# cloudwego/dynamicgo

Measured on AMD Instinct MI355X. Metric: conv/j2t GB/s JSON in + msgs/s, 64K-batch device-resident, 1→8 MI355X, higher is better.
Workload: dtype u8; 1 GPU; C2: 65536 flat baseline.Simple messages <=256 B, seed 42; global_batch=65536, msgs_per_rank=65536, thrift_bytes_rank0=6662181, flags=1, parallelism=dp1 (one batch per rank, descriptor broadcast over -), no data-path collective, inflight=2

## Files before the change

### dynamicgo_amd/csrc/flat_image.h

```cpp
#pragma once
#include <stdint.h>
#include <string.h>

namespace dg {

constexpr int FLI_WLO = -40;
constexpr int FLI_WN = 64;
constexpr uint32_t FLI_NP10U = 20, FLI_NP10D = 23;
constexpr uint32_t FLI_P10U = 0;
constexpr uint32_t FLI_P10D = FLI_P10U + 8 * FLI_NP10U;
constexpr uint32_t FLI_PW = FLI_P10D + 8 * FLI_NP10D;
constexpr uint32_t FLI_TABS = (FLI_PW + 8 * FLI_WN + 15) & ~15u;

static const double FLI_P10D_VALUES[FLI_NP10D] = {1e0,  1e1,  1e2,  1e3,  1e4,  1e5,  1e6,  1e7,  1e8,  1e9,  1e10, 1e11,
                                                  1e12, 1e13, 1e14, 1e15, 1e16, 1e17, 1e18, 1e19, 1e20, 1e21, 1e22};

constexpr uint32_t fli_blob16(uint32_t total_len) { return (total_len + 15) & ~15u; }
constexpr uint32_t fli_len(uint32_t total_len) { return fli_blob16(total_len) + FLI_TABS; }

inline void fli_build(const uint8_t *blob, uint32_t total_len, const uint64_t (*pw_hi)[2], uint8_t *img)
{
    const uint32_t b16 = fli_blob16(total_len);
    memset(img, 0, fli_len(total_len));
    memcpy(img, blob, total_len);
    uint8_t *t = img + b16;
    uint64_t v = 1;
    for (uint32_t k = 0; k < FLI_NP10U; k++, v *= 10) memcpy(t + FLI_P10U + 8 * k, &v, 8);
    memcpy(t + FLI_P10D, FLI_P10D_VALUES, sizeof FLI_P10D_VALUES);
    for (int k = 0; k < FLI_WN; k++) memcpy(t + FLI_PW + 8 * k, &pw_hi[FLI_WLO + 348 + k][1], 8);
}

}
```

### dynamicgo_amd/csrc/host_internal.h

```cpp
#pragma once
#include <hip/hip_runtime.h>

#include <stdint.h>
#include <stdlib.h>

#include <algorithm>
#include <memory>
#include <mutex>
#include <vector>

#include "../../include/dgj2t.h"
#include "../../include/dgj2t_desc.h"
#include "host_layout.h"

__attribute__((visibility("hidden"))) int set_err(int code, const char *fmt, ...);
#define HIPCHK(x)                                                                              \
    do {                                                                                       \
        hipError_t e_ = (x);                                                                   \
        if (e_ != hipSuccess) return set_err(DG_E_HIP, "%s: %s", #x, hipGetErrorString(e_));  \
    } while (0)


template <class T, hipError_t (*FREE)(void *)>
struct ArrBase {
    T *p = nullptr;
    uint64_t cap = 0;
    ArrBase() = default;
    ArrBase(ArrBase &&o) noexcept : p(o.p), cap(o.cap) { o.p = nullptr, o.cap = 0; }
    ArrBase &operator=(ArrBase &&o) noexcept
    {
        std::swap(p, o.p);
        std::swap(cap, o.cap);
        return *this;
    }
    ~ArrBase() { reset(); }
    void reset()
    {
        if (p) (void)FREE(p);
        p = nullptr, cap = 0;
    }
    operator T *() const { return p; }
};

template <class T>
struct DevArr : ArrBase<T, hipFree> {
    int alloc(uint64_t n)
    {
        HIPCHK(hipMalloc(&this->p, n * sizeof(T)));
        this->cap = n;
        return DG_OK;
    }
    int grow(uint64_t want)
    {
        if (this->cap >= want) return DG_OK;
        const uint64_t nc = std::max<uint64_t>(want, this->cap * 2);
        this->reset();
        return alloc(nc);
    }
};

template <class T>
struct PinArr : ArrBase<T, hipHostFree> {
    int alloc(uint64_t n, unsigned flags = hipHostMallocDefault)
    {
        HIPCHK(hipHostMalloc((void **)&this->p, n * sizeof(T), flags));
        this->cap = n;
        return DG_OK;
    }
    int grow(uint64_t want)
    {
        if (this->cap >= want) return DG_OK;
        const uint64_t nc = std::max<uint64_t>(std::max<uint64_t>(want, this->cap * 2), (1 << 16) / sizeof(T));
        this->reset();
        static const unsigned fl = getenv("DG_HOST_NUMA") ? hipHostMallocNumaUser : hipHostMallocDefault;
        return alloc(nc, fl);
    }
};

template <class H, hipError_t (*DESTROY)(H)>
struct Handle {
    H h = nullptr;
    Handle() = default;
    Handle(Handle &&o) noexcept : h(o.h) { o.h = nullptr; }
    Handle &operator=(Handle &&o) noexcept
    {
        std::swap(h, o.h);
        return *this;
    }
    ~Handle()
    {
        if (h) (void)DESTROY(h);
    }
    operator H() const { return h; }
};
struct Event : Handle<hipEvent_t, hipEventDestroy> {
    hipError_t create() { return hipEventCreate(&h); }
    hipError_t create(unsigned flags) { return hipEventCreateWithFlags(&h, flags); }
};
struct Stream : Handle<hipStream_t, hipStreamDestroy> {
    hipError_t create(unsigned flags) { return hipStreamCreateWithFlags(&h, flags); }
};

struct StreamOrder {
    Event done;
    hipStream_t last = nullptr;
    hipError_t acquire(hipStream_t s)
    {
        if (!done) {
            hipError_t e = done.create(hipEventDisableTiming | hipEventDisableSystemFence);
            if (e != hipSuccess) return e;
        }
        return last && last != s ? hipStreamWaitEvent(s, done, 0) : hipSuccess;
    }
    hipError_t publish(hipStream_t s)
    {
        hipError_t e = hipEventRecord(done, s);
        if (e == hipSuccess) last = s;
        return e;
    }
    hipError_t wait_host() const { return last ? hipEventSynchronize(done) : hipSuccess; }
    template <class T>
    int grow(DevArr<T> &a, uint64_t want)
    {
        if (a.cap >= want) return DG_OK;
        HIPCHK(wait_host());
        return a.grow(want);
    }
    void forget(const hipStream_t *s, int n)
    {
        if (std::find(s, s + n, last) != s + n) last = nullptr;
    }
};

struct SharedWs : StreamOrder {
    DevArr<uint8_t> ws;
};

struct AltCounters {
    uint32_t *set[2] = {nullptr, nullptr};
    uint32_t bytes = 0, cur = 0;
    uint32_t *mine() const { return set[cur]; }
    uint32_t *other() const { return set[cur ^ 1u]; }
    int init(DevArr<uint32_t> &buf, uint32_t words)
    {
        if (int rc = buf.alloc(4)) return rc;
        HIPCHK(hipMemset(buf, 0, 16));
        HIPCHK(hipDeviceSynchronize());
        set[0] = buf, set[1] = buf + words, bytes = 4 * words;
        return DG_OK;
    }
    void finish(bool ok, hipStream_t s)
    {
        if (ok) cur ^= 1u;
        else
            for (uint32_t *p : set) (void)hipMemsetAsync(p, 0, bytes, s);
    }
};

enum : uint32_t {
    CNT_BAIL = 0,
    CNT_BIG = 1,
    CNT_WAVEQ = 2,
    CNT_HUGE = 3,
    CNT_DEEP = 4,
    CNT_DEEP_DONE = 5,
    CNT_PACK = 6,
    CNT_T2J_A = 8,
    CNT_T2J_B = 16,
    T2J_DEEPQ = 0,
    T2J_BIG = 1,
    T2J_WAVEQ = 2,
    T2J_BAIL = 3,
};
constexpr uint32_t DG_NCOUNTS = 24;
constexpr uint32_t DG_J2T_COUNTS_BYTES = 6 * 4;
constexpr uint32_t FRAME_CAP = 4096;

constexpr int DG_MAX_SCRATCH = 40;
struct Scratch : StreamOrder {
    hipStream_t owner = nullptr;
    Stream side;
    Event side_done, side_go;
    DevArr<uint8_t> ws_fast;
    uint64_t ws_fast_lanes = 0;
    DevArr<uint64_t> deep_list;
    DevArr<uint32_t> counts;
    DevArr<uint32_t> bail_list, big_list;
    DevArr<uint8_t> ws_wave, ws_deep;
    DevArr<uint64_t> sums;
    DevArr<uint8_t> d_frame;
    std::vector<uint8_t> frame;
    DevArr<uint32_t> t2j_list;
    DevArr<uint32_t> t2j_big;
    DevArr<uint32_t> t2j_bail;
    AltCounters t2j_cnt;
    ~Scratch()
    {
        (void)wait_host();
        if (side) (void)hipStreamSynchronize(side);
    }
};

struct Knobs {
    int64_t flat = -1;
    int64_t wave_min = 512;
    int64_t wave_occ = 0;
    int64_t small_mpw = 64;
    int64_t list_blocks = 16;
    int64_t t2j_spread = 0;
    int64_t t2j_overlap = 0;
    int64_t t2j_wave_min = 256;
    int64_t flat_wrap = -1;
    int64_t tget_spread = 0;
    int64_t cut_wave_min = 4096;
    int64_t edit_reuse_rec = 0;
    int64_t edit_lanes = 4;
    int64_t edit_wave_min = 4096;
    int64_t kids_wide_min = 256;
    int64_t kids_no_scan = 0;
    int64_t cols_full_search = 0;
};

struct PipeBuf;
struct PipeBufDelete {
    void operator()(PipeBuf *p) const;
};

struct dg_ctx {
    int device = 0;
    Stream stream;
    int n_cu = 0;
    Knobs knobs;
    uint32_t rr = 0;
    std::mutex mu;
    const Event *kt = nullptr;
    Event fork_ev;
    std::vector<Event> side_ev;
    std::vector<Stream> side;
    SharedWs tget;
    DevArr<uint32_t> tget_list, tget_cnt_buf;
    AltCounters tget_cnt;
    StreamOrder cut;
    DevArr<uint32_t> cut_list, cut_cnt_buf;
    AltCounters cut_cnt;
    StreamOrder edit;
    DevArr<dg_tget_rec> edit_rec;
    uint64_t edit_rec_n = 0;
    StreamOrder editm;
    DevArr<dg_tget_rec> editm_rec;
    SharedWs kids;
    DevArr<uint32_t> kids_list, kids_cnt_buf;
    AltCounters kids_cnt;
    DevArr<uint64_t> kids_sums;
    SharedWs cols;
    DevArr<uint32_t> cols_list, cols_cnt_buf;
    AltCounters cols_cnt;
    DevArr<uint64_t> cols_sums;
    SharedWs t2j_tok;
    SharedWs t2j_deep;
    PinArr<uint8_t> h_down;
    PinArr<uint8_t> h_up;
    DevArr<uint64_t> d_pack_off;
    DevArr<uint8_t> d_pack;
    DevArr<uint8_t> d_cb;
    DevArr<uint64_t> d_aux;
    DevArr<uint64_t> d_ret;
    DevArr<uint32_t> d_out_len;
    DevArr<uint64_t> d_out_off;
    DevArr<uint8_t> d_out;
    DevArr<uint64_t> d_in_off;
    DevArr<uint8_t> d_json;
    DevArr<unsigned long long> d_stats;
    DevArr<uint64_t> d_zero;
    DevArr<uint32_t> d_pending;
    std::vector<std::unique_ptr<Scratch>> scratch;
    std::mutex pipe_mu;
    PinArr<uint8_t> h_pipe_aux, h_pipe_out;
    PinArr<uint8_t> h_pipe_ovf;
    DevArr<uint64_t> d_pipe_cur;
    std::vector<std::unique_ptr<PipeBuf, PipeBufDelete>> pipe;
    ~dg_ctx()
    {
        (void)hipSetDevice(device);
        if (stream) (void)hipStreamSynchronize(stream);
    }
};

struct Entry {
    std::unique_lock<std::mutex> lk;
    hipStream_t s = nullptr;
    int rc = DG_OK;
    Entry(dg_ctx *c, bool ok, void *stream = nullptr, const char *what = "bad args")
    {
        if (!ok) {
            rc = set_err(DG_E_INVALID, "%s", what);
            return;
        }
        lk = std::unique_lock<std::mutex>(c->mu);
        const hipError_t e = hipSetDevice(c->device);
        if (e != hipSuccess) rc = set_err(DG_E_HIP, "hipSetDevice(c->device): %s", hipGetErrorString(e));
        s = stream ? (hipStream_t)stream : (hipStream_t)c->stream;
    }
};

struct dg_desc {
    dg_ctx *ctx = nullptr;
    DevArr<uint8_t> d_blob;
    DevArr<uint8_t> d_flat;
    size_t len = 0;
    dg_desc_hdr hdr;
    DevArr<uint8_t> d_side;
    std::vector<uint8_t> hblob;
    size_t side_len = 0;
};

struct dg_path {
    dg_ctx *ctx;
    DevArr<uint8_t> d_blob;
    dg_path_hdr hdr;
};

struct dg_cols {
    dg_ctx *ctx;
    DevArr<uint8_t> d_blob;
    dg_path_hdr hdr;
    uint8_t kinds[DG_TGET_MAX_PATHS];
};

struct TGetBatch {
    const uint8_t *src;
    const uint64_t *in_off;
    uint64_t n;
    dg_tget_rec *rec;
    uint64_t *val_off;
    uint32_t *val_len;
    uint64_t max_len;
};

__attribute__((visibility("hidden"))) int dg_i_path_validate(const void *blob, size_t len, dg_path_hdr &h);

__attribute__((visibility("hidden"))) int tget_launch(dg_ctx *c, const dg_path *ps, uint8_t root_type,
                                                      const TGetBatch &b, hipStream_t s);

struct HMIn {
    const dg_hm_entry *tab = nullptr;
    uint32_t n_hm = 0;
    const uint8_t *bytes = nullptr;
    const dg_cb_entry *vm = nullptr;
};

struct BatchArgs {
    const uint8_t *src = nullptr;
    const uint64_t *in_off = nullptr;
    uint64_t n = 0, flags = 0;
    uint8_t *out = nullptr;
    const uint64_t *out_off = nullptr;
    uint32_t *out_len = nullptr;
    uint64_t *ret = nullptr;
    uint32_t *pending = nullptr;
    uint64_t max_len = 0;
    HMIn hm;
    uint64_t *aux = nullptr;
};

struct HostOut {
    uint8_t *out;
    uint64_t out_cap;
    uint64_t *out_off, *out_need;
};

struct PackChain {
    const uint64_t *base_in = nullptr;
    uint64_t dst_cap = 0;
    int base_mod16 = 0;
    uint64_t *ret_dst = nullptr, *cur_out = nullptr, *ovf_out = nullptr;
    hipEvent_t pack_after = nullptr;
};

__attribute__((visibility("hidden"))) void dg_i_scratch_release(dg_ctx *c, const hipStream_t *s, int n);

__attribute__((visibility("hidden"))) int scratch_for(dg_ctx *c, hipStream_t s, Scratch **out);

__attribute__((visibility("hidden"))) int dg_i_convert_pack(dg_ctx *c, const dg_desc *d, uint32_t root,
                                                            const BatchArgs &b, uint8_t *packed, uint64_t *pack_off,
                                                            hipStream_t s, const PackChain &ch);

__attribute__((visibility("hidden"))) int dg_i_pack_scan(dg_ctx *c, hipStream_t s, const BatchArgs &b, uint8_t *d_dst,
                                                         uint64_t *d_dst_off);

inline int empty_batch(uint64_t *off, uint64_t *need)
{
    if (off) off[0] = 0;
    if (need) *need = 0;
    return DG_OK;
}

struct HostBatch {
    dg_ctx *const c;
    const hipStream_t s;
    std::vector<uint64_t> io, so, vo, src;
    uint64_t n = 0, max_len = 0;
    bool busy = false;
    HostBatch(dg_ctx *c_, hipStream_t s_) : c(c_), s(s_) {}
    HostBatch(const HostBatch &) = delete;
    ~HostBatch()
    {
        if (busy) (void)hipStreamSynchronize(s);
    }
    int sync()
    {
        busy = false;
        HIPCHK(hipStreamSynchronize(s));
        return DG_OK;
    }
    int copy(void *dst, const void *from, uint64_t bytes, hipMemcpyKind kind)
    {
        busy = true;
        if (bytes) HIPCHK(hipMemcpyAsync(dst, from, bytes, kind, s));
        return DG_OK;
    }
    template <class F>
    int layout(const uint64_t *in_off, const uint64_t *idx, uint64_t m, F cap_of, bool with_slots = true,
               bool longest = true)
    {
        n = m, io.resize(m + 1), src.resize(idx ? m : 0);
        if (with_slots) so.resize(m + 1);
        uint64_t bad = 0, cap = 0;
        const int rc = dg::hl_layout(in_off, idx, m, cap_of, io.data(), with_slots ? so.data() : nullptr,
                                     idx ? src.data() : nullptr, longest && !idx ? &max_len : nullptr, &bad, &cap);
        if (rc == dg::HL_DESCENDING) return set_err(DG_E_INVALID, "in_off not ascending");
        if (rc) return set_err(DG_E_INVALID, "message %llu: an output of %llu bytes", (unsigned long long)bad,
                               (unsigned long long)cap);
        return DG_OK;
    }
    int messages(const uint64_t *in_off, uint64_t m, bool longest = true)
    {
        return layout(in_off, nullptr, m, [](uint64_t, uint64_t) { return uint64_t(0); }, false, longest);
    }
    int values(const uint64_t *val_off, uint64_t m, uint64_t K, uint64_t *max_val)
    {
        vo.resize(m * K + 1);
        return dg::hl_rebase(val_off, m * K, K, vo.data(), max_val) ? set_err(DG_E_INVALID, "val_off not ascending") : DG_OK;
    }
    int upload_messages(const uint8_t *thrift, const uint64_t *in_off)
    {
        int rc;
        if ((rc = c->d_json.grow(io[n] + 64)) || (rc = c->d_in_off.grow(n + 1))) return rc;
        if (src.empty()) rc = copy(c->d_json, thrift + in_off[0], io[n], hipMemcpyHostToDevice);
        for (uint64_t k = 0; k < src.size() && !rc; k++)
            rc = copy(c->d_json + io[k], thrift + src[k], io[k + 1] - io[k], hipMemcpyHostToDevice);
        if (rc) return rc;
        HIPCHK(hipMemsetAsync(c->d_json + io[n], 0, 64, s));
        return copy(c->d_in_off, io.data(), (n + 1) * 8, hipMemcpyHostToDevice);
    }
    int upload_slots(bool packs = true)
    {
        int rc;
        if ((rc = c->d_out.grow(so[n] + 64)) || (rc = c->d_out_off.grow(n + 1)) || (rc = c->d_out_len.grow(n + 1)) ||
            (rc = c->d_ret.grow(n + 1)) ||
            (packs && ((rc = c->d_pack.grow(so[n] + 64)) || (rc = c->d_pack_off.grow(n + 1)))))
            return rc;
        return copy(c->d_out_off, so.data(), (n + 1) * 8, hipMemcpyHostToDevice);
    }
    int upload_values(const uint8_t *val, const uint64_t *val_off, uint64_t shared)
    {
        const uint64_t vtotal = val_off ? vo.back() : shared;
        int rc;
        if ((rc = c->d_cb.grow(vtotal + 64)) || (rc = c->d_aux.grow(vo.size())) ||
            (rc = copy(c->d_cb, val_off ? val + val_off[0] : val, vtotal, hipMemcpyHostToDevice)))
            return rc;
        HIPCHK(hipMemsetAsync(c->d_cb + vtotal, 0, 64, s));
        return copy(c->d_aux, vo.data(), vo.size() * 8, hipMemcpyHostToDevice);
    }
    int pack(bool by_ret, uint64_t *ret, uint64_t *pack_off, uint32_t *len = nullptr)
    {
        BatchArgs pb;
        pb.out = c->d_out, pb.out_off = c->d_out_off, pb.out_len = c->d_out_len, pb.n = n;
        if (by_ret) pb.ret = c->d_ret;
        int rc;
        if ((rc = dg_i_pack_scan(c, s, pb, c->d_pack, c->d_pack_off)) ||
            (rc = copy(ret, c->d_ret, n * 8, hipMemcpyDeviceToHost)) ||
            (len && (rc = copy(len, c->d_out_len, n * 4, hipMemcpyDeviceToHost))) ||
            (rc = copy(pack_off, c->d_pack_off, (n + 1) * 8, hipMemcpyDeviceToHost)))
            return rc;
        return sync();
    }
    int download(void *dst, const void *d_from, uint64_t bytes)
    {
        if (int rc = copy(dst, d_from, bytes, hipMemcpyDeviceToHost)) return rc;
        return bytes ? sync() : DG_OK;
    }
    int pack_and_download(const HostOut &o, uint64_t *ret)
    {
        if (int rc = pack(false, ret, o.out_off)) return rc;
        const uint64_t total = o.out_off[n];
        if (o.out_need) *o.out_need = total;
        if (total > o.out_cap || (!o.out && total))
            return set_err(DG_E_NOMEM, "output needs %llu bytes", (unsigned long long)total);
        return download(o.out, c->d_pack, total);
    }
};

inline int upload_blob(DevArr<uint8_t> &d, const void *blob, size_t len, const char *what)
{
    if (int rc = d.alloc(len + 16)) return rc;
    hipError_t e = hipMemcpy(d, blob, len, hipMemcpyHostToDevice);
    if (e == hipSuccess) e = hipMemset(d + len, 0, 16);
    if (e == hipSuccess) e = hipDeviceSynchronize();
    if (e != hipSuccess) return set_err(DG_E_HIP, "%s upload: %s", what, hipGetErrorString(e));
    return DG_OK;
}

template <class P>
void destroy_with_blob(P *p)
{
    if (!p) return;
    {
        Entry g(p->ctx, true);
        p->d_blob.reset();
    }
    delete p;
}

inline uint32_t edit_step_extra(uint32_t kind, uint32_t key_len)
{
    return kind == DG_PS_FIELD ? 3u : kind == DG_PS_INDEX ? 0u : kind == DG_PS_STRKEY ? 4u + key_len
           : kind == DG_PS_BINKEY ? key_len : 8u;
}

template <class Lane, class Wave>
hipError_t launch_splice_routes(const dg_ctx *c, uint64_t n, uint32_t waves, bool no_wave, Lane lane, Wave wave)
{
    hipError_t err = hipSuccess;
    if (c->knobs.edit_wave_min > 0) {
        const int64_t g = c->knobs.edit_lanes;
        lane(g == 4 || g == 16 ? (uint32_t)g : 1u);
        err = hipGetLastError();
    }
    if (err == hipSuccess && !no_wave) {
        const uint64_t want = (n + waves - 1) / waves;
        wave((uint32_t)std::min<uint64_t>(want, (uint64_t)c->n_cu * 8));
        err = hipGetLastError();
    }
    return err;
}
```

### dynamicgo_amd/csrc/j2t_fast.h

```cpp
#pragma once
#include "j2t_device.h"

namespace dg {

#ifdef DG_FPROF
DGI unsigned long long *fprof_slots()
{
    __shared__ unsigned long long s_fp[16][17];
    return &s_fp[0][0];
}
DGI void fprof_mark(int k)
{
    const uint64_t now = __builtin_amdgcn_s_memtime();
    const uint32_t lane = threadIdx.x & 63, w = threadIdx.x >> 6;
    const uint64_t ex = __builtin_amdgcn_read_exec();
    if (lane == (uint32_t)__builtin_ctzll(ex)) {
        unsigned long long *f = fprof_slots() + w * 17;
        f[k] += now - f[16];
        f[16] = now;
    }
}
#define FP_MARK(k) fprof_mark(k)
#else
#define FP_MARK(k)
#endif

#define SI typename S::idx

constexpr uint32_t FK_STRUCT = 1, FK_MAP = 2, FK_LIST = 3;
constexpr uint32_t FAST_LDS_DEPTH = 8;

struct FFrame {
    uint32_t a;
    uint32_t b;
    uint64_t u;
};
typedef __attribute__((address_space(3))) FFrame LFFrame;
typedef const __attribute__((address_space(3))) double lds_f64;

constexpr uint64_t FAST_FLAGS = DG_F_ALLOW_UNKNOWN | DG_F_WRITE_DEFAULT | DG_F_ENABLE_VM | DG_F_ENABLE_I2S |
                                DG_F_WRITE_REQUIRE | DG_F_NO_BASE64 | DG_F_WRITE_OPTIONAL | DG_F_NO_WRITE_BASE |
                                DG_F_ENABLE_HM | DG_F_HM_SPLIT | DG_F_CB_COLLECT;

constexpr int EL_WLO = -40;
constexpr int EL_WN = 64;
struct FastTabs {
    const __attribute__((address_space(3))) uint64_t *p10u;
    lds_f64 *p10d;
    const __attribute__((address_space(3))) uint64_t *pw = nullptr;
};
DGI void el_window_fill(uint64_t *pw, uint32_t t)
{
    if (t < (uint32_t)EL_WN) pw[t] = DG_POW10_M128[EL_WLO + 348 + (int)t][1];
}
DGI bool eisel_lemire_t(uint64_t mant, int exp10, int sgn, double &val, const FastTabs &tb)
{
    if (exp10 < -348 || exp10 > 347) return false;
    const uint32_t wi = (uint32_t)(exp10 - EL_WLO);
    const uint64_t p_hi = tb.pw && wi < (uint32_t)EL_WN ? tb.pw[wi] : DG_POW10_M128[exp10 + 348][1];
    return eisel_lemire_p(mant, exp10, sgn, val, p_hi);
}


template <class S>
DGI uint32_t digits8(S &src, SI i, uint64_t &x)
{
    uint64_t w = src.get8(i);
    const uint32_t xl = (uint32_t)w ^ 0x30303030u, xh = (uint32_t)(w >> 32) ^ 0x30303030u;
    x = (uint64_t)xl | ((uint64_t)xh << 32);
    uint32_t ndl = (((xl & 0x7F7F7F7Fu) + 0x76767676u) | xl) & 0x80808080u;
    uint32_t ndh = (((xh & 0x7F7F7F7Fu) + 0x76767676u) | xh) & 0x80808080u;
    SI lim = src.n - i;
    if (lim < 8) {
        if (lim <= 4) {
            ndh = 0x80808080u;
            if (lim < 4) ndl |= lim <= 0 ? 0x80808080u : (0x80808080u & (~0u << (lim << 3)));
        } else {
            ndh |= 0x80808080u & (~0u << ((lim - 4) << 3));
        }
    }
    if (ndl) return (uint32_t)__builtin_ctz(ndl) >> 3;
    return ndh ? 4u + ((uint32_t)__builtin_ctz(ndh) >> 3) : 8u;
}

DGI uint32_t swar_val4(uint32_t x, uint32_t k)
{
    uint32_t y = k >= 4 ? x : (k == 0 ? 0u : x << ((4 - k) << 3));
    y &= 0x0F0F0F0Fu;
    y = (((y << 3) + (y << 1)) + (y >> 8)) & 0x00FF00FFu;
    return __umul24(y & 0xFFu, 100u) + (y >> 16);
}
DGI uint64_t swar_val(uint64_t x, uint32_t t)
{
    const uint32_t t1 = t < 4 ? t : 4u, t2 = t - t1;
    const uint32_t v1 = swar_val4((uint32_t)x, t1);
    if (!t2) return v1;
    const uint32_t v2 = swar_val4((uint32_t)(x >> 32), t2);
    const uint32_t p = t2 == 1 ? 10u : t2 == 2 ? 100u : t2 == 3 ? 1000u : 10000u;
    return (uint64_t)v1 * p + v2;
}

DGI uint32_t acc_digits(uint64_t &man, int &nd, uint64_t x, uint32_t k, const FastTabs &tb)
{
    (void)tb;
    uint32_t room = (uint32_t)(19 - nd);
    uint32_t t = k < room ? k : room;
    if (t) {
        uint32_t p = (t & 1) ? 10u : 1u;
        p = (t & 2) ? p * 100u : p;
        p = (t & 4) ? p * 10000u : p;
        p = (t & 8) ? 100000000u : p;
        man = man * (uint64_t)p + swar_val(x, t);
        nd += (int)t;
    }
    return t;
}

DGI bool atof_exact_l(uint64_t man, int exp, int sgn, double &val, const FastTabs &tb)
{
    val = (double)man;
    if (man >> 52 != 0) return false;
    val = with_sign(val, sgn);
    if (exp == 0 || man == 0) return true;
    if (exp > 0 && exp <= 15 + 22) {
        if (exp > 22) {
            val = __dmul_rn(val, tb.p10d[exp - 22]);
            exp = 22;
        }
        if (val > 1e15 || val < -1e15) return false;
        val = __dmul_rn(val, tb.p10d[exp]);
        return true;
    }
    if (exp < 0 && exp >= -22) {
        val = __ddiv_rn(val, tb.p10d[-exp]);
        return true;
    }
    return false;
}

template <class S>
DGI bool fast_int_regs(const S &src, int64_t &iv, double &dv, int32_t &end)
{
    const int32_t n = (int32_t)src.n;
    if (n < 1 || n > 20) return false;
    const uint64_t a0 = src.get8(0), a1 = src.get8(8), a2 = src.get8(16);
    const uint32_t neg = (uint8_t)a0 == '-' ? 1u : 0u;
    const uint32_t nd = (uint32_t)n - neg;
    const uint64_t d0 = neg ? (a0 >> 8) | (a1 << 56) : a0, d1 = neg ? (a1 >> 8) | (a2 << 56) : a1,
                   d2 = neg ? a2 >> 8 : a2;
    const uint64_t x0 = d0 ^ 0x3030303030303030ull, x1 = d1 ^ 0x3030303030303030ull, x2 = d2 ^ 0x3030303030303030ull;
    auto nondig = [](uint64_t x) { return (((x & 0x7F7F7F7F7F7F7F7Full) + 0x7676767676767676ull) | x) & 0x8080808080808080ull; };
    auto upto = [](uint32_t k) { return k >= 8 ? ~0ull : (1ull << (k << 3)) - 1; };
    const uint32_t t0 = nd < 8 ? nd : 8u, t1 = nd <= 8 ? 0u : nd - 8 < 8 ? nd - 8 : 8u, t2 = nd <= 16 ? 0u : nd - 16;
    const uint64_t bad = (nondig(x0) & upto(t0)) | (nondig(x1) & upto(t1)) | (nondig(x2) & upto(t2));
    const uint32_t f = (uint32_t)(x0 & 0xFF);
    if (nd < 1 || nd > 19 || bad || (f == 0 && nd > 1)) return false;
    auto p10 = [](uint32_t t) {
        uint32_t p = (t & 1) ? 10u : 1u;
        p = (t & 2) ? p * 100u : p;
        p = (t & 4) ? p * 10000u : p;
        return (t & 8) ? 100000000u : p;
    };
    uint64_t man = swar_val(x0, t0);
    man = man * (uint64_t)p10(t1) + swar_val(x1, t1);
    man = man * (uint64_t)p10(t2) + swar_val(x2, t2);
    if ((man >> 63) && !(neg && man == (1ull << 63))) return false;
    const int sgn = neg ? -1 : 1;
    iv = (int64_t)(man * (uint64_t)(int64_t)sgn);
    dv = man ? with_sign((double)man, sgn) : 0.0;
    end = n;
    return true;
}

template <class S>
DGI bool fast_dec_regs(const S &src, uint64_t &man, int &exp10, int &sgn)
{
    const int32_t n = (int32_t)src.n;
    if (n < 3 || n > 21) return false;
    const uint64_t a0 = src.get8(0), a1 = src.get8(8), a2 = src.get8(16);
    const uint32_t neg = (uint8_t)a0 == '-' ? 1u : 0u;
    const uint32_t len = (uint32_t)n - neg;
    const uint64_t d0 = neg ? (a0 >> 8) | (a1 << 56) : a0, d1 = neg ? (a1 >> 8) | (a2 << 56) : a1,
                   d2 = neg ? a2 >> 8 : a2;
    auto upto = [](uint32_t k) { return k >= 8 ? ~0ull : (1ull << (k << 3)) - 1; };
    auto eqdot = [](uint64_t x) {
        const uint64_t y = x ^ 0x2E2E2E2E2E2E2E2Eull;
        return ~(((y & 0x7F7F7F7F7F7F7F7Full) + 0x7F7F7F7F7F7F7F7Full) | y | 0x7F7F7F7F7F7F7F7Full);
    };
    const uint32_t u0 = len < 8 ? len : 8u, u1 = len <= 8 ? 0u : len - 8 < 8 ? len - 8 : 8u,
                   u2 = len <= 16 ? 0u : len - 16;
    const uint64_t m0 = eqdot(d0) & upto(u0), m1 = eqdot(d1) & upto(u1), m2 = eqdot(d2) & upto(u2);
    if (__builtin_popcountll(m0) + __builtin_popcountll(m1) + __builtin_popcountll(m2) != 1) return false;
    const uint32_t pd = m0 ? (uint32_t)__builtin_ctzll(m0) >> 3
                       : m1 ? 8u + ((uint32_t)__builtin_ctzll(m1) >> 3) : 16u + ((uint32_t)__builtin_ctzll(m2) >> 3);
    if (pd < 1 || pd + 2 > len) return false;
    const uint64_t s0 = (d0 >> 8) | (d1 << 56), s1 = (d1 >> 8) | (d2 << 56), s2 = d2 >> 8;
    const uint64_t k0 = upto(pd), k1 = pd <= 8 ? 0ull : upto(pd - 8), k2 = pd <= 16 ? 0ull : upto(pd - 16);
    const uint64_t r0 = (d0 & k0) | (s0 & ~k0), r1 = (d1 & k1) | (s1 & ~k1), r2 = (d2 & k2) | (s2 & ~k2);
    const uint32_t nd = len - 1;
    const uint64_t x0 = r0 ^ 0x3030303030303030ull, x1 = r1 ^ 0x3030303030303030ull, x2 = r2 ^ 0x3030303030303030ull;
    auto nondig = [](uint64_t x) { return (((x & 0x7F7F7F7F7F7F7F7Full) + 0x7676767676767676ull) | x) & 0x8080808080808080ull; };
    const uint32_t t0 = nd < 8 ? nd : 8u, t1 = nd <= 8 ? 0u : nd - 8 < 8 ? nd - 8 : 8u, t2 = nd <= 16 ? 0u : nd - 16;
    const uint64_t bad = (nondig(x0) & upto(t0)) | (nondig(x1) & upto(t1)) | (nondig(x2) & upto(t2));
    if (nd > 19 || bad || ((x0 & 0xFF) == 0 && pd > 1)) return false;
    auto p10 = [](uint32_t t) {
        uint32_t p = (t & 1) ? 10u : 1u;
        p = (t & 2) ? p * 100u : p;
        p = (t & 4) ? p * 10000u : p;
        return (t & 8) ? 100000000u : p;
    };
    uint64_t m = swar_val(x0, t0);
    m = m * (uint64_t)p10(t1) + swar_val(x1, t1);
    m = m * (uint64_t)p10(t2) + swar_val(x2, t2);
    man = m;
    exp10 = -(int)(nd - pd);
    sgn = neg ? -1 : 1;
    return true;
}

template <class S, class = void>
struct is_regsrc {
    static constexpr bool value = false;
};
template <class S>
struct is_regsrc<S, decltype((void)S::kRegs)> {
    static constexpr bool value = S::kRegs;
};

template <class S>
DGI bool fast_vnumber(S &src, SI &p, const FastTabs &tb, int64_t &iv, double &dv, bool &isint)
{
    SI i = p;
    uint64_t man = 0;
    int exp10 = 0, sgn = 1;
    bool trunc = false, regdec = false;
    if constexpr (is_regsrc<S>::value) {
        int32_t e;
        if (p == 0 && fast_int_regs(src, iv, dv, e)) {
            isint = true;
            p = (SI)e;
            return true;
        }
        if (p == 0 && fast_dec_regs(src, man, exp10, sgn)) {
            regdec = true;
            i = (SI)src.n;
        }
    }
    if (!regdec) {
    uint8_t c = src.at(i);
    if (c == '-') {
        sgn = -1;
        c = src.at(++i);
    }
    if ((uint8_t)(c - '0') > 9) return false;
    isint = true;
    iv = 0;
    dv = 0.0;
    if (c == '0') {
        uint8_t c1 = src.at(i + 1);
        if (c1 != '.' && c1 != 'e' && c1 != 'E') {
            p = i + 1;
            return true;
        }
    }
    int nd = 0;
    bool dbl = false;
    uint64_t x;
    for (;;) {
        uint32_t k = digits8(src, i, x);
        uint32_t t = acc_digits(man, nd, x, k, tb);
        exp10 += (int)(k - t);
        i += k;
        if (k < 8) break;
    }
    if (exp10 > 0) trunc = true;
    if (src.at(i) == '.') {
        i++;
        dbl = true;
        if ((uint8_t)(src.at(i) - '0') > 9) return false;
    }
    if (man == 0 && exp10 == 0) {
        while (src.at(i) == '0') {
            i++;
            exp10--;
        }
        nd = 0;
    }
    while (dbl && nd < 19) {
        uint32_t k = digits8(src, i, x);
        uint32_t t = acc_digits(man, nd, x, k, tb);
        exp10 -= (int)t;
        i += t;
        if (t < 8) break;
    }
    while (dbl) {
        uint32_t k = digits8(src, i, x);
        if (k) trunc = true;
        i += k;
        if (k < 8) break;
    }
    c = src.at(i);
    if (c == 'e' || c == 'E') {
        int esm = 1, e = 0;
        dbl = true;
        c = src.at(++i);
        if (c == '+' || c == '-') {
            esm = c == '+' ? 1 : -1;
            c = src.at(++i);
        }
        if ((uint8_t)(c - '0') > 9) return false;
        while ((uint8_t)(c - '0') <= 9) {
            if (e < 10000) e = e * 10 + (c - '0');
            c = src.at(++i);
        }
        exp10 += e * esm;
    } else if (!dbl) {
        bool ovf = exp10 != 0 || ((man >> 63) == 1 && (((uint64_t)(int64_t)sgn) & man) != (1ull << 63));
        if (!ovf) {
            iv = (int64_t)(man * (uint64_t)(int64_t)sgn);
            dv = with_sign((double)man, sgn);
            p = i;
            return true;
        }
    }
    }
    double val;
    if (!atof_exact_l(man, exp10, sgn, val, tb)) {
        if (!eisel_lemire_t(man, exp10, sgn, val, tb)) return false;
        if (trunc) {
            double vu;
            if (!eisel_lemire_t(man + 1, exp10, sgn, vu, tb) || vu != val) return false;
        }
    }
    if ((__double_as_longlong(val) << 1) == 0xFFE0000000000000ull) return false;
    isint = false;
    dv = val;
    p = i;
    return true;
}

template <class O>
DGI bool emit_number(O &out, uint8_t tt, bool isint, int64_t iv, double dv)
{
    switch (tt) {
    case DG_T_BYTE: out.w8(isint ? (uint8_t)iv : (uint8_t)cvt32(dv)); return true;
    case DG_T_I16: out.w16(isint ? (uint16_t)iv : (uint16_t)cvt32(dv)); return true;
    case DG_T_I32: out.w32(isint ? (uint32_t)iv : (uint32_t)cvt32(dv)); return true;
    case DG_T_I64: out.w64(isint ? (uint64_t)iv : (uint64_t)cvt64(dv)); return true;
    case DG_T_DOUBLE: out.w64((uint64_t)__double_as_longlong(dv)); return true;
    }
    return false;
}

template <class S, class O>
DGI void fast_copy(S &src, SI s0, SI n, O &out)
{
    SI i = 0;
    for (; i + 8 <= n; i += 8) out.wle(src.get8(s0 + i), 8);
    if (i < n) out.wle(src.get8(s0 + i), (uint32_t)(n - i));
}

template <class S>
DGI bool hex4w(S &src, SI i, uint32_t &v)
{
    uint32_t w = (uint32_t)src.get8(i);
    uint32_t r = 0;
#pragma unroll
    for (int k = 0; k < 4; k++) {
        int h = hexv((uint8_t)(w >> (8 * k)));
        if (h < 0) return false;
        r = (r << 4) | (uint32_t)h;
    }
    v = r;
    return true;
}

template <class S, class O>
DGI bool fast_unquote(S &src, SI s0, SI nb, O &out)
{
    SI i = s0, end = s0 + nb;
    while (i < end) {
        uint64_t w = src.get8(i);
        SI rem = end - i;
        uint64_t m = eqbytes(w, '\\');
        if (rem < 8) m &= (1ull << (rem << 3)) - 1;
        if (m == 0) {
            uint32_t k = rem < 8 ? (uint32_t)rem : 8u;
            out.wle(w, k);
            i += k;
            continue;
        }
        uint32_t j = (uint32_t)__builtin_ctzll(m) >> 3;
        if (j) out.wle(w, j);
        i += j;
        if (end - i < 2) return false;
        uint8_t c = src.at(i + 1);
        uint8_t cc;
        switch (c) {
        case '/': cc = '/'; break;
        case '"': cc = '"'; break;
        case 'b': cc = '\b'; break;
        case 'f': cc = '\f'; break;
        case 'n': cc = '\n'; break;
        case 'r': cc = '\r'; break;
        case 't': cc = '\t'; break;
        case '\\': cc = '\\'; break;
        case 'u': cc = 0; break;
        default: return false;
        }
        if (c != 'u') {
            out.w8(cc);
            i += 2;
            continue;
        }
        if (end - i < 6) return false;
        uint32_t r0, r1;
        if (!hex4w(src, i + 2, r0)) return false;
        i += 6;
        if (r0 <= 0x7f) {
            out.w8((uint8_t)r0);
        } else if (r0 <= 0x7ff) {
            out.wle((0xc0 | (r0 >> 6)) | ((0x80 | (r0 & 0x3f)) << 8), 2);
        } else if (r0 < 0xd800 || r0 > 0xdfff) {
            out.wle((0xe0 | (r0 >> 12)) | ((0x80 | ((r0 >> 6) & 0x3f)) << 8) | ((0x80 | (r0 & 0x3f)) << 16), 3);
        } else {
            if (end - i < 6 || r0 > 0xdbff || src.at(i) != '\\' || src.at(i + 1) != 'u') return false;
            if (!hex4w(src, i + 2, r1)) return false;
            if (r1 < 0xdc00 || r1 > 0xdfff) return false;
            i += 6;
            r0 = ((r0 - 0xd800) << 10) + (r1 - 0xdc00) + 0x10000;
            out.wle((0xf0 | (r0 >> 18)) | ((0x80 | ((r0 >> 12) & 0x3f)) << 8) | ((0x80 | ((r0 >> 6) & 0x3f)) << 16) |
                        ((uint64_t)(0x80 | (r0 & 0x3f)) << 24),
                    4);
        }
    }
    return true;
}

template <class S>
DGI bool fast_string(S &src, SI &p, Out &out)
{
    SI s0 = p;
    bool esc;
    SI e = advance_string(src, s0, esc);
    if (e < 0) return false;
    p = e;
    SI nb = e - 1 - s0;
    if (!esc) {
        out.w32((uint32_t)nb);
        fast_copy(src, s0, nb, out);
        return true;
    }
    uint64_t lp = out.alloc(4);
    uint64_t st = out.len;
    if (!fast_unquote(src, s0, nb, out)) return false;
    out.put32(lp, (uint32_t)(out.len - st));
    return true;
}

DGI bool b64_4(uint32_t w, uint32_t &o)
{
    const uint32_t H = 0x80808080u;
    if (w & H) return false;
#define DG_GE(lo) ((w + (uint32_t)(0x80 - (lo)) * 0x01010101u) & H)
    const uint32_t up = DG_GE('A') & ~DG_GE('Z' + 1);
    const uint32_t lw = DG_GE('a') & ~DG_GE('z' + 1);
    const uint32_t dg = DG_GE('0') & ~DG_GE('9' + 1);
#undef DG_GE
    const uint32_t pl = zb32(w ^ 0x2B2B2B2Bu), sl = zb32(w ^ 0x2F2F2F2Fu);
    if ((up | lw | dg | pl | sl) != H) return false;
    const uint32_t off = (ff32(up) & 0xBFBFBFBFu) | (ff32(lw) & 0xB9B9B9B9u) | (ff32(dg) & 0x04040404u) |
                         (ff32(pl) & 0x13131313u) | (ff32(sl) & 0x10101010u);
    const uint32_t v = ((w & 0x7F7F7F7Fu) + (off & 0x7F7F7F7Fu)) ^ ((w ^ off) & H);
    const uint32_t t = ((v & 0x3Fu) << 18) | (((v >> 8) & 0x3Fu) << 12) | (((v >> 16) & 0x3Fu) << 6) | (v >> 24);
    o = (t >> 16) | (t & 0xFF00u) | ((t & 0xFFu) << 16);
    return true;
}
DGI bool b64_8(uint64_t w, uint64_t &o)
{
    uint32_t lo, hi;
    const bool a = b64_4((uint32_t)w, lo), b = b64_4((uint32_t)(w >> 32), hi);
    o = (uint64_t)lo | ((uint64_t)hi << 24);
    return a && b;
}

template <class S>
DGI bool fast_binary(S &src, SI &p, Out &out)
{
    SI s0 = p;
    bool esc;
    SI e = advance_string(src, s0, esc);
    if (e < 0 || esc) return false;
    p = e;
    SI nb = e - 1 - s0;
    int64_t want = -1;
    if ((nb & 3) == 0) {
        const uint8_t c2 = nb ? src.raw(s0 + nb - 2) : 0, c3 = nb ? src.raw(s0 + nb - 1) : 0;
        want = (int64_t)(nb / 4 * 3) - (c3 == '=' ? (c2 == '=' ? 2 : 1) : 0);
    }
    uint64_t lp = 0;
    if (want >= 0) out.w32((uint32_t)want);
    else lp = out.alloc(4);
    SI ip = 0;
    int64_t op = 0;
    while (ip + 8 <= nb) {
        uint64_t o;
        if (!b64_8(src.get8(s0 + ip), o)) break;
        out.wle(o, 6);
        ip += 8;
        op += 6;
    }
    if (ip < nb) {
        op = b64decode_from(out, src, s0, nb, ip, op);
        if (op < 0) return false;
    }
    if (want >= 0) return op == want;
    out.put32(lp, (uint32_t)op);
    return true;
}

template <class S, int AS>
DGI bool key_eq(S &src, SI k0, uint32_t kn, const __attribute__((address_space(AS))) uint64_t *pk)
{
    for (uint32_t j = 0; j < kn; j += 8) {
        uint64_t a = src.get8(k0 + j);
        uint32_t rem = kn - j;
        if (rem < 8) a &= (1ull << (rem << 3)) - 1;
        if (a != pk[j >> 3]) return false;
    }
    return true;
}

template <bool LEAN = false, class S, class DV>
DGI bool fast_convert(const DV &D, S &src, Out &out, uint64_t flag, uint32_t root, LFFrame *fr, uint32_t fstride,
                      const FastTabs &tb)
{
    if (src.n == 0 || ldrec(&D.T[root]).ttype == DG_T_STRING) return false;
    SI p = 0;
    uint32_t sp = 0;
    uint32_t ca = 0, ck = 0, cb = 0;
    uint64_t cu = 0;
    bool null_val = false;
    uint64_t unwind = 0;
    uint32_t lastf = 0;
    uint32_t td = root;
    bool vmv = false;
    uint8_t c;

#define FAST_PUSH(na, nk, nu)                                             \
    do {                                                                  \
        if (sp) {                                                         \
            if (sp > FAST_LDS_DEPTH) return false;                        \
            LFFrame &f_ = fr[(sp - 1) * fstride];                         \
            f_.a = ca;                                                    \
            f_.b = ck | (cb << 2);                                        \
            f_.u = cu;                                                    \
        }                                                                 \
        sp++;                                                             \
        ca = (na);                                                        \
        ck = (nk);                                                        \
        cb = 0;                                                           \
        cu = (nu);                                                        \
    } while (0)
#define FAST_POP()                                                        \
    do {                                                                  \
        if (--sp) {                                                       \
            const LFFrame &f_ = fr[(sp - 1) * fstride];                   \
            ca = f_.a;                                                    \
            ck = f_.b & 3;                                                \
            cb = f_.b >> 2;                                               \
            cu = f_.u;                                                    \
        }                                                                 \
    } while (0)

    for (;;) {
        FP_MARK(0);
        c = src.at(p++);
        while (c <= ' ') {
            if (!isspace_(c)) return false;
            c = src.at(p++);
        }
        const dg_type t = ldrec(&D.T[td]);
        bool opened = false;
        FP_MARK(1);
        if (vmv) {
            vmv = false;
            const bool quoted = c == '"';
            bool number = true;
            if (quoted) {
                if (t.ttype == DG_T_STRING) {
                    if (!fast_string(src, p, out)) return false;
                    number = false;
                } else if (src.at(p) == '"') {
                    if constexpr (LEAN) return false;
                    const dg_field f = ldrec(&D.F[lastf]);
                    if (f.dflt_len != DG_NONE) {
                        for (uint32_t j = 0; j < f.dflt_len; j++) out.w8(D.P[f.dflt_off + j]);
                    } else {
                        switch (t.ttype) {
                        case DG_T_BOOL:
                        case DG_T_BYTE: out.w8(0); break;
                        case DG_T_I16: out.w16(0); break;
                        case DG_T_I32: out.w32(0); break;
                        case DG_T_I64:
                        case DG_T_DOUBLE: out.w64(0); break;
                        default: return false;
                        }
                    }
                    p += 1;
                    number = false;
                }
            } else {
                if (c != '-' && (uint8_t)(c - '0') > 9) return false;
                p -= 1;
            }
            if (number) {
                const SI s0 = p;
                int64_t iv;
                double dv;
                bool isint;
                if (!fast_vnumber(src, p, tb, iv, dv, isint)) return false;
                if (t.ttype == DG_T_STRING) {
                    out.w32((uint32_t)(p - s0));
                    fast_copy(src, s0, p - s0, out);
                } else if (t.ttype == DG_T_I16) {
                    emit_number(out, DG_T_I16, isint, iv, dv);
                    emit_number(out, DG_T_BYTE, isint, iv, dv);
                } else if (t.ttype == DG_T_BOOL || !emit_number(out, t.ttype, isint, iv, dv)) {
                    return false;
                }
                if (quoted) {
                    if (src.at(p) != '"') return false;
                    p += 1;
                }
            }
            goto after_value;
        }
        switch (c) {
        case '"':
            if (t.ttype != DG_T_STRING) return false;
            if ((flag & DG_F_NO_BASE64) == 0 && (t.flags & DG_TF_BINARY)) {
                if (!fast_binary(src, p, out)) return false;
                FP_MARK(2);
            } else {
                if (!fast_string(src, p, out)) return false;
                FP_MARK(3);
            }
            break;
        case '0': case '1': case '2': case '3': case '4':
        case '5': case '6': case '7': case '8': case '9': case '-': {
            p -= 1;
            int64_t iv;
            double dv;
            bool isint;
            if (!fast_vnumber(src, p, tb, iv, dv, isint)) return false;
            FP_MARK(4);
            if (!emit_number(out, t.ttype, isint, iv, dv)) return false;
            FP_MARK(5);
            break;
        }
        case 't':
            if (p + 3 > src.n || (uint32_t)src.get8(p - 1) != VS_TRUE || t.ttype != DG_T_BOOL) return false;
            p += 3;
            out.w8(1);
            break;
        case 'f':
            if (p + 4 > src.n || (uint32_t)src.get8(p) != VS_ALSE || t.ttype != DG_T_BOOL) return false;
            p += 4;
            out.w8(0);
            break;
        case 'n':
            if (p + 3 > src.n || (uint32_t)src.get8(p - 1) != VS_NULL || sp == 0) return false;
            p += 3;
            null_val = true;
            break;
        case '[': {
            if (t.ttype != DG_T_LIST && t.ttype != DG_T_SET) return false;
            out.w8(ldrec(&D.T[t.elem]).ttype);
            uint64_t bp = out.alloc(4);
            FAST_PUSH(t.elem, FK_LIST, bp);
            opened = true;
            break;
        }
        case '{':
            if (t.ttype == DG_T_STRUCT) {
                const dg_struct sd = ldrec(&D.S[t.st]);
                if (sd.req_words != 1) return false;
                if ((flag & DG_F_ENABLE_HM) && (sd.flags & DG_SF_HTTP_MAPPING)) return false;
                FAST_PUSH(t.st, FK_STRUCT, D.R[sd.req_begin]);
            } else if (t.ttype == DG_T_MAP) {
                out.wle(ldrec(&D.T[t.key]).ttype | ((uint32_t)ldrec(&D.T[t.elem]).ttype << 8), 2);
                uint64_t bp = out.alloc(4);
                FAST_PUSH(t.elem, FK_MAP, bp | ((uint64_t)t.key << 32));
            } else {
                return false;
            }
            opened = true;
            break;
        default:
            return false;
        }

        after_value:
        FP_MARK(6);
        bool first = opened;
        for (;;) {
            if (sp == 0) {
                out.finish();
                return out.len <= out.cap;
            }
            c = src.at(p++);
            while (c <= ' ') {
                if (!isspace_(c)) return false;
                c = src.at(p++);
            }
            if (ck == FK_LIST) {
                if (first) {
                    first = false;
                    if (c == ']') {
                        FAST_POP();
                        continue;
                    }
                    p -= 1;
                    td = ca;
                    break;
                }
                if (null_val) null_val = false;
                else cb++;
                if (c == ',') {
                    td = ca;
                    break;
                }
                if (c != ']') return false;
                out.put32(cu, cb);
                FAST_POP();
                continue;
            }
            if (first) {
                first = false;
                if (c == '}') {
                    if (ck == FK_MAP) {
                        FAST_POP();
                        continue;
                    }
                    goto close_struct;
                }
            } else if (ck == FK_MAP) {
                if (null_val) {
                    null_val = false;
                    out.set_len(unwind);
                } else {
                    cb++;
                }
                if (c == '}') {
                    out.put32((uint32_t)cu, cb);
                    FAST_POP();
                    continue;
                }
                if (c != ',') return false;
                c = src.at(p++);
                while (c <= ' ') {
                    if (!isspace_(c)) return false;
                    c = src.at(p++);
                }
            } else {
                if (null_val) {
                    null_val = false;
                    const dg_field f = ldrec(&D.F[lastf]);
                    const dg_struct sd = ldrec(&D.S[ca]);
                    uint64_t m = 1ull << (lastf - sd.field_begin);
                    if (f.required == DG_REQ_DEFAULT || f.required == DG_REQ_REQUIRED) cu |= m;
                    else if (f.required == DG_REQ_OPTIONAL) cu &= ~m;
                    out.set_len(unwind);
                }
                if (c == '}') goto close_struct;
                if (c != ',') return false;
                c = src.at(p++);
                while (c <= ' ') {
                    if (!isspace_(c)) return false;
                    c = src.at(p++);
                }
            }
            FP_MARK(7);
            if (c != '"') return false;
            {
                SI k0 = p;
                uint32_t kn;
                int32_t fi = -1;
                dg_field f;
                if (ck == FK_STRUCT) {
                    const dg_struct sdp = ldrec(&D.S[ca]);
                    if (cb < sdp.n_fields) {
                        f = ldrec(&D.F[sdp.field_begin + cb]);
                        kn = f.key_len;
                        if ((f.flags & (DG_FF_ALIAS_SELF | DG_FF_KEY_PLAIN)) == (DG_FF_ALIAS_SELF | DG_FF_KEY_PLAIN) &&
                            k0 + (SI)kn < src.n && key_eq(src, k0, kn, (decltype(&D.R[0]))(&D.P[f.key_off])) &&
                            src.raw(k0 + (SI)kn) == '"') {
                            fi = (int32_t)(sdp.field_begin + cb);
                            p = k0 + (SI)kn + 1;
                        }
                    }
                }
                if (fi < 0) {
                    bool esc;
                    SI e = advance_string(src, k0, esc);
                    if (e < 0 || esc) return false;
                    p = e;
                    kn = (uint32_t)(e - 1 - k0);
                }
                c = src.at(p++);
                while (c <= ' ') {
                    if (!isspace_(c)) return false;
                    c = src.at(p++);
                }
                if (c != ':') return false;
                FP_MARK(8);
                if (ck == FK_MAP) {
                    unwind = out.len;
                    const uint8_t kt = ldrec(&D.T[(uint32_t)(cu >> 32)]).ttype;
                    if (kt == DG_T_STRING) {
                        out.w32(kn);
                        fast_copy(src, k0, kn, out);
                    } else {
                        if constexpr (LEAN) return false;
                        S ks = src.sub(k0, kn);
                        SI q = 0;
                        int64_t iv;
                        double dv;
                        bool isint;
                        if (!fast_vnumber(ks, q, tb, iv, dv, isint)) return false;
                        if (!emit_number(out, kt, isint, iv, dv)) return false;
                    }
                    td = ca;
                    break;
                }
                const dg_struct sd = ldrec(&D.S[ca]);
                if (fi < 0 && cb < sd.n_fields) {
                    f = ldrec(&D.F[sd.field_begin + cb]);
                    if ((f.flags & DG_FF_ALIAS_SELF) && f.key_len == kn &&
                        key_eq(src, k0, kn, (decltype(&D.R[0]))(&D.P[f.key_off])))
                        fi = (int32_t)(sd.field_begin + cb);
                }
                if (fi < 0) {
                    uint32_t h = DG_NAME_HASH_SEED;
                    for (uint32_t j = 0; j < kn; j += 8) {
                        const uint64_t w = src.get8(k0 + (SI)j);
                        const uint32_t r = kn - j < 8 ? kn - j : 8u;
#pragma unroll
                        for (uint32_t b = 0; b < 8; b++)
                            if (b < r) h = DG_NAME_HASH_STEP(h, (uint8_t)(w >> (8 * b)));
                    }
                    for (uint32_t s = h & sd.name_mask;; s = (s + 1) & sd.name_mask) {
                        const dg_name nm = ldrec(&D.N[sd.name_begin + s]);
                        if (nm.field == DG_NONE) break;
                        if (nm.hash == h && nm.key_len == kn &&
                            key_eq(src, k0, kn, (decltype(&D.R[0]))(&D.P[nm.key_off]))) {
                            fi = (int32_t)nm.field;
                            break;
                        }
                    }
                    if (fi >= 0) f = ldrec(&D.F[fi]);
                }
                if (fi < 0 || ((f.flags & DG_FF_REQUEST_BASE) && (flag & DG_F_NO_WRITE_BASE))) {
                    if (fi < 0 && (flag & DG_F_ALLOW_UNKNOWN) == 0) return false;
                    c = src.at(p++);
                    while (c <= ' ') {
                        if (!isspace_(c)) return false;
                        c = src.at(p++);
                    }
                    p -= 1;
                    if constexpr (LEAN) return false;
                    SkipRes sr = skip_one(src, p, nullptr, 64);
                    if (sr.r < 0) return false;
                    p = sr.p;
                    continue;
                }
                uint32_t k = (uint32_t)fi - sd.field_begin;
                const dg_type ft = ldrec(&D.T[f.type]);
                if ((flag & DG_F_ENABLE_VM) && f.vm != DG_VM_NONE) {
                    if (f.vm != DG_VM_JSCONV) return false;
                    vmv = true;
                    lastf = (uint32_t)fi;
                } else {
                    unwind = out.len;
                    lastf = (uint32_t)fi;
                }
                out.wle((uint32_t)ft.ttype | ((uint32_t)__builtin_bswap16(f.id) << 8), 3);
                cu &= ~(1ull << k);
                cb = k + 1;
                td = f.type;
                FP_MARK(9);
                break;
            }
        close_struct: {
            FP_MARK(10);
            const dg_struct sd = ldrec(&D.S[ca]);
            uint64_t bits = cu;
            bool wr = flag & DG_F_WRITE_REQUIRE, wd = flag & DG_F_WRITE_DEFAULT, wo = flag & DG_F_WRITE_OPTIONAL;
            while (bits) {
                uint32_t k = __builtin_ctzll(bits);
                bits &= bits - 1;
                const dg_field f = ldrec(&D.F[sd.field_begin + k]);
                if (f.flags & DG_FF_REQUEST_BASE) continue;
                if (!wr && f.required == DG_REQ_REQUIRED) return false;
                if ((wr && f.required == DG_REQ_REQUIRED) || (wd && f.required == DG_REQ_DEFAULT) ||
                    (wo && f.required == DG_REQ_OPTIONAL)) {
                    if constexpr (LEAN) return false;
                    const dg_type ft = ldrec(&D.T[f.type]);
                    out.wle((uint32_t)ft.ttype | ((uint32_t)__builtin_bswap16(f.id) << 8), 3);
                    if (f.dflt_len != DG_NONE) {
                        for (uint32_t j = 0; j < f.dflt_len; j++) out.w8(D.P[f.dflt_off + j]);
                        continue;
                    }
                    switch (ft.ttype) {
                    case DG_T_BOOL:
                    case DG_T_BYTE: out.w8(0); break;
                    case DG_T_I16: out.w16(0); break;
                    case DG_T_I32:
                    case DG_T_STRING: out.w32(0); break;
                    case DG_T_I64:
                    case DG_T_DOUBLE: out.w64(0); break;
                    case DG_T_LIST:
                    case DG_T_SET:
                        out.w8(ldrec(&D.T[ft.elem]).ttype);
                        out.w32(0);
                        break;
                    case DG_T_MAP:
                        out.w8(ldrec(&D.T[ft.key]).ttype);
                        out.w8(ldrec(&D.T[ft.elem]).ttype);
                        out.w32(0);
                        break;
                    case DG_T_STRUCT: out.w8(0); break;
                    default: return false;
                    }
                }
            }
            out.w8(0);
            FAST_POP();
            FP_MARK(11);
            continue;
        }
        }
    }
#undef FAST_PUSH
#undef FAST_POP
}
#undef SI

}
```

### dynamicgo_amd/csrc/j2t_flat.h

```cpp
#pragma once
#include "flat_image.h"
#include "j2t_small.h"

namespace dg {

constexpr uint32_t FL_G = 4;
#ifndef DG_FL_WAVES
#define DG_FL_WAVES 4
#endif
constexpr uint32_t FL_WAVES = DG_FL_WAVES;
#ifndef DG_FL_FPW
#define DG_FL_FPW 2
#endif
constexpr uint32_t FL_FPW = DG_FL_FPW;
constexpr uint32_t FL_SLOTS = FL_FPW * FL_WAVES;
constexpr uint32_t FL_MPB = 64;
constexpr uint32_t FL_LW = 9;
constexpr uint32_t FL_MAXLEN = 256;
constexpr uint32_t FL_SLOTW = FL_MAXLEN / 8;
constexpr uint32_t FL_STAGEW = FL_MPB * FL_SLOTW;
constexpr uint32_t FL_SLACKW = FL_G * FL_LW + 2;
constexpr uint32_t FL_MAXF = 24;
constexpr uint32_t FL_DESC = 16 * 1024;
#ifndef DG_FL_INLINE
#define DG_FL_INLINE 8
#endif
#ifndef DG_FL_CHUNK
#define DG_FL_CHUNK 32
#endif
constexpr uint32_t FL_INLINE = DG_FL_INLINE;
constexpr uint32_t FL_CHUNK = DG_FL_CHUNK;
constexpr uint32_t FL_MAXTASK = 320;
constexpr uint32_t FL_KEYS = 32;
constexpr uint32_t FL_NESC = 8;
static_assert(FLI_WLO == EL_WLO && FLI_WN == EL_WN, "the image's window is FastTabs' window");
constexpr uint32_t FL_FMAPW = FL_SLOTS * FL_MPB / 8;
static_assert(FL_MAXTASK >= FL_FMAPW + FL_MPB, "the task area holds the field map and, behind it, an unstaged block's offsets");
#ifndef DG_FL_WPE
#define DG_FL_WPE 4
#endif

#ifndef DG_FL_DEFER_NUM
#define DG_FL_DEFER_NUM 0
#endif
#ifndef DG_FL_PERM
#define DG_FL_PERM 0
#endif
#ifndef DG_FL_REMAP
#define DG_FL_REMAP 1
#endif

#ifdef DG_FLPROF_G
#define FLG_ARG , uint64_t *flg
#define FLG_PASS , flg
#define FLG(k)                                             \
    do {                                                   \
        const uint64_t now_ = __builtin_amdgcn_s_memtime(); \
        flg[k] += now_ - flg[7];                           \
        flg[7] = now_;                                     \
    } while (0)
#else
#define FLG_ARG
#define FLG_PASS
#define FLG(k)
#endif
DGI uint32_t fl_slot(uint32_t w, uint32_t h)
{
    return DG_FL_PERM == 1 ? (h & 1 ? (h + 1) * FL_WAVES - 1 - w : h * FL_WAVES + w) : w + h * FL_WAVES;
}

#define DG_DPP(v, ctrl) ((uint32_t)__builtin_amdgcn_update_dpp(0, (int)(v), (ctrl), 0xF, 0xF, false))
DGI uint32_t g4_incl_sum(uint32_t v, uint32_t g)
{
    uint32_t t = DG_DPP(v, 0x111);
    v += g >= 1 ? t : 0u;
    t = DG_DPP(v, 0x112);
    v += g >= 2 ? t : 0u;
    return v;
}
DGI uint32_t g4_sum(uint32_t v)
{
    v += DG_DPP(v, 0xB1);
    v += DG_DPP(v, 0x4E);
    return v;
}
DGI uint32_t g4_next(uint32_t v, uint32_t g)
{
    const uint32_t t = DG_DPP(v, 0x101);
    return g < 3 ? t : 0u;
}

DGI uint32_t eq32(uint32_t w, uint32_t cc) { return zb32(w ^ cc); }

struct LSrc {
    typedef int32_t idx;
    const __attribute__((address_space(3))) uint64_t *w8;
    int32_t off0;
    int32_t n;
    DGI void init(const __attribute__((address_space(3))) uint64_t *words, int32_t off, int32_t len)
    {
        w8 = words;
        off0 = off;
        n = len;
    }
    DGI uint8_t raw(int32_t i) const
    {
        return ((const __attribute__((address_space(3))) uint8_t *)w8)[off0 + i];
    }
    DGI uint8_t at(int32_t i) const { return (uint32_t)i < (uint32_t)n ? raw(i) : 0; }
    DGI uint64_t get8(int32_t i) const
    {
        const uint32_t b = (uint32_t)(off0 + i), k = b >> 3, sh = (b & 7) << 3;
        const uint64_t lo = w8[k], hi = w8[k + 1];
        return (lo >> sh) | ((hi << 1) << (63 - sh));
    }
    DGI LSrc sub(int32_t s0, int32_t len) const
    {
        LSrc r;
        r.init(w8, off0 + s0, len);
        return r;
    }
};

constexpr int32_t RSL_MAX = 24;
struct RSrcL {
    typedef int32_t idx;
    static constexpr bool kRegs = true;
    uint64_t w0, w1, w2, w3, w4;
    uint32_t sh;
    int32_t n;
    DGI void load(const LSrc &src, int32_t p, int32_t len)
    {
        const uint32_t b = (uint32_t)(src.off0 + p);
        const __attribute__((address_space(3))) uint64_t *q = src.w8 + (b >> 3);
        sh = b & 7;
        n = len;
        w0 = q[0];
        w1 = q[1];
        w2 = q[2];
        w3 = q[3];
        w4 = q[4];
    }
    DGI uint64_t word(uint32_t j) const { return j == 0 ? w0 : j == 1 ? w1 : j == 2 ? w2 : j == 3 ? w3 : w4; }
    DGI uint8_t raw(int32_t i) const
    {
        const uint32_t b = sh + (uint32_t)i;
        return (uint8_t)(word(b >> 3) >> ((b & 7) << 3));
    }
    DGI uint8_t at(int32_t i) const { return (uint32_t)i < (uint32_t)n ? raw(i) : 0; }
    DGI uint64_t get8(int32_t i) const
    {
        const uint32_t b = sh + (uint32_t)i, j = b >> 3, s8 = (b & 7) << 3;
        return (word(j) >> s8) | ((word(j + 1) << 1) << (63 - s8));
    }
};

enum : uint32_t { FV_NONE = 0, FV_NUM, FV_STR, FV_BIN, FV_BOOL, FV_NUMSTR };
struct FField {
    int32_t fi;
    uint32_t kind;
    uint32_t s0, nb;
    bool esc;
    bool isint;
    int64_t iv;
    double dv;
    uint32_t size;
    uint8_t tt;
    uint16_t id;
    bool i16q;
    bool defer;
};

template <class S>
DGI uint32_t skip_ws(S &s, uint32_t p)
{
    while (p < (uint32_t)s.n && isspace_(s.raw((int32_t)p))) p++;
    return p;
}

template <class S, class DV>
DGI int32_t fl_lookup(const DV &D, const dg_struct &sd, S &src, uint32_t k0, uint32_t kn)
{
    typedef typename S::idx SI;
    uint32_t h = DG_NAME_HASH_SEED;
    for (uint32_t j = 0; j < kn; j += 8) {
        const uint64_t w = src.get8((SI)(k0 + j));
        const uint32_t r = kn - j < 8 ? kn - j : 8u;
#pragma unroll
        for (uint32_t bb = 0; bb < 8; bb++)
            if (bb < r) h = DG_NAME_HASH_STEP(h, (uint8_t)(w >> (8 * bb)));
    }
    for (uint32_t s = h & sd.name_mask;; s = (s + 1) & sd.name_mask) {
        const dg_name nm = ldrec(&D.N[sd.name_begin + s]);
        if (nm.field == DG_NONE) return -1;
        if (nm.hash == h && nm.key_len == kn && key_eq(src, (SI)k0, kn, (decltype(&D.R[0]))(&D.P[nm.key_off])))
            return (int32_t)nm.field;
    }
}

typedef const __attribute__((address_space(3))) uint32_t lds_esc;
DGI uint32_t esc_pos(uint32_t x) { return x & 0xFFF; }
DGI uint32_t esc_in(uint32_t x) { return (x >> 12) & 1 ? 6u : 2u; }
DGI uint32_t esc_cp(uint32_t x) { return (x >> 13) & 0xFFFF; }
DGI uint32_t esc_out(uint32_t x) { const uint32_t cp = esc_cp(x); return cp <= 0x7f ? 1u : cp <= 0x7ff ? 2u : 3u; }
DGI uint32_t esc_utf8(uint32_t x)
{
    const uint32_t cp = esc_cp(x);
    return cp <= 0x7f ? cp
           : cp <= 0x7ff ? (0xc0 | (cp >> 6)) | ((0x80 | (cp & 0x3f)) << 8)
                         : (0xe0 | (cp >> 12)) | ((0x80 | ((cp >> 6) & 0x3f)) << 8) | ((0x80 | (cp & 0x3f)) << 16);
}
DGI bool fl_hex4(uint32_t w, uint32_t &v)
{
    uint32_t r = 0, ok = 1;
#pragma unroll
    for (int k = 0; k < 4; k++) {
        const uint32_t b = (w >> (8 * k)) & 0xFF, d = b - '0', l = (b | 0x20) - 'a';
        ok &= (uint32_t)(d < 10) | (uint32_t)(l < 6);
        r = (r << 4) | (d < 10 ? d : (l + 10) & 0xF);
    }
    v = r;
    return ok != 0;
}
DGI uint32_t fl_escape(uint32_t p, uint64_t e0)
{
    const uint32_t c = (uint32_t)(e0 >> 8) & 0xFF;
    if (c == 'u') {
        uint32_t cp;
        if (!fl_hex4((uint32_t)(e0 >> 16), cp) || (cp >= 0xd800 && cp <= 0xdfff)) return 0;
        return 0x80000000u | p | (1u << 12) | (cp << 13);
    }
    const uint32_t cc = c == 'b' ? 8u : c == 'f' ? 12u : c == 'n' ? 10u : c == 'r' ? 13u : c == 't' ? 9u : c;
    const bool ok = (c == '"') | (c == '\\') | (c == '/') | (c == 'b') | (c == 'f') | (c == 'n') | (c == 'r') | (c == 't');
    return ok ? 0x80000000u | p | (cc << 13) : 0u;
}
DGI bool fl_esc_in(lds_esc *E, uint32_t ne, uint32_t a, uint32_t b, uint32_t &shrink)
{
    bool any = false;
    shrink = 0;
    for (uint32_t e = 0; e < ne; e++) {
        const uint32_t x = E[e];
        const uint32_t p = esc_pos(x);
        const bool in = p >= a && p < b;
        any |= in;
        shrink += in ? esc_in(x) - esc_out(x) : 0u;
    }
    return any;
}

template <bool KO = false, class S, class DV>
DGI bool fl_field(const DV &D, const dg_struct &sd, S &src, uint32_t sk, uint32_t ck, uint32_t ek, uint32_t nq,
                  bool hasbs, lds_esc *E, uint32_t ne, const __attribute__((address_space(3))) uint64_t *KW,
                  const __attribute__((address_space(3))) uint32_t *KM, uint32_t nk, uint32_t k, uint64_t flag,
                  const FastTabs &tb, FField &F FLG_ARG)
{
    typedef typename S::idx SI;
    const uint8_t d_s = src.raw((SI)sk), d_q = src.raw((SI)(ck - 1)), d_v = src.raw((SI)(ck + 1)),
                  d_e = src.raw((SI)(ek - 1));
    const bool pred = k < sd.n_fields;
    dg_field f = ldrec(&D.F[sd.field_begin + (pred ? k : 0u)]);
    uint32_t p = sk, q = ck, v0 = ck + 1, ve = ek;
    uint8_t cs = d_s, cq = d_q, c = d_v, ce = d_e;
    if (isspace_(d_s) | isspace_(d_q) | isspace_(d_v) | isspace_(d_e) | (ck + 1 >= ek)) {
        p = skip_ws(src, sk);
        while (q > p && isspace_(src.raw((SI)(q - 1)))) q--;
        v0 = skip_ws(src, ck + 1);
        while (ve > v0 && isspace_(src.raw((SI)(ve - 1)))) ve--;
        if (v0 >= ve) return false;
        cs = src.raw((SI)p);
        cq = src.raw((SI)(q - 1));
        c = src.raw((SI)v0);
        ce = src.raw((SI)(ve - 1));
    }
    if ((q < p + 2) | (cs != '"') | (cq != '"') | (nq != (c == '"' ? 4u : 2u))) return false;
    const uint32_t k0 = p + 1, kn = q - 1 - k0;
    FLG(1);
    uint32_t shrink = 0;
    if (hasbs && fl_esc_in(E, ne, k0, k0 + kn, shrink)) return false;
    int32_t fi = -1;
    uint64_t a0m = 0, a1m = 0;
    {
        const __attribute__((address_space(3))) uint64_t *pk = (decltype(&D.R[0]))(&D.P[f.key_off]);
        bool hit;
        if (kn <= 16) {
            const uint64_t a0 = src.get8((SI)k0), a1 = src.get8((SI)(k0 + 8)), b0 = pk[0], b1 = pk[1];
            const uint64_t m0 = kn >= 8 ? ~0ull : (1ull << (kn << 3)) - 1;
            const uint64_t m1 = kn >= 16 ? ~0ull : kn <= 8 ? 0ull : (1ull << ((kn - 8) << 3)) - 1;
            a0m = a0 & m0;
            a1m = a1 & m1;
            hit = (a0m == b0) & ((kn <= 8) | (a1m == b1));
        } else {
            hit = key_eq(src, (SI)k0, kn, pk);
        }
        if (pred & ((f.flags & DG_FF_ALIAS_SELF) != 0) & (f.key_len == kn) & hit) fi = (int32_t)(sd.field_begin + k);
    }
    if (fi < 0) {
        if (nk && kn <= 16) {
#pragma unroll 4
            for (uint32_t e = 0; e < nk; e++) {
                const uint32_t mt = KM[e];
                if (((mt >> 24) == kn) & (KW[2 * e] == a0m) & (KW[2 * e + 1] == a1m)) fi = (int32_t)(mt & 0xFFFFFFu);
            }
        } else {
            fi = fl_lookup(D, sd, src, k0, kn);
        }
        if (fi >= 0) f = ldrec(&D.F[fi]);
    }
    if constexpr (KO) {
        F.fi = fi;
        return true;
    }
    FLG(2);
    F.defer = false;
    uint32_t vk;
    uint32_t vs0 = 0, vnb = 0;
    bool vesc = false, isint = false, bv = false;
    int64_t iv = 0;
    double dv = 0.0;
    if (c == '"') {
        if ((ve - v0 < 2) | (ce != '"')) return false;
        vs0 = v0 + 1;
        vnb = ve - 1 - vs0;
        vesc = hasbs && fl_esc_in(E, ne, vs0, vs0 + vnb, shrink);
        vk = FV_STR;
    } else if (c == '-' || (uint8_t)(c - '0') <= 9) {
        const bool later = DG_FL_DEFER_NUM && fi >= 0 && !((flag & DG_F_ENABLE_VM) && f.vm != DG_VM_NONE);
        if (!later) {
            const int32_t nl = (int32_t)(ve - v0);
            bool okn;
            if (nl <= RSL_MAX) {
                RSrcL rs;
                rs.load(src, (int32_t)v0, nl);
                int32_t qq = 0;
                okn = fast_vnumber(rs, qq, tb, iv, dv, isint) && qq == nl;
            } else {
                SI qq = (SI)v0;
                okn = fast_vnumber(src, qq, tb, iv, dv, isint) && (uint32_t)qq == ve;
            }
            if (!okn) return false;
        }
        F.defer = later;
        vs0 = v0;
        vnb = ve - v0;
        vk = FV_NUM;
    } else if (c == 't') {
        if (ve - v0 != 4 || (uint32_t)src.get8((SI)v0) != VS_TRUE) return false;
        bv = true;
        vk = FV_BOOL;
    } else if (c == 'f') {
        if (ve - v0 != 5 || (uint32_t)src.get8((SI)(v0 + 1)) != VS_ALSE) return false;
        vk = FV_BOOL;
    } else {
        return false;
    }
    FLG(3);
    F.fi = fi;
    if (fi < 0 || ((f.flags & DG_FF_REQUEST_BASE) && (flag & DG_F_NO_WRITE_BASE))) {
        if (fi < 0 && !(flag & DG_F_ALLOW_UNKNOWN)) return false;
        if (fi >= 0) return false;
        F.kind = FV_NONE;
        F.size = 0;
        return true;
    }
    const dg_type ft = ldrec(&D.T[f.type]);
    const uint8_t tt = ft.ttype;
    const bool bin = (ft.flags & DG_TF_BINARY) && !(flag & DG_F_NO_BASE64);
    F.tt = tt;
    F.id = f.id;
    F.i16q = false;
    uint32_t vsize;
    if ((flag & DG_F_ENABLE_VM) && f.vm != DG_VM_NONE) {
        if (f.vm != DG_VM_JSCONV) return false;
        if (vk == FV_STR && tt != DG_T_STRING) {
            if (vnb == 0 || vesc) return false;
            S sub = src.sub((SI)vs0, (SI)vnb);
            SI qq = 0;
            if (!fast_vnumber(sub, qq, tb, iv, dv, isint) || (uint32_t)qq != vnb) return false;
            vk = FV_NUM;
        } else if (vk == FV_NUM && tt == DG_T_STRING) {
            vk = FV_NUMSTR;
        } else if (vk == FV_BOOL) {
            return false;
        }
        if (vk == FV_NUM && tt == DG_T_I16) F.i16q = true;
    }
    switch (vk) {
    case FV_STR:
        if (tt != DG_T_STRING) return false;
        if (bin) {
            if (vesc || (vnb & 3)) return false;
            const uint8_t c2 = vnb ? src.raw((SI)(vs0 + vnb - 2)) : 0, c3 = vnb ? src.raw((SI)(vs0 + vnb - 1)) : 0;
            vsize = 4 + vnb / 4 * 3 - (c3 == '=' ? (c2 == '=' ? 2 : 1) : 0);
            vk = FV_BIN;
        } else if (vesc) {
            vsize = 4 + vnb - shrink;
        } else {
            vsize = 4 + vnb;
        }
        break;
    case FV_NUMSTR:
        vsize = 4 + vnb;
        break;
    case FV_NUM:
        switch (tt) {
        case DG_T_BYTE: vsize = 1; break;
        case DG_T_I16: vsize = F.i16q ? 3 : 2; break;
        case DG_T_I32: vsize = 4; break;
        case DG_T_I64: case DG_T_DOUBLE: vsize = 8; break;
        default: return false;
        }
        break;
    default:
        if (tt != DG_T_BOOL) return false;
        vsize = 1;
        break;
    }
    F.kind = vk;
    F.s0 = vs0;
    F.nb = vnb;
    F.esc = vesc;
    F.isint = isint;
    F.iv = vk == FV_BOOL ? (int64_t)bv : iv;
    F.dv = dv;
    F.size = 3 + vsize;
    FLG(4);
    return true;
}

template <class S, class O>
DGI void body_copy(S &src, uint32_t s0, uint32_t n, O &o)
{
    fast_copy(src, (typename S::idx)s0, (typename S::idx)n, o);
}
template <class S, class O>
DGI bool body_b64(S &src, uint32_t s0, uint32_t n, bool last, O &o)
{
    typedef typename S::idx SI;
    uint32_t ip = 0;
    const uint32_t full = last && n >= 4 ? n - 4 : n;
    for (; ip + 8 <= full; ip += 8) {
        uint64_t v;
        if (!b64_8(src.get8((SI)(s0 + ip)), v)) return false;
        o.wle(v, 6);
    }
    for (; ip < full; ip += 4) {
        uint32_t v;
        if (!b64_4((uint32_t)src.get8((SI)(s0 + ip)), v)) return false;
        o.wle(v, 3);
    }
    if (last && n >= 4) {
        uint32_t w = (uint32_t)src.get8((SI)(s0 + ip));
        const uint32_t c2 = (w >> 16) & 0xFF, c3 = w >> 24;
        if (c2 == '=' && c3 != '=') return false;
        const uint32_t keep = c3 == '=' ? (c2 == '=' ? 1u : 2u) : 3u;
        if (c3 == '=') w = (w & 0x00FFFFFFu) | ((uint32_t)'A' << 24);
        if (c2 == '=') w = (w & 0xFF00FFFFu) | ((uint32_t)'A' << 16);
        uint32_t v;
        if (!b64_4(w, v)) return false;
        o.wle(v, keep);
    }
    return true;
}

template <class S, class O>
DGI uint32_t flat_write(S &src, const FField &F, const FastTabs &tb, O &o, lds_esc *E, uint32_t ne)
{
    typedef typename S::idx SI;
    if (F.kind == FV_NONE) return 1;
    bool isint = F.isint;
    int64_t iv = F.iv;
    double dv = F.dv;
    if (F.kind == FV_NUM && F.defer) {
        SI qq = (SI)F.s0;
        if (!fast_vnumber(src, qq, tb, iv, dv, isint) || (uint32_t)qq != F.s0 + F.nb) return 0;
    }
    o.wle((uint32_t)F.tt | ((uint32_t)__builtin_bswap16(F.id) << 8), 3);
    switch (F.kind) {
    case FV_BOOL: o.w8((uint8_t)iv); return 1;
    case FV_NUM:
        if (F.i16q) {
            emit_number(o, DG_T_I16, isint, iv, dv);
            emit_number(o, DG_T_BYTE, isint, iv, dv);
            return 1;
        }
        return emit_number(o, F.tt, isint, iv, dv) ? 1u : 0u;
    case FV_NUMSTR:
    case FV_STR:
        o.w32(F.kind == FV_NUMSTR ? F.nb : F.size - 7);
        if (F.esc) {
            uint32_t cur = F.s0;
            const uint32_t end = F.s0 + F.nb;
            for (uint32_t it = 0; it < FL_NESC; it++) {
                uint32_t best = 0xFFFFFFFFu;
                for (uint32_t e = 0; e < ne; e++) {
                    const uint32_t x = E[e], p = esc_pos(x);
                    if (p >= cur && p < end && p < esc_pos(best)) best = x;
                }
                if (best == 0xFFFFFFFFu) break;
                const uint32_t p = esc_pos(best);
                body_copy(src, cur, p - cur, o);
                o.wle(esc_utf8(best), esc_out(best));
                cur = p + esc_in(best);
            }
            body_copy(src, cur, end - cur, o);
            return 1;
        }
        if (F.nb > FL_INLINE) return 2;
        body_copy(src, F.s0, F.nb, o);
        return 1;
    default:
        o.w32(F.size - 7);
        if (F.nb > FL_INLINE) return 2;
        return body_b64(src, F.s0, F.nb, true, o) ? 1u : 0u;
    }
}

struct FlatParams {
    const uint8_t *img;
    dg_desc_hdr hdr;
    uint32_t *bail_count;
    uint32_t *bail_list;
    uint32_t wrap;
    uint32_t wrap_inner;
    uint64_t wrap_ok;
};

#ifdef DG_FLPROF
#define FLP_DECL uint64_t flp_t = __builtin_amdgcn_s_memtime(); uint64_t flp[8] = {0, 0, 0, 0, 0, 0, 0, 0};
#define FLP(k)                                              \
    do {                                                    \
        const uint64_t now_ = __builtin_amdgcn_s_memtime(); \
        flp[k] += now_ - flp_t;                             \
        flp_t = now_;                                       \
    } while (0)
#define FLP_END()                                                                        \
    do {                                                                                 \
        if ((threadIdx.x & 63) == 0 && (blockIdx.x & 31) == 0)                           \
            for (int k_ = 0; k_ < 8; k_++) atomicAdd(&P.stats[2 + k_], (unsigned long long)flp[k_]); \
    } while (0)
#else
#define FLP_DECL
#define FLP(k)
#define FLP_END()
#endif
#ifdef DG_FLPROF_F
#define FLF_DECL uint64_t flf[12] = {0, 0, 0, 0, 0, 0, 0, 0, 0, 0, 0, 0};
#define FLF_T0() const uint64_t flf_t0 = __builtin_amdgcn_s_memtime()
#define FLF_ADD(k) do { if ((k) < 12) flf[k] += __builtin_amdgcn_s_memtime() - flf_t0; } while (0)
#define FLF_END()                                                                         \
    do {                                                                                  \
        if ((threadIdx.x & 63) == 0 && (blockIdx.x & 31) == 0)                            \
            for (int k_ = 0; k_ < 12; k_++) atomicAdd(&P.stats[2 + k_], (unsigned long long)flf[k_]); \
    } while (0)
#else
#define FLF_DECL
#define FLF_T0()
#define FLF_ADD(k)
#define FLF_END()
#endif

struct FlatLds {
    uint64_t in[FL_STAGEW + FL_SLACKW];
    uint64_t task[FL_MAXTASK];
    uint64_t oa[FL_MPB];
    uint32_t cap[FL_MPB];
    uint32_t ok[FL_MPB];
    uint32_t n[FL_MPB];
    uint32_t lw[FL_MPB];
    uint32_t oc[FL_MPB];
    uint32_t nfq[FL_MPB];
    uint32_t plo[FL_MPB], phi[FL_MPB];
    uint32_t big[FL_MPB];
    uint32_t nbytes[FL_MPB];
    uint32_t wid[FL_MPB];
    uint32_t nesc[FL_MPB];
    uint32_t esc[FL_MPB * FL_NESC];
    uint64_t kw[2 * FL_KEYS];
    uint32_t km[FL_KEYS];
    uint32_t fkm[FL_SLOTS];
    uint32_t sep[FL_MAXF * FL_MPB];
    uint16_t col[FL_MAXF * FL_MPB];
    uint16_t size[2 * FL_SLOTS * FL_MPB];
    uint32_t fseen[FL_MPB];
    uint32_t rounds, ntask, tgrab, noremap;
    uint8_t *a_out;
    uint64_t *a_ret;
    uint32_t *a_out_len, *a_bail_count, *a_bail_list;
    uint32_t a_nb, a_wrap;
};
static_assert(sizeof(FlatLds) % 16 == 0, "the image behind FlatLds starts 16-byte aligned");

template <int V>
__global__ __launch_bounds__(64 * FL_WAVES) __attribute__((amdgpu_waves_per_eu(DG_FL_WPE))) void j2t_flat_kernel(
    Params P, FlatParams S)
{
    __shared__ __attribute__((aligned(16))) FlatLds L;
    extern __shared__ __attribute__((aligned(16))) uint64_t s_fdesc[];
    FLP_DECL
    FLF_DECL
    const uint32_t tid = threadIdx.x, lane = tid & 63, wave = tid >> 6;
    const uint64_t b0 = (uint64_t)blockIdx.x * FL_MPB;
    const uint64_t b1 = b0 + FL_MPB < P.n ? b0 + FL_MPB : P.n;
    const uint32_t nb = (uint32_t)(b1 - b0);
    constexpr uint32_t NT = 64 * FL_WAVES;
    static_assert(FL_WAVES >= 4, "the prologue gives waves 0..3 a part each");

    const uint32_t blob16 = fli_blob16(S.hdr.total_len);
    const uint32_t ni = (blob16 + FLI_TABS) >> 4;
    const uint4 *gi = (const uint4 *)S.img;
    const uint4 i0 = gi[min(tid, ni - 1)], i1 = gi[min(tid + NT, ni - 1)];
    const uint64_t *po = (wave & 1) ? P.out_off : P.in_off;
    const uint64_t ov = po[b0 + min(lane, nb)];
    const uint64_t lo = P.in_off[b0], hi = P.in_off[b1], oend = P.out_off[b1];
    const uint64_t base = lo & ~15ull;
    const bool staged = hi - base <= (uint64_t)FL_STAGEW * 8;
    const uint32_t nw = staged ? (uint32_t)((hi - base + 15) >> 4) : 0u;
    static_assert(FL_STAGEW * 8 / 16 <= 4 * NT, "four 16-byte loads per thread cover the stage");
    const uint4 *gs = (const uint4 *)(P.json + base);
    const uint32_t l = nw ? nw - 1 : 0u;
    const uint4 v0 = gs[min(tid, l)], v1 = gs[min(tid + NT, l)], v2 = gs[min(tid + 2 * NT, l)],
                v3 = gs[min(tid + 3 * NT, l)];
    const uint64_t onx = __shfl_down(ov, 1);
    const uint64_t nx = lane == 63 ? ((wave & 1) ? oend : hi) : onx;
    if (tid == 0) {
        L.rounds = 0;
        L.ntask = 0;
        L.tgrab = 0;
        L.noremap = 0;
        L.a_out = P.out;
        L.a_ret = P.ret;
        L.a_out_len = P.out_len;
        L.a_bail_count = S.bail_count;
        L.a_bail_list = S.bail_list;
        L.a_nb = nb;
        L.a_wrap = S.wrap;
    }
    const uint32_t wv = (uint32_t)__builtin_amdgcn_readfirstlane((int)wave);
    if (wv == 0) {
        uint32_t ok = 0, n = 0, lw = 0, big = 0;
        const bool live = lane < nb;
        const uint64_t a = ov, n64 = live ? nx - a : 0;
        const bool tobig = live && P.big_list && (n64 > P.big_max || n64 > FL_MAXLEN);
        list_big_w(P, tobig, b0 + lane, n64);
        if (tobig) {
            big = 1;
        } else if (n64 > 0 && n64 <= FL_MAXLEN) {
            n = (uint32_t)n64;
            ok = 1;
            if (staged) lw = (uint32_t)(((a - base) >> 3) << 3) | (uint32_t)(a & 7);
            else lw = (lane * FL_SLOTW) << 3;
        }
        L.ok[lane] = ok;
        L.n[lane] = n;
        L.lw[lane] = lw;
        L.big[lane] = big;
        if (!staged) L.task[FL_FMAPW + lane] = a;
    } else if (wv == 1) {
        const bool live = lane < nb;
        L.oa[lane] = live ? ov : 0;
        L.cap[lane] = live ? (uint32_t)min(nx - ov, (uint64_t)0xFFFFFFFFu) : 0u;
    } else if (wv == 2) {
        L.plo[lane] = 0;
        L.phi[lane] = 0;
        L.oc[lane] = 0;
        L.nfq[lane] = 0;
        L.nesc[lane] = 0;
        L.fseen[lane] = 0;
    } else if (wv == 3) {
        for (uint32_t k = lane; k < FL_FMAPW; k += 64) L.task[k] = ~0ull;
    }
    {
        uint4 *ls = (uint4 *)L.in;
        if (tid < nw) ls[tid] = v0;
        if (tid + NT < nw) ls[tid + NT] = v1;
        if (tid + 2 * NT < nw) ls[tid + 2 * NT] = v2;
        if (tid + 3 * NT < nw) ls[tid + 3 * NT] = v3;
        uint4 *li = (uint4 *)s_fdesc;
        if (tid < ni) li[tid] = i0;
        if (tid + NT < ni) li[tid + NT] = i1;
        for (uint32_t k = tid + 2 * NT; k < ni; k += NT) li[k] = gi[k];
    }
    __syncthreads();
    const uint32_t g = tid & 3, m1 = tid >> 2;
    if (!staged) {
        if (tid < FL_G * FL_MPB && L.ok[m1]) {
            const uint64_t a = L.task[FL_FMAPW + m1];
            const uint32_t nw = (L.n[m1] + 7) >> 3, sh = (uint32_t)(a & 7) << 3;
            const glb_u64 *gsrc = (const glb_u64 *)(const void *)P.json + (a >> 3);
            constexpr uint32_t NWL = FL_MAXLEN / 8 / FL_G;
            uint64_t lo[NWL], hi[NWL];
#pragma unroll
            for (uint32_t j = 0; j < NWL; j++) {
                const uint32_t w = g + FL_G * j;
                lo[j] = gsrc[min(w, nw)];
                hi[j] = gsrc[min(w + 1, nw)];
            }
#pragma unroll
            for (uint32_t j = 0; j < NWL; j++) {
                const uint32_t w = g + FL_G * j;
                if (w < nw) L.in[(L.lw[m1] >> 3) + w] = sh ? (lo[j] >> sh) | (hi[j] << (64 - sh)) : lo[j];
            }
        }
        __syncthreads();
    }
    FLP(0);
#if defined(DG_FL_STOP) && DG_FL_STOP == 9
    return;
#endif
    const auto D = desc_view<3>((const __attribute__((address_space(3))) uint8_t *)(void *)s_fdesc, S.hdr);
    const __attribute__((address_space(3))) uint8_t *tabs =
        (const __attribute__((address_space(3))) uint8_t *)(void *)s_fdesc + blob16;
    const FastTabs tb{(const __attribute__((address_space(3))) uint64_t *)(tabs + FLI_P10U), (lds_f64 *)(tabs + FLI_P10D),
                      (const __attribute__((address_space(3))) uint64_t *)(tabs + FLI_PW)};
    const dg_type rt = ldrec(&D.T[S.wrap ? S.wrap_inner : P.root]);
    const dg_struct sd = ldrec(&D.S[rt.st]);
    const uint32_t nk = sd.name_mask + 1 <= FL_KEYS ? sd.name_mask + 1 : 0u;
    if (tid < nk) {
        const dg_name nm = ldrec(&D.N[sd.name_begin + tid]);
        uint32_t mt = 0xFF000000u;
        uint64_t w0 = 0, w1 = 0;
        if (nm.field != DG_NONE && nm.key_len <= 16) {
            const __attribute__((address_space(3))) uint64_t *pk = (decltype(&D.R[0]))(&D.P[nm.key_off]);
            w0 = nm.key_len ? pk[0] : 0ull;
            w1 = nm.key_len > 8 ? pk[1] : 0ull;
            mt = nm.field | (nm.key_len << 24);
        }
        L.km[tid] = mt;
        L.kw[2 * tid] = w0;
        L.kw[2 * tid + 1] = w1;
    }
    if (tid >= 64 && tid < 64 + FL_SLOTS) {
        const uint32_t j = tid - 64;
        uint32_t len = 0xFF;
        if (j < sd.n_fields) {
            const dg_field f = ldrec(&D.F[sd.field_begin + j]);
            if (f.flags & DG_FF_ALIAS_SELF) len = f.key_len;
        }
        L.fkm[j] = len;
    }
    if (S.wrap) {
        if (tid < FL_MPB) {
            uint32_t wid = 0;
            if (L.ok[tid]) {
                const uint32_t n = L.n[tid], lwa = L.lw[tid];
                LSrc src;
                src.init((const __attribute__((address_space(3))) uint64_t *)(void *)&L.in[lwa >> 3], (int32_t)(lwa & 7),
                         (int32_t)n);
                uint32_t p = skip_ws(src, 0);
                bool ok = p < n && src.raw((int32_t)p) == '{';
                p = ok ? skip_ws(src, p + 1) : p;
                ok = ok && p < n && src.raw((int32_t)p) == '"';
                const uint32_t k0 = p + 1;
                uint32_t q = k0;
                while (ok && q < n && src.raw((int32_t)q) != '"') {
                    if (src.raw((int32_t)q) == '\\') ok = false;
                    q++;
                }
                ok = ok && q < n;
                const uint32_t kn = q - k0;
                p = ok ? skip_ws(src, q + 1) : p;
                ok = ok && p < n && src.raw((int32_t)p) == ':';
                p = ok ? skip_ws(src, p + 1) : p;
                ok = ok && p < n && src.raw((int32_t)p) == '{';
                uint32_t e = n;
                while (ok && e > p && isspace_(src.raw((int32_t)(e - 1)))) e--;
                ok = ok && e > p + 1 && src.raw((int32_t)(e - 1)) == '}';
                uint32_t ic = e - 1;
                while (ok && ic > p && isspace_(src.raw((int32_t)(ic - 1)))) ic--;
                ok = ok && ic > p + 1 && src.raw((int32_t)(ic - 1)) == '}';
                if (ok) {
                    const dg_struct rs = ldrec(&D.S[ldrec(&D.T[P.root]).st]);
                    const int32_t fi = fl_lookup(D, rs, src, k0, kn);
                    const uint32_t k = (uint32_t)fi - rs.field_begin;
                    ok = fi >= 0 && k < 64 && ((S.wrap_ok >> k) & 1);
                    if (ok) {
                        wid = 0x10000u | ldrec(&D.F[fi]).id;
                        L.lw[tid] = lwa + p;
                        L.n[tid] = ic - p;
                        L.oa[tid] += 3;
                        L.cap[tid] = L.cap[tid] > 4 ? L.cap[tid] - 4 : 0u;
                    }
                }
                if (!ok) L.ok[tid] = 0;
            }
            L.wid[tid] = wid;
        }
        __syncthreads();
    }

    if (tid < FL_G * FL_MPB) {
        const bool on = L.ok[m1] != 0;
        const uint32_t n = L.n[m1], lwa = L.lw[m1], a7 = lwa & 7, lw = lwa >> 3;
        const int32_t nv0 = on ? (int32_t)n - 64 * (int32_t)g : 0;
        const uint32_t nv = nv0 <= 0 ? 0u : nv0 >= 64 ? 64u : (uint32_t)nv0;
        const uint64_t vmask = nv >= 64 ? ~0ull : (1ull << nv) - 1;
        uint32_t d[18];
#pragma unroll
        for (uint32_t j = 0; j < 9; j++) {
            const uint64_t w = L.in[lw + 8 * g + j];
            d[2 * j] = (uint32_t)w;
            d[2 * j + 1] = (uint32_t)(w >> 32);
        }
        const bool hi4 = a7 >= 4;
        const uint32_t sh = a7 & 3;
        uint32_t x[16];
#pragma unroll
        for (uint32_t i = 0; i < 16; i++) {
            const uint32_t lo_ = hi4 ? d[i + 1] : d[i], hi_ = hi4 ? d[i + 2] : d[i + 1];
            x[i] = __builtin_amdgcn_alignbyte(hi_, lo_, sh);
        }
        auto pack8 = [](uint32_t m0, uint32_t m1_) -> uint32_t {
            return (((m0 >> 7) | (m1_ >> 3)) * 0x01020408u) >> 24;
        };
        uint32_t ql = 0, qh = 0, cl = 0, ch = 0, kl = 0, kh = 0, anybs = 0;
#pragma unroll
        for (uint32_t j = 0; j < 8; j++) {
            const uint32_t x0 = x[2 * j], x1 = x[2 * j + 1];
            const uint32_t q8 = pack8(eq32(x0, 0x22222222u), eq32(x1, 0x22222222u));
            const uint32_t c8 = pack8(eq32(x0, 0x2C2C2C2Cu), eq32(x1, 0x2C2C2C2Cu));
            const uint32_t k8 = pack8(eq32(x0, 0x3A3A3A3Au), eq32(x1, 0x3A3A3A3Au));
            anybs |= eq32(x0, 0x5C5C5C5Cu) | eq32(x1, 0x5C5C5C5Cu);
            if (j < 4) {
                ql |= q8 << (8 * j);
                cl |= c8 << (8 * j);
                kl |= k8 << (8 * j);
            } else {
                qh |= q8 << (8 * (j - 4));
                ch |= c8 << (8 * (j - 4));
                kh |= k8 << (8 * (j - 4));
            }
        }
        uint64_t Q = ((uint64_t)qh << 32 | ql) & vmask, C = ((uint64_t)ch << 32 | cl) & vmask,
                 K = ((uint64_t)kh << 32 | kl) & vmask;
        const uint32_t nq = (uint32_t)__builtin_popcountll(Q);
        const uint32_t qx = g4_incl_sum(nq, g) - nq;
        uint64_t S = Q;
        S ^= S << 1;
        S ^= S << 2;
        S ^= S << 4;
        S ^= S << 8;
        S ^= S << 16;
        S ^= S << 32;
        if (qx & 1) S = ~S;
        C &= ~S;
        K &= ~S;
        const uint32_t nc = (uint32_t)__builtin_popcountll(C), nk = (uint32_t)__builtin_popcountll(K);
        const uint32_t pk = nc | (nk << 10) | (nq << 20);
        const uint32_t pin = g4_incl_sum(pk, g);
        const uint32_t ptot = g4_sum(pk);
        const uint32_t hasbs = g4_sum((anybs & 0x80808080u) && nv ? 1u : 0u);
        FLP(1);
        uint32_t bad = 0;
        if (hasbs) {
            uint32_t bl = 0, bh = 0;
#pragma unroll
            for (uint32_t j = 0; j < 8; j++) {
                const uint32_t b8 = pack8(eq32(x[2 * j], 0x5C5C5C5Cu), eq32(x[2 * j + 1], 0x5C5C5C5Cu));
                if (j < 4) bl |= b8 << (8 * j);
                else bh |= b8 << (8 * (j - 4));
            }
            const uint64_t B = ((uint64_t)bh << 32 | bl) & vmask, QB = Q | B;
            const uint32_t nxt = g4_next((uint32_t)(QB & 1), g);
            const uint64_t bb = B & ((QB >> 1) | ((uint64_t)nxt << 63));
            uint32_t ebad = 0;
            if (on && !bb && B) {
                LSrc es;
                es.init((const __attribute__((address_space(3))) uint64_t *)(void *)&L.in[lw], (int32_t)a7, (int32_t)n);
                for (uint64_t eb = B; eb; eb &= eb - 1) {
                    const uint32_t p = 64 * g + (uint32_t)__builtin_ctzll(eb);
                    const uint32_t x = fl_escape(p, es.get8((int32_t)p));
                    const uint32_t idx = atomicAdd(&L.nesc[m1], 1u);
                    if (!x || p + esc_in(x) > n) ebad = 1;
                    else if (idx < FL_NESC) L.esc[m1 * FL_NESC + idx] = x;
                    else ebad = 1;
                }
            }
            bad = g4_sum((bb ? 1u : 0u) | ebad);
        }
        if (on) {
            uint32_t ci = (pin & 0x3FF) - nc, ki = ((pin >> 10) & 0x3FF) - nk;
            const uint32_t pos0 = 64 * g;
            uint64_t c = C, k = K;
            while (c) {
                const uint32_t bit = (uint32_t)__builtin_ctzll(c);
                c &= c - 1;
                if (ci < FL_MAXF)
                    L.sep[ci * FL_MPB + m1] =
                        (pos0 + bit) | ((qx + (uint32_t)__builtin_popcountll(Q & ((1ull << bit) - 1))) << 16);
                ci++;
            }
            while (k) {
                const uint32_t bit = (uint32_t)__builtin_ctzll(k);
                k &= k - 1;
                if (ki < FL_MAXF) L.col[ki * FL_MPB + m1] = (uint16_t)(pos0 + bit);
                ki++;
            }
        }
        FLP(2);
        if (g == 0 && on) {
            LSrc src;
            src.init((const __attribute__((address_space(3))) uint64_t *)(void *)&L.in[lw], (int32_t)a7, (int32_t)n);
            const uint32_t open = skip_ws(src, 0);
            uint32_t close = n - 1;
            while (close > open && isspace_(src.raw((int32_t)close))) close--;
            const uint32_t nsep = ptot & 0x3FF, ncol = (ptot >> 10) & 0x3FF, qtot = ptot >> 20;
            bool ok = !bad && open < close && src.raw((int32_t)open) == '{' && src.raw((int32_t)close) == '}' &&
                      !(qtot & 1) && nsep + 1 < FL_MAXF;
            uint32_t nf = nsep + 1;
            if (ok && nsep == 0 && ncol == 0 && skip_ws(src, open + 1) == close) nf = 0;
            ok = ok && ncol == nf;
            L.ok[m1] = ok ? 1u : 0u;
            L.oc[m1] = open | (close << 16);
            L.nfq[m1] = nf | (qtot << 8) | (hasbs ? 1u << 31 : 0u);
            if (ok) atomicMax(&L.rounds, (nf + FL_SLOTS - 1) / FL_SLOTS);
        }
    }
    __syncthreads();
    FLP(3);
#if defined(DG_FL_STOP) && DG_FL_STOP == 1
    return;
#endif

    {
        const uint32_t mm = lane;
#ifndef DG_FL_ROT
#define DG_FL_ROT 1
#endif
        const uint32_t fwave = DG_FL_ROT ? (wave + blockIdx.x) % FL_WAVES : wave;
        const uint32_t ok0 = L.ok[mm], lwa = L.lw[mm], oc = L.oc[mm], nfq = L.nfq[mm];
        const uint32_t nf = nfq & 0xFF, qtot = (nfq >> 8) & 0x3FF;
        const bool hasbs = (nfq >> 31) != 0;
        const uint32_t cap = L.cap[mm];
        gu8 *const slot = (gu8 *)(void *)(L.a_out + L.oa[mm]);
        LSrc src;
        src.init((const __attribute__((address_space(3))) uint64_t *)(void *)&L.in[lwa >> 3], (int32_t)(lwa & 7), (int32_t)L.n[mm]);
        const uint32_t rounds = L.rounds;
        uint32_t nbytes = 0;
        lds_esc *E = (lds_esc *)(void *)&L.esc[mm * FL_NESC];
        const __attribute__((address_space(3))) uint64_t *KW = (const __attribute__((address_space(3))) uint64_t *)(void *)L.kw;
        const __attribute__((address_space(3))) uint32_t *KM = (const __attribute__((address_space(3))) uint32_t *)(void *)L.km;
        const uint32_t ne = min(L.nesc[mm], FL_NESC);
#ifdef DG_FLPROF_G
        uint64_t flg[8] = {0, 0, 0, 0, 0, 0, 0, __builtin_amdgcn_s_memtime()};
#endif
        auto parse = [&](uint32_t k, FField &F) {
            F.size = 0;
            F.kind = FV_NONE;
            if (ok0 && k < nf) {
                const uint32_t e0 = k ? L.sep[(k - 1) * FL_MPB + mm] : 0;
                const uint32_t sk = k ? (e0 & 0xFFFF) + 1 : (oc & 0xFFFF) + 1, q0 = e0 >> 16;
                uint32_t ek = oc >> 16, q1 = qtot;
                if (k + 1 < nf) {
                    const uint32_t e1 = L.sep[k * FL_MPB + mm];
                    ek = e1 & 0xFFFF;
                    q1 = e1 >> 16;
                }
                const uint32_t ck = L.col[k * FL_MPB + mm];
                FLG(0);
                if (!(ck >= sk && ck < ek && fl_field(D, sd, src, sk, ck, ek, q1 - q0, hasbs, E, ne, KW, KM, nk, k, P.flag, tb, F FLG_PASS))) {
                    L.ok[mm] = 0;
                    F.size = 0;
                    F.kind = FV_NONE;
                } else if (F.fi >= 0) {
                    const uint32_t bit = (uint32_t)F.fi - sd.field_begin;
                    atomicOr(&L.plo[mm], bit < 32 ? 1u << (bit & 31) : 0u);
                    atomicOr(&L.phi[mm], bit >= 32 ? 1u << (bit & 31) : 0u);
                }
                FLG(5);
            }
        };
        auto write = [&](const FField &F, uint32_t off) -> uint32_t {
            if (!F.size) return 1;
            if (off + F.size >= cap) return 0;
            WOut o;
            o.init(slot + off);
#ifdef DG_FL_ABL_NOSTORE
            o.dry = true;
#endif
            const uint32_t wr = flat_write(src, F, tb, o, E, ne);
            o.finish();
            return wr;
        };
        uint8_t *fmap = (uint8_t *)(void *)L.task;
        bool remap_try = DG_FL_REMAP && rounds == 1 && sd.n_fields <= FL_SLOTS && nk != 0;
        if (remap_try) {
            uint32_t mis = 0;
#pragma unroll
            for (uint32_t h = 0; h < FL_FPW; h++) {
                const uint32_t k = fl_slot(fwave, h);
                if (ok0 && k < nf) {
                    const uint32_t sk = k ? (L.sep[(k - 1) * FL_MPB + mm] & 0xFFFF) + 1 : (oc & 0xFFFF) + 1;
                    const uint32_t ck = L.col[k * FL_MPB + mm];
                    mis |= (k >= sd.n_fields || L.fkm[k] != ck - sk - 2) ? 1u : 0u;
                }
            }
            if (ballot(mis != 0) && lane == 0) atomicOr(&L.noremap, 2u);
            __syncthreads();
            remap_try = (L.noremap & 2u) != 0;
        }
        if (remap_try) {
            uint32_t fail = 0;
#pragma unroll
            for (uint32_t h = 0; h < FL_FPW; h++) {
                const uint32_t k = fl_slot(fwave, h);
                if (ok0 && k < nf) {
                    const uint32_t e0 = k ? L.sep[(k - 1) * FL_MPB + mm] : 0;
                    const uint32_t sk = k ? (e0 & 0xFFFF) + 1 : (oc & 0xFFFF) + 1, q0 = e0 >> 16;
                    uint32_t ek = oc >> 16, q1 = qtot;
                    if (k + 1 < nf) {
                        const uint32_t e1 = L.sep[k * FL_MPB + mm];
                        ek = e1 & 0xFFFF;
                        q1 = e1 >> 16;
                    }
                    const uint32_t ck = L.col[k * FL_MPB + mm];
                    FField G;
                    G.fi = -1;
                    if (!(ck >= sk && ck < ek &&
                          fl_field<true>(D, sd, src, sk, ck, ek, q1 - q0, hasbs, E, ne, KW, KM, nk, k, P.flag, tb, G FLG_PASS)) ||
                        G.fi < 0) {
                        fail = 1;
                    } else {
                        const uint32_t j = (uint32_t)G.fi - sd.field_begin;
                        if (atomicOr(&L.fseen[mm], 1u << j) & (1u << j)) fail = 1;
                        else fmap[j * FL_MPB + mm] = (uint8_t)k;
                    }
                }
            }
            if (ballot(fail != 0) && lane == 0) atomicOr(&L.noremap, 1u);
            __syncthreads();
        }
        const bool remap = remap_try && (L.noremap & 1u) == 0;
        for (uint32_t r = 0; r < rounds; r++) {
            FField F[FL_FPW];
            uint32_t kslot[FL_FPW];
            uint16_t *sz = &L.size[(r & 1) * FL_SLOTS * FL_MPB];
#pragma unroll
            for (uint32_t h = 0; h < FL_FPW; h++) {
                FLF_T0();
                const uint32_t j = fl_slot(fwave, h);
                const uint32_t k = remap ? (uint32_t)fmap[j * FL_MPB + mm] : r * FL_SLOTS + j;
                const uint32_t si = remap ? k : j;
                kslot[h] = si;
                parse(k, F[h]);
                if (si < FL_SLOTS) sz[si * FL_MPB + mm] = (uint16_t)F[h].size;
                if (remap && j >= nf) sz[j * FL_MPB + mm] = 0;
                FLF_ADD(r * FL_SLOTS + fl_slot(fwave, h));
            }
            FLP(4);
            __syncthreads();
            FLP(5);
#if defined(DG_FL_STOP) && DG_FL_STOP == 2
            continue;
#endif
            uint32_t off[FL_FPW], tot = 0;
#pragma unroll
            for (uint32_t h = 0; h < FL_FPW; h++) off[h] = nbytes;
#pragma unroll
            for (uint32_t f = 0; f < FL_SLOTS; f++) {
                const uint32_t v = sz[f * FL_MPB + mm];
#pragma unroll
                for (uint32_t h = 0; h < FL_FPW; h++) off[h] += f < kslot[h] ? v : 0u;
                tot += v;
            }
            nbytes += tot;
            uint32_t nch[FL_FPW], nsum = 0, good = 1;
#pragma unroll
            for (uint32_t h = 0; h < FL_FPW; h++) {
                const FField &G = F[h];
                const bool body = G.kind == FV_BIN || ((G.kind == FV_STR || G.kind == FV_NUMSTR) && !G.esc);
                nch[h] = body && G.nb > FL_INLINE && off[h] + G.size < cap ? (G.nb + FL_CHUNK - 1) / FL_CHUNK : 0u;
                nsum += nch[h];
            }
            {
                const uint32_t incl = wave_incl_sum(nsum, lane);
                const uint32_t wtot = (uint32_t)__builtin_amdgcn_readlane((int)incl, 63);
                if (wtot) {
                    uint32_t tb0 = 0;
                    if (lane == 63) tb0 = atomicAdd(&L.ntask, wtot);
                    tb0 = (uint32_t)__builtin_amdgcn_readlane((int)tb0, 63);
                    uint32_t t0 = tb0 + incl - nsum;
                    if (nsum && t0 + nsum <= FL_MAXTASK) {
#pragma unroll
                        for (uint32_t h = 0; h < FL_FPW; h++) {
                            const bool b64 = F[h].kind == FV_BIN;
                            for (uint32_t c = 0; c < nch[h]; c++) {
                                const uint32_t cs = c * FL_CHUNK, cn = min(FL_CHUNK, F[h].nb - cs);
                                const uint32_t dst = off[h] + 7 + (b64 ? c * (FL_CHUNK / 4 * 3) : cs);
                                L.task[t0 + c] = (uint64_t)mm | ((uint64_t)b64 << 6) |
                                                 ((uint64_t)(c + 1 == nch[h]) << 7) | ((uint64_t)(F[h].s0 + cs) << 8) |
                                                 ((uint64_t)cn << 20) | ((uint64_t)dst << 32);
                            }
                            t0 += nch[h];
                        }
                    } else if (nsum) {
                        good = 0;
                        for (uint32_t c = t0; c < t0 + nsum && c < FL_MAXTASK; c++) L.task[c] = ~0ull;
                    }
                }
            }
            if (r + 1 == rounds) __syncthreads();
#pragma unroll
            for (uint32_t h = 0; h < FL_FPW; h++) {
                FLF_T0();
                const uint32_t wr = write(F[h], off[h]);
                FLF_ADD(6 + r * FL_SLOTS + fl_slot(fwave, h));
                good &= wr != 0;
            }
            if (!good) L.ok[mm] = 0;
            FLP(6);
        }
        if (wave == 0) L.nbytes[mm] = nbytes;
#ifdef DG_FLPROF_G
        if (lane == 0 && (blockIdx.x & 31) == 0)
            for (int k_ = 0; k_ < 6; k_++) atomicAdd(&P.stats[2 + k_], (unsigned long long)flg[k_]);
#endif
    }
    FLP(6);
    {
        const uint32_t nt = min(L.ntask, FL_MAXTASK);
        for (;;) {
            uint32_t t0 = 0;
            if (lane == 0) t0 = atomicAdd(&L.tgrab, 64u);
            t0 = (uint32_t)__builtin_amdgcn_readfirstlane((int)t0);
            if (t0 >= nt) break;
            const uint32_t t = t0 + lane;
            const uint64_t tk = t < nt ? L.task[t] : ~0ull;
            if (tk == ~0ull) continue;
            const uint32_t m = (uint32_t)tk & 63, s0 = (uint32_t)(tk >> 8) & 0xFFF, cn = (uint32_t)(tk >> 20) & 0xFFF;
            const uint32_t lwa = L.lw[m];
            LSrc src;
            src.init((const __attribute__((address_space(3))) uint64_t *)(void *)&L.in[lwa >> 3], (int32_t)(lwa & 7), (int32_t)L.n[m]);
            WOut o;
            o.init((gu8 *)(void *)(L.a_out + L.oa[m] + (uint32_t)(tk >> 32)));
#ifdef DG_FL_ABL_NOSTORE
            o.dry = true;
#endif
            bool cok = true;
            if ((tk >> 6) & 1) cok = body_b64(src, s0, cn, ((tk >> 7) & 1) != 0, o);
            else body_copy(src, s0, cn, o);
            o.finish();
            if (!cok) L.ok[m] = 0;
        }
    }
    __syncthreads();
    FLP(7);

    if (tid < FL_MPB) {
        const uint32_t m = tid;
        const uint64_t i = (uint64_t)blockIdx.x * FL_MPB + m;
        if (m < L.a_nb) {
            const uint32_t len = L.nbytes[m] + 1;
            const uint32_t wid = L.a_wrap ? L.wid[m] : 0u;
            bool good = L.ok[m] && len <= L.cap[m];
            if (good) {
                const uint64_t present = (uint64_t)L.plo[m] | ((uint64_t)L.phi[m] << 32);
                uint64_t bits = D.R[sd.req_begin] & ~present;
                const uint64_t flag = P.flag;
                while (bits) {
                    const uint32_t kk = (uint32_t)__builtin_ctzll(bits);
                    bits &= bits - 1;
                    const dg_field f = ldrec(&D.F[sd.field_begin + kk]);
                    if (f.flags & DG_FF_REQUEST_BASE) continue;
                    if (f.required == DG_REQ_REQUIRED || ((flag & DG_F_WRITE_DEFAULT) && f.required == DG_REQ_DEFAULT) ||
                        ((flag & DG_F_WRITE_OPTIONAL) && f.required == DG_REQ_OPTIONAL)) {
                        good = false;
                        break;
                    }
                }
            }
            if (good && wid) {
                gu8 *o = (gu8 *)(void *)L.a_out + L.oa[m];
                o[-3] = DG_T_STRUCT;
                o[-2] = (uint8_t)(wid >> 8);
                o[-1] = (uint8_t)wid;
                o[len - 1] = 0;
                o[len] = 0;
                L.a_ret[i] = 0;
                L.a_out_len[i] = len + 4;
            } else if (good) {
                ((gu8 *)(void *)L.a_out)[L.oa[m] + len - 1] = 0;
                L.a_ret[i] = 0;
                L.a_out_len[i] = len;
            } else if (!L.big[m]) {
                const uint32_t qq = atomicAdd(L.a_bail_count, 1u);
                L.a_bail_list[qq] = (uint32_t)i;
            }
        }
    }
    FLP_END();
    FLF_END();
}

void launch_flat_kernel(dim3 grid, hipStream_t s, const Params &P, const FlatParams &S);
void flat_image_build(const uint8_t *blob, uint32_t total_len, uint8_t *img);

}
```

### dynamicgo_amd/csrc/j2t_host.hip

```cpp
#include <hip/hip_runtime.h>

#include <stdarg.h>
#include <stdio.h>
#include <stdlib.h>
#include <string.h>

#include <algorithm>
#include <mutex>
#include <vector>

#include "j2t_flat.h"
#include "host_internal.h"

using namespace dg;

static thread_local char g_err[512];
int set_err(int code, const char *fmt, ...)
{
    va_list ap;
    va_start(ap, fmt);
    vsnprintf(g_err, sizeof g_err, fmt, ap);
    va_end(ap);
    return code;
}

static const uint64_t FAST_WS_STRIDE = DCAP + WS_KEYCAP + (uint64_t)WS_REQCAP * 8;
static const uint64_t DEEP_WS_STRIDE = DCAP + DEEP_KEYCAP + (uint64_t)DEEP_REQCAP * 8 +
                                       (uint64_t)MAX_RECURSE * sizeof(Frame) + MAX_RECURSE / 8;

static int scratch_new(dg_ctx *c, hipStream_t owner, std::unique_ptr<Scratch> &out)
{
    std::unique_ptr<Scratch> x(new Scratch());
    x->owner = owner;
    int rc = x->counts.alloc(DG_NCOUNTS);
    if (!rc) HIPCHK(hipMemsetAsync(x->counts, 0, DG_NCOUNTS * 4, owner));
    if (!rc) rc = x->ws_deep.alloc(DEEP_WS_STRIDE * DEEP_THREADS);
    if (!rc) rc = x->ws_wave.alloc((size_t)c->n_cu * std::max(WV_BLOCKS_PER_CU, WV5_BLOCKS_PER_CU) * WV_WAVES * DCAP);
    if (!rc) rc = x->sums.alloc((size_t)c->n_cu);
    if (!rc) rc = x->d_frame.alloc(FRAME_CAP);
    if (rc) return rc;
    x->t2j_cnt.set[0] = x->counts + CNT_T2J_A;
    x->t2j_cnt.set[1] = x->counts + CNT_T2J_B;
    x->t2j_cnt.bytes = 16;
    out = std::move(x);
    return DG_OK;
}

void dg_i_scratch_release(dg_ctx *c, const hipStream_t *s, int n)
{
    if (!c || n <= 0) return;
    Entry g(c, true);
    (void)hipDeviceSynchronize();
    for (auto &x : c->scratch) {
        x->forget(s, n);
        if (std::find(s, s + n, x->owner) == s + n) continue;
        x->last = nullptr;
        x.reset();
    }
    c->scratch.erase(std::remove(c->scratch.begin(), c->scratch.end(), nullptr), c->scratch.end());
    c->rr = 0;
    c->t2j_deep.forget(s, n);
    c->t2j_tok.forget(s, n);
    c->tget.forget(s, n);
}

int scratch_for(dg_ctx *c, hipStream_t s, Scratch **out)
{
    Scratch *x = nullptr;
    for (auto &y : c->scratch)
        if (y->owner == s) x = y.get();
    if (!x) {
        if ((int)c->scratch.size() < DG_MAX_SCRATCH) {
            std::unique_ptr<Scratch> nx;
            int rc = scratch_new(c, s, nx);
            if (rc) return rc;
            c->scratch.push_back(std::move(nx));
            x = c->scratch.back().get();
        } else {
            x = c->scratch[c->rr++ % c->scratch.size()].get();
        }
    }
    HIPCHK(x->acquire(s));
    *out = x;
    return DG_OK;
}

#ifndef DG_SRC_HASH
#define DG_SRC_HASH "unknown"
#endif
static const char g_build_info[] = "dgj2t-build:" DG_SRC_HASH " arch:gfx950";

static int64_t *knob_ref(dg_ctx *c, const char *name)
{
    Knobs &K = c->knobs;
    if (!strcmp(name, "flat")) return &K.flat;
    if (!strcmp(name, "wave_min")) return &K.wave_min;
    if (!strcmp(name, "wave_occ")) return &K.wave_occ;
    if (!strcmp(name, "small_mpw")) return &K.small_mpw;
    if (!strcmp(name, "list_blocks")) return &K.list_blocks;
    if (!strcmp(name, "t2j_spread")) return &K.t2j_spread;
    if (!strcmp(name, "t2j_wave_min")) return &K.t2j_wave_min;
    if (!strcmp(name, "t2j_overlap")) return &K.t2j_overlap;
    if (!strcmp(name, "flat_wrap")) return &K.flat_wrap;
    if (!strcmp(name, "tget_spread")) return &K.tget_spread;
    if (!strcmp(name, "cut_wave_min")) return &K.cut_wave_min;
    if (!strcmp(name, "edit_wave_min")) return &K.edit_wave_min;
    if (!strcmp(name, "edit_reuse_rec")) return &K.edit_reuse_rec;
    if (!strcmp(name, "edit_lanes")) return &K.edit_lanes;
    if (!strcmp(name, "kids_wide_min")) return &K.kids_wide_min;
    if (!strcmp(name, "kids_no_scan")) return &K.kids_no_scan;
    if (!strcmp(name, "cols_full_search")) return &K.cols_full_search;
    return nullptr;
}

extern "C" {

const char *dg_last_error(void) { return g_err; }

const char *dg_build_info(void) { return g_build_info; }

int dg_ctx_create(int device, dg_ctx **out)
{
    if (!out) return set_err(DG_E_INVALID, "null out");
    int ndev = 0;
    HIPCHK(hipGetDeviceCount(&ndev));
    if (device < 0 || device >= ndev) return set_err(DG_E_INVALID, "device %d out of range (%d)", device, ndev);
    HIPCHK(hipSetDevice(device));
    std::unique_ptr<dg_ctx> c(new dg_ctx());
    c->device = device;
    HIPCHK(c->stream.create(hipStreamDefault));
    int rc;
    if ((rc = c->d_pending.alloc(4)) || (rc = c->d_zero.alloc(2))) return rc;
    HIPCHK(hipMemset(c->d_zero, 0, 16));
    if ((rc = c->d_stats.alloc(16))) return rc;
    HIPCHK(hipMemset(c->d_stats, 0, 16 * 8));
    HIPCHK(hipDeviceSynchronize());
    HIPCHK(hipDeviceGetAttribute(&c->n_cu, hipDeviceAttributeMultiprocessorCount, device));
    static const struct { const char *env; const char *name; } envk[] = {
        {"DG_FLAT", "flat"}, {"DG_WAVE_MIN", "wave_min"}, {"DG_WAVE_OCC", "wave_occ"},
        {"DG_SMALL_MPW", "small_mpw"}, {"DG_LIST_BLOCKS", "list_blocks"}, {"DG_T2J_SPREAD", "t2j_spread"},
        {"DG_T2J_WAVE_MIN", "t2j_wave_min"}, {"DG_T2J_OVERLAP", "t2j_overlap"}, {"DG_FLAT_WRAP", "flat_wrap"},
        {"DG_TGET_SPREAD", "tget_spread"}, {"DG_CUT_WAVE_MIN", "cut_wave_min"},
        {"DG_EDIT_WAVE_MIN", "edit_wave_min"}, {"DG_EDIT_LANES", "edit_lanes"},
        {"DG_KIDS_WIDE_MIN", "kids_wide_min"}};
    for (const auto &e : envk) {
        const char *v = getenv(e.env);
        if (v && *v) *knob_ref(c.get(), e.name) = strtoll(v, nullptr, 10);
    }
    *out = c.release();
    return DG_OK;
}

int dg_ctx_set_knob(dg_ctx *c, const char *name, int64_t value)
{
    if (!c || !name) return set_err(DG_E_INVALID, "null ctx/name");
    std::lock_guard<std::mutex> g(c->mu);
    int64_t *k = knob_ref(c, name);
    if (!k) return set_err(DG_E_INVALID, "unknown knob '%s'", name);
    *k = value;
    return DG_OK;
}

int dg_ctx_get_knob(dg_ctx *c, const char *name, int64_t *value)
{
    if (!c || !name || !value) return set_err(DG_E_INVALID, "bad args");
    std::lock_guard<std::mutex> g(c->mu);
    int64_t *k = knob_ref(c, name);
    if (!k) return set_err(DG_E_INVALID, "unknown knob '%s'", name);
    *value = *k;
    return DG_OK;
}

void dg_ctx_destroy(dg_ctx *c) { delete c; }

void *dg_ctx_stream(dg_ctx *c) { return c ? (void *)(hipStream_t)c->stream : nullptr; }

static int desc_finish(dg_ctx *c, const dg_desc_hdr &h, DevArr<uint8_t> &d_blob, size_t len, const void *host_blob,
                       dg_desc **out)
{
    if (h.magic != DG_DESC_MAGIC || h.version < 1 || h.version > DG_DESC_VERSION || h.total_len > len)
        return set_err(DG_E_DESC, "bad descriptor blob header");
    DevArr<uint8_t> d_flat;
    if (h.version >= 2 && h.total_len <= FL_DESC) {
        std::vector<uint8_t> img(fli_len(h.total_len));
        flat_image_build((const uint8_t *)host_blob, h.total_len, img.data());
        if (int rc = d_flat.alloc(img.size())) return rc;
        HIPCHK(hipMemcpy(d_flat, img.data(), img.size(), hipMemcpyHostToDevice));
    }
    dg_desc *d = new dg_desc();
    d->ctx = c;
    d->d_blob = std::move(d_blob);
    d->d_flat = std::move(d_flat);
    d->len = len;
    d->hdr = h;
    d->hblob.assign((const uint8_t *)host_blob, (const uint8_t *)host_blob + h.total_len);
    *out = d;
    return DG_OK;
}

static bool flat_root(const dg_desc *d, uint32_t root, uint64_t flags)
{
    const dg_desc_hdr &h = d->hdr;
    if (d->hblob.size() < h.total_len || h.version < 2 || h.total_len > FL_DESC || root >= h.n_types) return false;
    const uint8_t *b = d->hblob.data();
    const dg_type *T = (const dg_type *)(b + h.off_types);
    if (T[root].ttype != DG_T_STRUCT) return false;
    const dg_struct &sd = ((const dg_struct *)(b + h.off_structs))[T[root].st];
    if (sd.req_words != 1 || ((flags & DG_F_ENABLE_HM) && (sd.flags & DG_SF_HTTP_MAPPING))) return false;
    const dg_field *F = (const dg_field *)(b + h.off_fields);
    for (uint32_t k = 0; k < sd.n_fields; k++) {
        switch (T[F[sd.field_begin + k].type].ttype) {
        case DG_T_BOOL: case DG_T_BYTE: case DG_T_I16: case DG_T_I32: case DG_T_I64: case DG_T_DOUBLE: case DG_T_STRING:
            break;
        default:
            return false;
        }
    }
    return true;
}

static uint64_t wrap_root(const dg_desc *d, uint32_t root, uint64_t flags, uint32_t *inner)
{
    const dg_desc_hdr &h = d->hdr;
    if (d->hblob.size() < h.total_len || h.version < 2 || h.total_len > FL_DESC || root >= h.n_types) return 0;
    const uint8_t *b = d->hblob.data();
    const dg_type *T = (const dg_type *)(b + h.off_types);
    if (T[root].ttype != DG_T_STRUCT) return 0;
    const dg_struct &rs = ((const dg_struct *)(b + h.off_structs))[T[root].st];
    if (rs.req_words != 1 || rs.n_fields > 64 || ((flags & DG_F_ENABLE_HM) && (rs.flags & DG_SF_HTTP_MAPPING))) return 0;
    const dg_field *F = (const dg_field *)(b + h.off_fields);
    const uint64_t req = ((const uint64_t *)(b + h.off_reqwords))[rs.req_begin];
    uint32_t w = DG_NONE;
    for (uint32_t k = 0; k < rs.n_fields && w == DG_NONE; k++) {
        const uint32_t t = F[rs.field_begin + k].type;
        if (T[t].ttype == DG_T_STRUCT && flat_root(d, t, flags)) w = t;
    }
    if (w == DG_NONE) return 0;
    uint64_t ok = 0;
    for (uint32_t k = 0; k < rs.n_fields; k++) {
        const dg_field &f = F[rs.field_begin + k];
        if (f.type != w || ((flags & DG_F_ENABLE_VM) && f.vm != DG_VM_NONE) ||
            ((f.flags & DG_FF_REQUEST_BASE) && (flags & DG_F_NO_WRITE_BASE)))
            continue;
        bool fine = true;
        for (uint32_t j = 0; j < rs.n_fields && fine; j++) {
            if (j == k || !((req >> j) & 1)) continue;
            const dg_field &g = F[rs.field_begin + j];
            if (g.flags & DG_FF_REQUEST_BASE) continue;
            if ((flags & DG_F_TRACE_BACK) || g.required == DG_REQ_REQUIRED ||
                ((flags & DG_F_WRITE_DEFAULT) && g.required == DG_REQ_DEFAULT) ||
                ((flags & DG_F_WRITE_OPTIONAL) && g.required == DG_REQ_OPTIONAL))
                fine = false;
        }
        if (fine) ok |= 1ull << k;
    }
    *inner = w;
    return ok;
}

int dg_desc_create(dg_ctx *c, const void *blob, size_t len, dg_desc **out)
{
    if (!c || !blob || !out || len < sizeof(dg_desc_hdr)) return set_err(DG_E_INVALID, "bad args");
    dg_desc_hdr h;
    memcpy(&h, blob, sizeof h);
    if (h.magic != DG_DESC_MAGIC || h.total_len > len) return set_err(DG_E_DESC, "bad descriptor blob");
    HIPCHK(hipSetDevice(c->device));
    DevArr<uint8_t> d_blob;
    if (int rc = d_blob.alloc(len)) return rc;
    HIPCHK(hipMemcpy(d_blob, blob, len, hipMemcpyHostToDevice));
    return desc_finish(c, h, d_blob, len, blob, out);
}

int dg_desc_create_device(dg_ctx *c, const void *d_src, size_t len, dg_desc **out)
{
    if (!c || !d_src || !out || len < sizeof(dg_desc_hdr)) return set_err(DG_E_INVALID, "bad args");
    HIPCHK(hipSetDevice(c->device));
    DevArr<uint8_t> d_blob;
    if (int rc = d_blob.alloc(len)) return rc;
    HIPCHK(hipMemcpy(d_blob, d_src, len, hipMemcpyDeviceToDevice));
    std::vector<uint8_t> hb(len);
    HIPCHK(hipMemcpy(hb.data(), d_blob, len, hipMemcpyDeviceToHost));
    dg_desc_hdr h;
    memcpy(&h, hb.data(), sizeof h);
    if (h.total_len > len) return set_err(DG_E_DESC, "bad descriptor blob");
    return desc_finish(c, h, d_blob, len, hb.data(), out);
}

void dg_desc_destroy(dg_desc *d) { delete d; }

uint32_t dg_desc_root(const dg_desc *d) { return d ? d->hdr.root_type : 0; }

int dg_ctx_stats(dg_ctx *c, uint64_t *bails, uint64_t *deeps, int reset)
{
    Entry g(c, c, nullptr, "null ctx");
    if (g.rc) return g.rc;
    HIPCHK(hipDeviceSynchronize());
    unsigned long long h[2];
    HIPCHK(hipMemcpy(h, c->d_stats, sizeof h, hipMemcpyDeviceToHost));
    if (bails) *bails = h[0];
    if (deeps) *deeps = h[1];
    if (reset) {
        HIPCHK(hipMemset(c->d_stats, 0, sizeof h));
        HIPCHK(hipDeviceSynchronize());
    }
    return DG_OK;
}

int dg_ctx_counters(dg_ctx *c, uint64_t *out, int n, int reset)
{
    Entry g(c, c && out && n >= 0 && n <= 16);
    if (g.rc) return g.rc;
    HIPCHK(hipDeviceSynchronize());
    HIPCHK(hipMemcpy(out, c->d_stats, (size_t)n * 8, hipMemcpyDeviceToHost));
    if (reset) {
        HIPCHK(hipMemset(c->d_stats, 0, 16 * 8));
        HIPCHK(hipDeviceSynchronize());
    }
    return DG_OK;
}

uint64_t dg_slot_bound(uint64_t len) { return (4 * len + 64 + 127) & ~127ull; }

static int ensure_fast_ws(Scratch *x, uint64_t lanes)
{
    if (x->ws_fast_lanes >= lanes) return DG_OK;
    HIPCHK(x->wait_host());
    x->ws_fast.reset();
    x->deep_list.reset();
    x->ws_fast_lanes = 0;
    const uint64_t want = std::max<uint64_t>(lanes, 1 << 16);
    int rc;
    if ((rc = x->ws_fast.alloc(want * FAST_WS_STRIDE)) || (rc = x->deep_list.alloc(want))) return rc;
    x->ws_fast_lanes = want;
    return DG_OK;
}

static int enqueue(dg_ctx *c, Scratch *x, const dg_desc *d, uint32_t root, const BatchArgs &b, hipStream_t s)
{
    const uint64_t n = b.n, max_len = b.max_len;
    int rc = ensure_fast_ws(x, n);
    if (rc) return rc;
    uint64_t flags = b.flags;
    const bool no_wave = (flags & DG_F_NO_WAVE_PATH) != 0;
    const Knobs &K = c->knobs;
    const bool use_flat = K.flat >= 0 ? K.flat != 0
                                      : (flags & DG_F_FLAT_PATH) != 0 ||
                                            (!(flags & DG_F_NO_FLAT_PATH) && (max_len == 0 || max_len <= FL_MAXLEN));
    const bool no_flat = (flags & DG_F_NO_FLAT_PATH) != 0 || K.flat == 0;
    auto mark = [&](int i) {
        if (c->kt) (void)hipEventRecord(c->kt[i], s);
    };
    flags &= ~(DG_F_NO_WAVE_PATH | DG_F_FLAT_PATH | DG_F_NO_FLAT_PATH);
    uint32_t *const cnt = x->counts;
    Params P;
    P.root = root;
    P.json = b.src;
    P.in_off = b.in_off;
    P.n = n;
    P.flag = flags;
    P.list = nullptr;
    P.list_count = nullptr;
    P.reset2 = nullptr;
    P.big_list = nullptr;
    P.big_count = nullptr;
    P.big_max = 0;
    P.huge_count = nullptr;
    P.huge_min = WV_HUGE_MIN;
    P.hm_tab = b.hm.tab;
    P.hm_bytes = b.hm.bytes;
    P.n_hm = b.hm.n_hm;
    P.ans_tab = b.hm.vm;
    P.out = b.out;
    P.out_off = b.out_off;
    P.out_len = b.out_len;
    P.ret = b.ret;
    P.pending = b.pending;
    P.deep_count = cnt + CNT_DEEP;
    P.deep_list = x->deep_list;
    P.ws = x->ws_fast;
    P.ws_stride = FAST_WS_STRIDE;
    P.keycap = WS_KEYCAP;
    P.reqcap = WS_REQCAP;
    P.fast = d->hdr.version >= 2 && (flags & ~FAST_FLAGS) == 0;
    P.stats = c->d_stats;
    const uint64_t blocks = (n + LANE_BLOCK - 1) / LANE_BLOCK;
    DeepParams DP;
    DP.ws = x->ws_deep;
    DP.ws_stride = DEEP_WS_STRIDE;
    DP.keycap = DEEP_KEYCAP;
    DP.reqcap = DEEP_REQCAP;
    DP.done = cnt + CNT_DEEP_DONE;
    DP.blob = d->d_blob;
    DP.hdr = d->hdr;
    const uint64_t big_max = (uint64_t)K.wave_min;
    const bool may_be_long = max_len == 0 || max_len > big_max;
    const bool wave = P.fast && !no_wave && d->hdr.total_len <= WV_DESC && d->hdr.total_len <= DESC_LDS_BYTES &&
                      may_be_long;
    auto lane_launch = [&](uint64_t grid, const Params &Q) {
        if (d->hdr.total_len <= DESC_LDS_BYTES) launch_lane_kernel_lds(dim3((uint32_t)grid), s, Q, DP);
        else launch_lane_kernel_glb(dim3((uint32_t)grid), s, Q, DP);
    };
    const int mpw = (int)K.small_mpw;
    const bool small = P.fast && !no_wave && mpw > 0 && d->hdr.total_len <= SM_DESC;
    if (!small && !wave) {
        mark(0);
        lane_launch(blocks, P);
        mark(1);
        mark(2);
        mark(3);
        HIPCHK(hipGetLastError());
        return DG_OK;
    }
    if ((rc = x->grow(x->bail_list, n))) return rc;
    if ((rc = x->grow(x->big_list, n))) return rc;
    const bool wave_stage = small ? may_be_long : true;
    Params P1 = P;
    if (wave_stage) {
        P1.big_list = x->big_list;
        P1.big_count = cnt + CNT_BIG;
        P1.big_max = big_max;
        P1.huge_count = cnt + CNT_HUGE;
    }
    uint32_t inner = DG_NONE;
    const uint64_t wrap_ok = (small && K.flat_wrap != 0 && !no_flat && !flat_root(d, root, flags))
                                 ? wrap_root(d, root, flags, &inner)
                                 : 0;
    mark(0);
    if (!small) {
        lane_launch(blocks, P1);
    } else if ((use_flat && flat_root(d, root, flags)) || wrap_ok) {
        FlatParams FP;
        FP.img = d->d_flat;
        FP.hdr = d->hdr;
        FP.bail_count = cnt + CNT_BAIL;
        FP.bail_list = x->bail_list;
        FP.wrap = wrap_ok ? 1u : 0u;
        FP.wrap_inner = wrap_ok ? inner : 0u;
        FP.wrap_ok = wrap_ok;
        launch_flat_kernel(dim3((uint32_t)((n + FL_MPB - 1) / FL_MPB)), s, P1, FP);
    } else {
        SmallParams S;
        S.blob = d->d_blob;
        S.hdr = d->hdr;
        S.bail_count = cnt + CNT_BAIL;
        S.bail_list = x->bail_list;
        const uint64_t mpb = (uint64_t)SM_WAVES * (uint64_t)(mpw >= 64 ? 64 : mpw == 16 ? 16 : 32);
        launch_small_kernel(mpw, dim3((uint32_t)((n + mpb - 1) / mpb)), s, P1, S);
    }
    HIPCHK(hipGetLastError());
    mark(1);
    if (wave_stage) {
        WaveParams W;
        W.blob = d->d_blob;
        W.hdr = d->hdr;
        W.bail_count = cnt + CNT_BAIL;
        W.bail_list = x->bail_list;
        W.list = x->big_list;
        W.list_count = cnt + CNT_BIG;
        W.huge_count = cnt + CNT_HUGE;
        W.list_cap = n;
        W.ws = x->ws_wave;
        W.queue = cnt + CNT_WAVEQ;
        const bool wave5 = K.wave_occ == 5;
        const uint64_t bpc = wave5 ? WV5_BLOCKS_PER_CU : WV_BLOCKS_PER_CU;
        const dim3 wgrid((uint32_t)std::min<uint64_t>((n + WV_WAVES - 1) / WV_WAVES, (uint64_t)c->n_cu * bpc));
        if (wave5) launch_wave_kernel5(wgrid, s, P, W);
        else launch_wave_kernel(wgrid, s, P, W);
        HIPCHK(hipGetLastError());
    }
    mark(2);
    Params P3 = P;
    P3.list = x->bail_list;
    P3.list_count = cnt + CNT_BAIL;
    P3.reset2 = cnt + CNT_BIG;
    if (!small) P3.fast = 0;
    const uint64_t cap = small ? (uint64_t)std::max<int64_t>(1, K.list_blocks) : 32;
    lane_launch(std::min<uint64_t>(blocks, cap), P3);
    mark(3);
    HIPCHK(hipGetLastError());
    return DG_OK;
}

static int launch(dg_ctx *c, const dg_desc *d, uint32_t root, const BatchArgs &b, hipStream_t s)
{
    if (b.n == 0) return DG_OK;
    if (root >= d->hdr.n_types) return set_err(DG_E_INVALID, "root type %u out of range", root);
    Scratch *x;
    int rc = scratch_for(c, s, &x);
    if (rc) return rc;
    rc = enqueue(c, x, d, root, b, s);
    if (rc) (void)hipMemsetAsync(x->counts, 0, DG_J2T_COUNTS_BYTES, s);
    HIPCHK(x->publish(s));
    return rc;
}

int dg_j2t_batch_device(dg_ctx *c, const dg_desc *d, uint32_t root, const uint8_t *d_json, const uint64_t *d_in_off,
                        uint64_t n, uint64_t flags, uint8_t *d_out, const uint64_t *d_out_off, uint32_t *d_out_len,
                        uint64_t *d_ret, uint32_t *d_pending, void *stream)
{
    Entry g(c, c && d, stream, "null ctx/desc");
    if (g.rc) return g.rc;
    const BatchArgs b{d_json, d_in_off, n, flags, d_out, d_out_off, d_out_len, d_ret, d_pending};
    return launch(c, d, root, b, g.s);
}

int dg_j2t_batch_device_ml(dg_ctx *c, const dg_desc *d, uint32_t root, const uint8_t *d_json, const uint64_t *d_in_off,
                           uint64_t n, uint64_t flags, uint8_t *d_out, const uint64_t *d_out_off, uint32_t *d_out_len,
                           uint64_t *d_ret, uint32_t *d_pending, void *stream, uint64_t max_len)
{
    Entry g(c, c && d, stream, "null ctx/desc");
    if (g.rc) return g.rc;
    const BatchArgs b{d_json, d_in_off, n, flags, d_out, d_out_off, d_out_len, d_ret, d_pending, max_len};
    return launch(c, d, root, b, g.s);
}

int dg_j2t_batch_device_hm(dg_ctx *c, const dg_desc *d, uint32_t root, const uint8_t *d_json, const uint64_t *d_in_off,
                           uint64_t n, uint64_t flags, const dg_hm_entry *d_hm_tab, uint32_t n_hm,
                           const uint8_t *d_hm_bytes, uint8_t *d_out, const uint64_t *d_out_off, uint32_t *d_out_len,
                           uint64_t *d_ret, uint32_t *d_pending, void *stream, uint64_t max_len)
{
    Entry g(c, c && d && !(d_hm_tab && n_hm && !d_hm_bytes), stream);
    if (g.rc) return g.rc;
    BatchArgs b{d_json, d_in_off, n, flags, d_out, d_out_off, d_out_len, d_ret, d_pending, max_len};
    if (d_hm_tab) b.hm = HMIn{d_hm_tab, n_hm, d_hm_bytes};
    return launch(c, d, root, b, g.s);
}

int dg_j2t_batch_device_cb(dg_ctx *c, const dg_desc *d, uint32_t root, const uint8_t *d_json, const uint64_t *d_in_off,
                           uint64_t n, uint64_t flags, const dg_cb_tables *cb, uint8_t *d_out, const uint64_t *d_out_off,
                           uint32_t *d_out_len, uint64_t *d_ret, uint32_t *d_pending, void *stream, uint64_t max_len)
{
    Entry g(c, c && d && !(cb && (cb->hm_tab || cb->ans_tab) && !cb->bytes), stream);
    if (g.rc) return g.rc;
    BatchArgs b{d_json, d_in_off, n, flags, d_out, d_out_off, d_out_len, d_ret, d_pending, max_len};
    if (cb) b.hm = HMIn{cb->hm_tab, cb->n_hm, cb->bytes, cb->ans_tab};
    return launch(c, d, root, b, g.s);
}

int dg_j2t_batch_device_iters(dg_ctx *c, const dg_desc *d, uint32_t root, const uint8_t *d_json,
                              const uint64_t *d_in_off, uint64_t n, uint64_t flags, uint8_t *d_out,
                              const uint64_t *d_out_off, uint32_t *d_out_len, uint64_t *d_ret, uint32_t *d_pending,
                              void *stream, uint64_t max_len, int iters)
{
    Entry g(c, c && d && iters >= 0, stream);
    if (g.rc) return g.rc;
    const BatchArgs b{d_json, d_in_off, n, flags, d_out, d_out_off, d_out_len, d_ret, d_pending, max_len};
    for (int k = 0; k < iters; k++)
        if (int rc = launch(c, d, root, b, g.s)) return rc;
    return DG_OK;
}

int dg_j2t_batch_device_ktime(dg_ctx *c, const dg_desc *d, uint32_t root, const uint8_t *d_json,
                              const uint64_t *d_in_off, uint64_t n, uint64_t flags, uint8_t *d_out,
                              const uint64_t *d_out_off, uint32_t *d_out_len, uint64_t *d_ret, uint32_t *d_pending,
                              void *stream, uint64_t max_len, int iters, double *ms)
{
    Entry g(c, c && d && iters >= 1 && ms, stream);
    if (g.rc) return g.rc;
    const BatchArgs b{d_json, d_in_off, n, flags, d_out, d_out_off, d_out_len, d_ret, d_pending, max_len};
    std::vector<Event> ev((size_t)iters * 4);
    int rc = DG_OK;
    for (auto &e : ev)
        if (e.create(hipEventDisableSystemFence) != hipSuccess) rc = set_err(DG_E_HIP, "hipEventCreate");
    for (int k = 0; k < iters && !rc; k++) {
        c->kt = &ev[(size_t)k * 4];
        rc = launch(c, d, root, b, g.s);
    }
    c->kt = nullptr;
    ms[0] = ms[1] = ms[2] = 0;
    if (!rc && hipStreamSynchronize(g.s) != hipSuccess) rc = set_err(DG_E_HIP, "hipStreamSynchronize");
    for (int k = 0; k < iters && !rc; k++)
        for (int i = 0; i < 3; i++) {
            float t = 0;
            if (hipEventElapsedTime(&t, ev[(size_t)k * 4 + i], ev[(size_t)k * 4 + i + 1]) != hipSuccess)
                rc = set_err(DG_E_HIP, "hipEventElapsedTime");
            ms[i] += t / iters;
        }
    return rc;
}

int dg_j2t_batch_device_inflight(dg_ctx *c, const dg_desc *d, uint32_t root, const uint8_t *d_json,
                                 const uint64_t *d_in_off, uint64_t n, uint64_t flags, const uint64_t *d_out_off,
                                 const dg_out_set *sets, int depth, void *stream, uint64_t max_len, int iters)
{
    Entry g(c, c && d && sets && depth >= 1 && depth <= 8 && iters >= 0, stream);
    if (g.rc) return g.rc;
    const hipStream_t s0 = g.s;
    const unsigned order_only = hipEventDisableTiming | hipEventDisableSystemFence;
    const int used = std::min(depth, std::max(iters, 1));
    while ((int)c->side.size() < used - 1) {
        Stream x;
        Event e;
        HIPCHK(x.create(hipStreamNonBlocking));
        HIPCHK(e.create(order_only));
        c->side.push_back(std::move(x));
        c->side_ev.push_back(std::move(e));
    }
    if (!c->fork_ev) HIPCHK(c->fork_ev.create(order_only));
    if (used > 1) {
        HIPCHK(hipEventRecord(c->fork_ev, s0));
        for (int j = 0; j < used - 1; j++) HIPCHK(hipStreamWaitEvent(c->side[j], c->fork_ev, 0));
    }
    int rc = DG_OK;
    for (int k = 0; k < iters && !rc; k++) {
        const int j = k % used;
        const dg_out_set &o = sets[j];
        const BatchArgs b{d_json, d_in_off, n, flags, o.d_out, d_out_off, o.d_out_len, o.d_ret, o.d_pending, max_len};
        rc = launch(c, d, root, b, j ? (hipStream_t)c->side[j - 1] : s0);
    }
    for (int j = 0; j < used - 1; j++) {
        HIPCHK(hipEventRecord(c->side_ev[j], c->side[j]));
        HIPCHK(hipStreamWaitEvent(s0, c->side_ev[j], 0));
    }
    return rc;
}

struct FrameIn {
    const uint8_t *hdr, *ftr;
    uint32_t hdr_len, ftr_len;
};

static int pack_scan_nolock(dg_ctx *c, hipStream_t s, const BatchArgs &b, const FrameIn *f, uint8_t *d_dst,
                            uint64_t *d_dst_off, const PackChain &ch = PackChain());

static const uint64_t HOST_ONE_TRIP = 4ull << 20;

static int batch_host(dg_ctx *c, const dg_desc *d, uint32_t root, const BatchArgs &in, uint64_t hm_len,
                      const HostOut &o)
{
    const uint8_t *const json = in.src;
    const uint64_t *const in_off = in.in_off, n = in.n;
    uint8_t *const out = o.out;
    uint64_t *const out_off = o.out_off, *const ret = in.ret;
    const HMIn *const hm = in.hm.tab || in.hm.vm ? &in.hm : nullptr;
    Entry g(c, c && d && (json || !n) && in_off && out_off && (ret || !n));
    if (g.rc) return g.rc;
    int rc;
    const hipStream_t s = g.s;
    const uint64_t base = in_off[0], bytes = in_off[n] - in_off[0];
    const uint64_t nhm = hm && hm->tab ? hm->n_hm : 0;
    const uint64_t nvm = hm && hm->vm ? 1 : 0;
    const uint64_t hmb = hm ? (hm_len + 7) & ~7ull : 0;
    const uint64_t hmw = hm ? 2 * n * nhm + n * nvm + hmb / 8 : 0;
    const uint64_t up_bytes = 16 * (n + 1) + 8 * hmw + bytes + 64;
    if ((rc = c->h_up.grow(up_bytes))) return rc;
    uint64_t *ioff = (uint64_t *)(void *)c->h_up, *soff = ioff + n + 1;
    uint64_t *hhm = soff + n + 1;
    uint8_t *hj = (uint8_t *)(void *)(hhm + hmw);
    if (hm) {
        if (n * nhm) memcpy(hhm, hm->tab, 16 * n * nhm);
        if (n * nvm) memcpy(hhm + 2 * n * nhm, hm->vm, 8 * n);
        if (hm_len) memcpy(hhm + 2 * n * nhm + n * nvm, hm->bytes, hm_len);
    }
    uint64_t max_len = 1;
    soff[0] = 0;
    for (uint64_t i = 0; i <= n; i++) ioff[i] = in_off[i] - base;
    for (uint64_t i = 0; i < n; i++) {
        const uint64_t l = ioff[i + 1] - ioff[i];
        max_len = std::max<uint64_t>(max_len, l);
        soff[i + 1] = soff[i] + dg_slot_bound(l);
    }
    if (bytes) memcpy(hj, json + base, bytes);
    memset(hj + bytes, 0, 64);
    const uint64_t slots = soff[n];
    const uint64_t head = 8 * n + ((4 * n + 7) & ~7ull);
    const bool one_trip = slots <= HOST_ONE_TRIP;
    if ((rc = c->d_json.grow(up_bytes))) return rc;
    if ((rc = c->d_out.grow(slots + 64))) return rc;
    if ((rc = c->d_pack.grow(head + slots + 64))) return rc;
    if ((rc = c->d_pack_off.grow(n + 1))) return rc;
    if ((rc = c->h_down.grow(one_trip ? head + slots + 64 : head + 8))) return rc;
    const uint64_t *d_in = (const uint64_t *)(void *)c->d_json, *d_oo = d_in + n + 1;
    BatchArgs b;
    if (hm) {
        b.hm.n_hm = (uint32_t)nhm;
        b.hm.tab = nhm ? (const dg_hm_entry *)(const void *)(d_oo + n + 1) : nullptr;
        b.hm.vm = nvm ? (const dg_cb_entry *)(const void *)(d_oo + n + 1 + 2 * n * nhm) : nullptr;
        b.hm.bytes = (const uint8_t *)(const void *)(d_oo + n + 1 + 2 * n * nhm + n * nvm);
    }
    const uint8_t *d_j = c->d_json + 16 * (n + 1) + 8 * hmw;
    uint64_t *d_ret = (uint64_t *)(void *)c->d_pack;
    uint32_t *d_ol = (uint32_t *)(void *)(c->d_pack + 8 * n);
    uint8_t *d_packed = c->d_pack + head;
    HIPCHK(hipMemcpyAsync(c->d_json, c->h_up, up_bytes, hipMemcpyHostToDevice, s));
    b.src = d_j, b.in_off = d_in, b.n = n, b.flags = in.flags, b.max_len = max_len;
    b.out = c->d_out, b.out_off = d_oo, b.out_len = d_ol, b.ret = d_ret;
    if ((rc = launch(c, d, root, b, s))) return rc;
    if ((rc = pack_scan_nolock(c, s, b, nullptr, d_packed, c->d_pack_off))) return rc;
    HIPCHK(hipMemcpyAsync(c->h_down, c->d_pack, one_trip ? head + slots : head, hipMemcpyDeviceToHost, s));
    HIPCHK(hipStreamSynchronize(s));
    const uint64_t *hret = (const uint64_t *)(void *)c->h_down;
    const uint32_t *hol = (const uint32_t *)(void *)(c->h_down + 8 * n);
    std::vector<uint32_t> olen(hol, hol + n);
    memcpy(ret, hret, n * 8);
    auto kept = [&](uint64_t i) {
        return ret[i] == 0 || (uint8_t)ret[i] == DG_ST_HM_END || (uint8_t)ret[i] == 24  ||
               (uint8_t)ret[i] == DG_ST_HM_END_AT || (uint8_t)ret[i] == DG_ST_CB_LIST;
    };
    uint64_t packed = 0;
    for (uint64_t i = 0; i < n; i++)
        if (kept(i)) packed += olen[i];
    std::vector<uint64_t> redo;
    for (uint64_t i = 0; i < n; i++)
        if ((uint8_t)ret[i] == DG_ST_OUT_OVERFLOW) redo.push_back(i);
    std::vector<uint8_t> main_buf, rdown;
    std::vector<uint64_t> redo_so;
    uint64_t rhead = 0;
    if (!redo.empty()) {
        const uint64_t m = redo.size();
        uint64_t rb = 0;
        for (uint64_t i : redo) rb += ioff[i + 1] - ioff[i];
        const uint64_t rhw = hm ? 2 * m * nhm + m * nvm + hmb / 8 : 0;
        std::vector<uint8_t> up(16 * (m + 1) + 8 * rhw + rb + 64, 0);
        HostBatch hb(c, s);
        uint64_t *io = (uint64_t *)(void *)up.data(), *so = io + m + 1, *rhm = so + m + 1;
        uint8_t *rj = (uint8_t *)(void *)(rhm + rhw);
        io[0] = so[0] = 0;
        if (hm && hm_len) memcpy(rhm + 2 * m * nhm + m * nvm, hm->bytes, hm_len);
        for (uint64_t k = 0; k < m; k++) {
            const uint64_t i = redo[k], l = ioff[i + 1] - ioff[i];
            if (hm && nhm) memcpy(rhm + 2 * k * nhm, hm->tab + i * nhm, 16 * nhm);
            if (hm && nvm) memcpy(rhm + 2 * m * nhm + k, hm->vm + i, 8);
            memcpy(rj + io[k], hj + ioff[i], l);
            io[k + 1] = io[k] + l;
            so[k + 1] = so[k] + (((uint64_t)olen[i] + 64 + 7) & ~7ull);
        }
        if (!one_trip) {
            main_buf.resize(packed);
            if (packed) HIPCHK(hipMemcpy(main_buf.data(), d_packed, packed, hipMemcpyDeviceToHost));
        }
        rhead = 8 * m + ((4 * m + 7) & ~7ull);
        if ((rc = c->d_json.grow(up.size()))) return rc;
        if ((rc = c->d_out.grow(so[m] + 64))) return rc;
        const uint64_t *r_in = (const uint64_t *)(void *)c->d_json, *r_oo = r_in + m + 1;
        uint64_t *r_ret = (uint64_t *)(void *)c->d_pack;
        uint32_t *r_ol = (uint32_t *)(void *)(c->d_pack + 8 * m);
        if ((rc = hb.copy(c->d_json, up.data(), up.size(), hipMemcpyHostToDevice))) return rc;
        if (hm)
            b.hm = HMIn{nhm ? (const dg_hm_entry *)(const void *)(r_oo + m + 1) : nullptr, (uint32_t)nhm,
                        (const uint8_t *)(const void *)(r_oo + m + 1 + 2 * m * nhm + m * nvm),
                        nvm ? (const dg_cb_entry *)(const void *)(r_oo + m + 1 + 2 * m * nhm) : nullptr};
        b.src = c->d_json + 16 * (m + 1) + 8 * rhw, b.in_off = r_in, b.n = m;
        b.out = c->d_out, b.out_off = r_oo, b.out_len = r_ol, b.ret = r_ret;
        if ((rc = launch(c, d, root, b, s))) return rc;
        rdown.resize(rhead + so[m]);
        if ((rc = hb.copy(rdown.data(), c->d_pack, rhead, hipMemcpyDeviceToHost)) ||
            (rc = hb.copy(rdown.data() + rhead, c->d_out, so[m], hipMemcpyDeviceToHost)) || (rc = hb.sync()))
            return rc;
        redo_so.assign(so, so + m + 1);
        for (uint64_t k = 0; k < m; k++) {
            const uint64_t i = redo[k];
            memcpy(&ret[i], rdown.data() + 8 * k, 8);
            memcpy(&olen[i], rdown.data() + 8 * m + 4 * k, 4);
            if ((uint8_t)ret[i] == DG_ST_OUT_OVERFLOW)
                return set_err(DG_E_NOMEM, "message %llu overflowed its exact-size slot", (unsigned long long)i);
        }
    }
    uint64_t total = 0;
    out_off[0] = 0;
    for (uint64_t i = 0; i < n; i++) {
        if (!kept(i)) olen[i] = 0;
        total += olen[i];
        out_off[i + 1] = total;
    }
    if (o.out_need) *o.out_need = total;
    if (total > o.out_cap || (!out && total)) return set_err(DG_E_NOMEM, "output needs %llu bytes", (unsigned long long)total);
    if (redo.empty()) {
        if (one_trip) {
            if (total) memcpy(out, c->h_down + head, total);
        } else if (total) {
            HIPCHK(hipMemcpy(out, d_packed, total, hipMemcpyDeviceToHost));
        }
        return DG_OK;
    }
    const uint8_t *mp = one_trip ? c->h_down + head : main_buf.data();
    uint64_t pp = 0;
    size_t rk = 0;
    for (uint64_t i = 0; i < n; i++) {
        if (rk < redo.size() && redo[rk] == i) {
            if (olen[i]) memcpy(out + out_off[i], rdown.data() + rhead + redo_so[rk], olen[i]);
            rk++;
        } else if (olen[i]) {
            memcpy(out + out_off[i], mp + pp, olen[i]);
            pp += olen[i];
        }
    }
    return DG_OK;
}

static BatchArgs host_batch(const uint8_t *json, const uint64_t *in_off, uint64_t n, uint64_t flags, uint64_t *ret)
{
    BatchArgs b;
    b.src = json, b.in_off = in_off, b.n = n, b.flags = flags, b.ret = ret;
    return b;
}

int dg_j2t_batch_host(dg_ctx *c, const dg_desc *d, uint32_t root, const uint8_t *json, const uint64_t *in_off,
                      uint64_t n, uint64_t flags, uint8_t *out, uint64_t out_cap, uint64_t *out_off, uint64_t *ret,
                      uint64_t *out_need)
{
    return batch_host(c, d, root, host_batch(json, in_off, n, flags, ret), 0, HostOut{out, out_cap, out_off, out_need});
}

int dg_j2t_batch_host_hm(dg_ctx *c, const dg_desc *d, uint32_t root, const uint8_t *json, const uint64_t *in_off,
                         uint64_t n, uint64_t flags, const dg_hm_entry *hm_tab, uint32_t n_hm, const uint8_t *hm_bytes,
                         uint64_t hm_len, uint8_t *out, uint64_t out_cap, uint64_t *out_off, uint64_t *ret,
                         uint64_t *out_need)
{
    if ((hm_tab && n_hm && n && !hm_tab) || (hm_len && !hm_bytes)) return set_err(DG_E_INVALID, "bad args");
    for (uint64_t k = 0; hm_tab && k < n * n_hm; k++)
        if (hm_tab[k].len != DG_HM_ERR && (uint64_t)hm_tab[k].off + hm_tab[k].len > hm_len)
            return set_err(DG_E_INVALID, "HTTP-mapping entry %llu outside the bytes", (unsigned long long)k);
    BatchArgs b = host_batch(json, in_off, n, flags, ret);
    if (hm_tab) b.hm = HMIn{hm_tab, n_hm, hm_bytes};
    return batch_host(c, d, root, b, hm_len, HostOut{out, out_cap, out_off, out_need});
}

int dg_j2t_batch_host_cb(dg_ctx *c, const dg_desc *d, uint32_t root, const uint8_t *json, const uint64_t *in_off,
                         uint64_t n, uint64_t flags, const dg_cb_tables *cb, uint8_t *out, uint64_t out_cap,
                         uint64_t *out_off, uint64_t *ret, uint64_t *out_need)
{
    BatchArgs b = host_batch(json, in_off, n, flags, ret);
    const HostOut o{out, out_cap, out_off, out_need};
    if (!cb) return batch_host(c, d, root, b, 0, o);
    if ((cb->len && !cb->bytes) || (cb->hm_tab && cb->n_hm && !n)) return set_err(DG_E_INVALID, "bad args");
    for (uint64_t k = 0; cb->hm_tab && k < n * cb->n_hm; k++)
        if (cb->hm_tab[k].len != DG_HM_ERR && (uint64_t)cb->hm_tab[k].off + cb->hm_tab[k].len > cb->len)
            return set_err(DG_E_INVALID, "HTTP-mapping entry %llu outside the bytes", (unsigned long long)k);
    for (uint64_t i = 0; cb->ans_tab && i < n; i++) {
        uint64_t at = cb->ans_tab[i].off;
        for (uint32_t k = 0; k < cb->ans_tab[i].count; k++) {
            if (at + 4 > cb->len) return set_err(DG_E_INVALID, "value-mapping entry %llu outside the bytes", (unsigned long long)i);
            uint32_t l;
            memcpy(&l, cb->bytes + at, 4);
            at += 4 + (uint64_t)l;
            if (at > cb->len) return set_err(DG_E_INVALID, "value-mapping entry %llu outside the bytes", (unsigned long long)i);
        }
    }
    if (cb->hm_tab || cb->ans_tab) b.hm = HMIn{cb->hm_tab, cb->hm_tab ? cb->n_hm : 0u, cb->bytes, cb->ans_tab};
    return batch_host(c, d, root, b, cb->len, o);
}

int dg_j2t_do(dg_ctx *c, const dg_desc *d, uint32_t root, const uint8_t *json, size_t len, uint64_t flags,
              uint8_t *out, size_t out_cap, size_t *out_len, uint64_t *ret)
{
    uint64_t in_off[2] = {0, len};
    uint64_t oo[2];
    uint64_t need = 0;
    static const uint8_t empty = 0;
    int rc = dg_j2t_batch_host(c, d, root, len ? json : &empty, in_off, 1, flags, out, out_cap, oo, ret, &need);
    if (out_len) *out_len = need;
    return rc;
}

int dg_pack_device(dg_ctx *c, const uint8_t *d_out, const uint64_t *d_out_off, const uint32_t *d_out_len, uint64_t n,
                   uint8_t *d_dst, const uint64_t *d_dst_off, void *stream)
{
    if (!c || (n && (!d_out || !d_out_off || !d_out_len || !d_dst || !d_dst_off))) return set_err(DG_E_INVALID, "bad args");
    if (n == 0) return DG_OK;
    HIPCHK(hipSetDevice(c->device));
    hipStream_t s = stream ? (hipStream_t)stream : (hipStream_t)c->stream;
    uint64_t blocks = std::min<uint64_t>((n + 3) / 4, (uint64_t)c->n_cu * 8);
    launch_pack_kernel(dim3((uint32_t)blocks), s, d_out, d_out_off, d_out_len, n, d_dst, d_dst_off);
    HIPCHK(hipGetLastError());
    return DG_OK;
}

static int pack_scan_nolock(dg_ctx *c, hipStream_t s, const BatchArgs &b, const FrameIn *f, uint8_t *d_dst,
                            uint64_t *d_dst_off, const PackChain &ch)
{
    if (b.n == 0) {
        if (ch.ovf_out) HIPCHK(hipMemsetAsync(ch.ovf_out, 0, 8, s));
        if (ch.base_in && !ch.base_mod16) HIPCHK(hipMemcpyAsync(d_dst_off, ch.base_in, 8, hipMemcpyDefault, s));
        else HIPCHK(hipMemsetAsync(d_dst_off, 0, 8, s));
        if (ch.cur_out) HIPCHK(hipMemcpyAsync(ch.cur_out, d_dst_off, 8, hipMemcpyDefault, s));
        return DG_OK;
    }
    Scratch *x;
    int rc = scratch_for(c, s, &x);
    if (rc) return rc;
    MsgFrame fr{};
    fr.ret = b.ret;
    fr.base_in = ch.base_in;
    fr.dst_cap = ch.dst_cap;
    fr.base_mod16 = ch.base_mod16 ? 1u : 0u;
    fr.phase_add = (uint32_t)(ch.base_mod16 >> 1) & 15;
    fr.ret_dst = ch.ret_dst;
    fr.cur_out = ch.cur_out;
    fr.ovf_out = b.ret ? ch.ovf_out : nullptr;
    if (f) {
        const uint32_t fo = (f->hdr_len + 7) & ~7u;
        std::vector<uint8_t> tmp(fo + f->ftr_len + 16, 0);
        memcpy(tmp.data(), f->hdr, f->hdr_len);
        if (f->ftr_len) memcpy(tmp.data() + fo, f->ftr, f->ftr_len);
        if (tmp != x->frame) {
            HIPCHK(x->wait_host());
            HIPCHK(hipMemcpy(x->d_frame, tmp.data(), tmp.size(), hipMemcpyHostToDevice));
            x->frame = tmp;
        }
        fr.hdr = x->d_frame;
        fr.hdr_len = f->hdr_len;
        fr.ftr = x->d_frame + fo;
        fr.ftr_len = f->ftr_len;
    }
    const uint64_t G = std::min<uint64_t>((b.n + 255) / 256, (uint64_t)c->n_cu);
    launch_pack_scan_kernel(dim3((uint32_t)G), s, b.out, b.out_off, b.out_len, b.n, d_dst, d_dst_off, x->sums,
                            x->counts + CNT_PACK, fr);
    hipError_t e = hipGetLastError();
    if (e != hipSuccess) (void)hipMemsetAsync(x->counts + CNT_PACK, 0, 8, s);
    HIPCHK(x->publish(s));
    if (e != hipSuccess) return set_err(DG_E_HIP, "pack scan launch: %s", hipGetErrorString(e));
    return DG_OK;
}

}

int dg_i_pack_scan(dg_ctx *c, hipStream_t s, const BatchArgs &b, uint8_t *d_dst, uint64_t *d_dst_off)
{
    return pack_scan_nolock(c, s, b, nullptr, d_dst, d_dst_off);
}

int dg_i_convert_pack(dg_ctx *c, const dg_desc *d, uint32_t root, const BatchArgs &b, uint8_t *packed,
                      uint64_t *pack_off, hipStream_t s, const PackChain &ch)
{
    Entry g(c, true);
    if (g.rc) return g.rc;
    int rc = launch(c, d, root, b, s);
    if (rc) return rc;
    if (ch.pack_after) HIPCHK(hipStreamWaitEvent(s, ch.pack_after, 0));
    return pack_scan_nolock(c, s, b, nullptr, packed, pack_off, ch);
}

extern "C" {

int dg_pack_device_scan(dg_ctx *c, const uint8_t *d_out, const uint64_t *d_out_off, const uint32_t *d_out_len,
                        uint64_t n, uint8_t *d_dst, uint64_t *d_dst_off, void *stream)
{
    Entry g(c, c && d_dst_off && !(n && (!d_out || !d_out_off || !d_out_len || !d_dst)), stream);
    if (g.rc) return g.rc;
    BatchArgs b;
    b.out = (uint8_t *)d_out, b.out_off = d_out_off, b.out_len = (uint32_t *)d_out_len, b.n = n;
    return pack_scan_nolock(c, g.s, b, nullptr, d_dst, d_dst_off);
}

int dg_pack_device_framed(dg_ctx *c, const uint8_t *d_out, const uint64_t *d_out_off, const uint32_t *d_out_len,
                          const uint64_t *d_ret, uint64_t n, const uint8_t *hdr, uint32_t hdr_len, const uint8_t *ftr,
                          uint32_t ftr_len, uint8_t *d_dst, uint64_t *d_dst_off, void *stream)
{
    Entry g(c, c && d_dst_off && hdr && (!ftr_len || ftr) && ((hdr_len + 7) & ~7u) + ftr_len + 16 <= FRAME_CAP &&
                   !(n && (!d_out || !d_out_off || !d_out_len || !d_ret || !d_dst)), stream);
    if (g.rc) return g.rc;
    BatchArgs b;
    b.out = (uint8_t *)d_out, b.out_off = d_out_off, b.out_len = (uint32_t *)d_out_len, b.ret = (uint64_t *)d_ret, b.n = n;
    const FrameIn f{hdr, ftr, hdr_len, ftr_len};
    return pack_scan_nolock(c, g.s, b, &f, d_dst, d_dst_off);
}

int dg_bench_device(dg_ctx *c, const dg_desc *d, uint32_t root, const uint8_t *d_json, const uint64_t *d_in_off,
                    uint64_t n, uint64_t flags, uint8_t *d_out, const uint64_t *d_out_off, uint32_t *d_out_len,
                    uint64_t *d_ret, int iters, float *ms)
{
    Entry g(c, c && d && iters >= 1 && ms);
    if (g.rc) return g.rc;
    Event e0, e1;
    HIPCHK(e0.create());
    HIPCHK(e1.create());
    HIPCHK(hipEventRecord(e0, g.s));
    const BatchArgs b{d_json, d_in_off, n, flags, d_out, d_out_off, d_out_len, d_ret, c->d_pending};
    for (int k = 0; k < iters; k++)
        if (int rc = launch(c, d, root, b, g.s)) return rc;
    HIPCHK(hipEventRecord(e1, g.s));
    HIPCHK(hipEventSynchronize(e1));
    HIPCHK(hipEventElapsedTime(ms, e0, e1));
    return DG_OK;
}

}
```

### dynamicgo_amd/csrc/j2t_kern_flat.hip

```cpp
#include "j2t_flat.h"

namespace dg {
void launch_flat_kernel(dim3 grid, hipStream_t s, const Params &P, const FlatParams &S)
{
    const uint32_t shmem = fli_len(S.hdr.total_len);
    hipLaunchKernelGGL(j2t_flat_kernel<0>, grid, dim3(64 * FL_WAVES), shmem, s, P, S);
}
}
```

Before: 459.1 GB/s.

## Precompute per-struct field plans in LDS and add typed register number parsing

```diff
diff --git a/dynamicgo_amd/csrc/flat_image.h b/dynamicgo_amd/csrc/flat_image.h
--- a/dynamicgo_amd/csrc/flat_image.h
+++ b/dynamicgo_amd/csrc/flat_image.h
@@ -1,6 +1,8 @@
 #pragma once
 #include <stdint.h>
 #include <string.h>
+
+#include "../../include/dgj2t_desc.h"
 
 namespace dg {
 
@@ -30,4 +32,152 @@
     for (int k = 0; k < FLI_WN; k++) memcpy(t + FLI_PW + 8 * k, &pw_hi[FLI_WLO + 348 + k][1], 8);
 }
 
+constexpr uint32_t FLP_SLOTS = 8;
+constexpr uint32_t FLP_KEYS = 32;
+constexpr uint32_t FLP_NOPLAN = 0xFFFFFFFFu;
+
+struct flp_hdr {
+    uint32_t field_begin, n_fields, req_begin, name_begin, name_mask;
+    uint32_t nk;
+    uint32_t len;
+    uint32_t _pad;
+};
+struct flp_rec {
+    uint64_t k0, k1;
+    uint16_t key_len;
+    uint16_t id;
+    uint16_t vm;
+    uint8_t ttype;
+    uint8_t bin;
+    uint8_t flags;
+    uint8_t pred;
+    int8_t required;
+    uint8_t _pad[5];
+};
+static_assert(sizeof(flp_hdr) == 32 && sizeof(flp_rec) == 32, "plan records");
+
+constexpr uint32_t flp_len(uint32_t n_fields, uint32_t nk)
+{
+    return ((uint32_t)sizeof(flp_hdr) + 32 * n_fields + 16 * nk + 4 * nk + 4 * FLP_SLOTS + 15) & ~15u;
 }
+
+namespace flp_detail {
+template <class T>
+inline T rd(const uint8_t *p)
+{
+    T v;
+    memcpy(&v, p, sizeof v);
+    return v;
+}
+inline bool header(const uint8_t *blob, uint32_t total_len, dg_desc_hdr &h)
+{
+    if (total_len < sizeof h) return false;
+    h = rd<dg_desc_hdr>(blob);
+    auto in = [&](uint32_t off, uint64_t n, uint32_t sz) { return off % 8 == 0 && off <= total_len && n * sz <= total_len - off; };
+    return h.version >= 2 && h.total_len <= total_len && in(h.off_types, h.n_types, sizeof(dg_type)) &&
+           in(h.off_structs, h.n_structs, sizeof(dg_struct)) && in(h.off_fields, h.n_fields, sizeof(dg_field)) &&
+           in(h.off_names, h.n_names, sizeof(dg_name)) && in(h.off_reqwords, h.n_reqwords, 8) && in(h.off_pool, h.pool_len, 1);
+}
+}
+
+inline bool flp_flat(const uint8_t *blob, const dg_desc_hdr &h, uint32_t s)
+{
+    using namespace flp_detail;
+    if (s >= h.n_structs) return false;
+    const dg_struct sd = rd<dg_struct>(blob + h.off_structs + sizeof(dg_struct) * s);
+    if (sd.req_words != 1 || sd.n_fields > 64 || sd.req_begin >= h.n_reqwords) return false;
+    if (sd.field_begin > h.n_fields || sd.n_fields > h.n_fields - sd.field_begin) return false;
+    if (sd.name_begin > h.n_names || sd.name_mask >= h.n_names - sd.name_begin) return false;
+    for (uint32_t k = 0; k < sd.n_fields; k++) {
+        const dg_field f = rd<dg_field>(blob + h.off_fields + sizeof(dg_field) * (sd.field_begin + k));
+        if (f.type >= h.n_types || f.key_off % 8 || f.key_off > h.pool_len) return false;
+        if (((uint32_t)f.key_len + 7) / 8 * 8 > h.pool_len - f.key_off) return false;
+        switch (rd<dg_type>(blob + h.off_types + sizeof(dg_type) * f.type).ttype) {
+        case DG_T_BOOL: case DG_T_BYTE: case DG_T_I16: case DG_T_I32: case DG_T_I64: case DG_T_DOUBLE: case DG_T_STRING:
+            break;
+        default:
+            return false;
+        }
+    }
+    return true;
+}
+
+inline uint32_t flp_total(const uint8_t *blob, uint32_t total_len)
+{
+    using namespace flp_detail;
+    dg_desc_hdr h;
+    if (!header(blob, total_len, h)) return 0;
+    uint32_t n = 0;
+    for (uint32_t s = 0; s < h.n_structs; s++) {
+        if (!flp_flat(blob, h, s)) continue;
+        const dg_struct sd = rd<dg_struct>(blob + h.off_structs + sizeof(dg_struct) * s);
+        n += flp_len(sd.n_fields, sd.name_mask + 1 <= FLP_KEYS ? sd.name_mask + 1 : 0u);
+    }
+    return n;
+}
+
+inline void flp_build(const uint8_t *blob, uint32_t total_len, uint8_t *out, uint32_t *off)
+{
+    using namespace flp_detail;
+    dg_desc_hdr h;
+    if (!header(blob, total_len, h)) return;
+    uint32_t at = 0;
+    for (uint32_t s = 0; s < h.n_structs; s++) {
+        if (off) off[s] = FLP_NOPLAN;
+        if (!flp_flat(blob, h, s)) continue;
+        const dg_struct sd = rd<dg_struct>(blob + h.off_structs + sizeof(dg_struct) * s);
+        const uint32_t nk = sd.name_mask + 1 <= FLP_KEYS ? sd.name_mask + 1 : 0u;
+        flp_hdr ph = {sd.field_begin, sd.n_fields, sd.req_begin, sd.name_begin, sd.name_mask, nk, flp_len(sd.n_fields, nk), 0};
+        uint8_t *p = out + at;
+        memset(p, 0, ph.len);
+        memcpy(p, &ph, sizeof ph);
+        auto key_word = [&](uint32_t key_off, uint32_t key_len, uint32_t w) -> uint64_t {
+            if (key_len <= 8 * w || key_off > h.pool_len || 8 * (w + 1) > h.pool_len - key_off) return 0;
+            return rd<uint64_t>(blob + h.off_pool + key_off + 8 * w);
+        };
+        uint8_t *fkm = p + sizeof ph + 32 * sd.n_fields + 20 * nk;
+        for (uint32_t j = 0; j < FLP_SLOTS; j++) {
+            const uint32_t none = 0xFF;
+            memcpy(fkm + 4 * j, &none, 4);
+        }
+        for (uint32_t k = 0; k < sd.n_fields; k++) {
+            const dg_field f = rd<dg_field>(blob + h.off_fields + sizeof(dg_field) * (sd.field_begin + k));
+            const dg_type t = rd<dg_type>(blob + h.off_types + sizeof(dg_type) * f.type);
+            flp_rec r;
+            memset(&r, 0, sizeof r);
+            r.k0 = key_word(f.key_off, f.key_len, 0);
+            r.k1 = key_word(f.key_off, f.key_len, 1);
+            r.key_len = f.key_len;
+            r.id = f.id;
+            r.vm = f.vm;
+            r.ttype = t.ttype;
+            r.bin = (t.flags & DG_TF_BINARY) ? 1 : 0;
+            r.flags = f.flags;
+            r.pred = (f.flags & DG_FF_ALIAS_SELF) && f.key_len <= 16 ? 1 : 0;
+            r.required = f.required;
+            memcpy(p + sizeof ph + 32 * k, &r, sizeof r);
+            if (k < FLP_SLOTS && (f.flags & DG_FF_ALIAS_SELF)) {
+                const uint32_t len = f.key_len;
+                memcpy(fkm + 4 * k, &len, 4);
+            }
+        }
+        uint8_t *kw = p + sizeof ph + 32 * sd.n_fields, *km = kw + 16 * nk;
+        for (uint32_t e = 0; e < nk; e++) {
+            const dg_name nm = rd<dg_name>(blob + h.off_names + sizeof(dg_name) * (sd.name_begin + e));
+            uint32_t mt = 0xFF000000u;
+            uint64_t w0 = 0, w1 = 0;
+            if (nm.field != DG_NONE && nm.key_len <= 16) {
+                w0 = key_word(nm.key_off, nm.key_len, 0);
+                w1 = key_word(nm.key_off, nm.key_len, 1);
+                mt = nm.field | (nm.key_len << 24);
+            }
+            memcpy(kw + 16 * e, &w0, 8);
+            memcpy(kw + 16 * e + 8, &w1, 8);
+            memcpy(km + 4 * e, &mt, 4);
+        }
+        if (off) off[s] = at;
+        at += ph.len;
+    }
+}
+
+}
diff --git a/dynamicgo_amd/csrc/host_internal.h b/dynamicgo_amd/csrc/host_internal.h
--- a/dynamicgo_amd/csrc/host_internal.h
+++ b/dynamicgo_amd/csrc/host_internal.h
@@ -307,6 +307,8 @@
     dg_ctx *ctx = nullptr;
     DevArr<uint8_t> d_blob;
     DevArr<uint8_t> d_flat;
+    std::vector<uint32_t> plan_off;
+    std::vector<uint32_t> plan_len;
     size_t len = 0;
     dg_desc_hdr hdr;
     DevArr<uint8_t> d_side;
diff --git a/dynamicgo_amd/csrc/j2t_fast.h b/dynamicgo_amd/csrc/j2t_fast.h
--- a/dynamicgo_amd/csrc/j2t_fast.h
+++ b/dynamicgo_amd/csrc/j2t_fast.h
@@ -215,6 +215,106 @@
     man = m;
     exp10 = -(int)(nd - pd);
     sgn = neg ? -1 : 1;
+    return true;
+}
+
+
+DGI uint32_t swar_val32(uint64_t x, uint32_t t)
+{
+    const uint32_t t1 = t < 4 ? t : 4u, t2 = t - t1;
+    const uint32_t v1 = swar_val4((uint32_t)x, t1), v2 = swar_val4((uint32_t)(x >> 32), t2);
+    const uint32_t p = t2 == 0 ? 1u : t2 == 1 ? 10u : t2 == 2 ? 100u : t2 == 3 ? 1000u : 10000u;
+    return v1 * p + v2;
+}
+
+template <int W, class S>
+DGI bool fast_int_short(const S &src, int64_t &iv)
+{
+    static_assert(W == 1 || W == 2, "one or two windows");
+    const int32_t n = (int32_t)src.n;
+    if (n < 1 || n > (W == 1 ? 7 : 15)) return false;
+    const uint64_t a0 = src.get8(0);
+    const uint32_t neg = (uint8_t)a0 == '-' ? 1u : 0u;
+    const uint32_t nd = (uint32_t)n - neg;
+    auto nondig = [](uint64_t x) { return (((x & 0x7F7F7F7F7F7F7F7Full) + 0x7676767676767676ull) | x) & 0x8080808080808080ull; };
+    auto upto = [](uint32_t k) { return k >= 8 ? ~0ull : (1ull << (k << 3)) - 1; };
+    if constexpr (W == 1) {
+        const uint64_t x0 = (neg ? a0 >> 8 : a0) ^ 0x3030303030303030ull;
+        if (nd < 1 || (nondig(x0) & upto(nd)) || ((x0 & 0xFF) == 0 && nd > 1)) return false;
+        const uint32_t man = swar_val32(x0, nd);
+        iv = neg ? -(int64_t)man : (int64_t)man;
+    } else {
+        const uint64_t a1 = src.get8(8);
+        const uint64_t x0 = (neg ? (a0 >> 8) | (a1 << 56) : a0) ^ 0x3030303030303030ull,
+                       x1 = (neg ? a1 >> 8 : a1) ^ 0x3030303030303030ull;
+        const uint32_t t0 = nd < 8 ? nd : 8u, t1 = nd - t0;
+        if (nd < 1 || ((nondig(x0) & upto(t0)) | (nondig(x1) & upto(t1))) || ((x0 & 0xFF) == 0 && nd > 1)) return false;
+        uint32_t p = (t1 & 1) ? 10u : 1u;
+        p = (t1 & 2) ? p * 100u : p;
+        p = (t1 & 4) ? p * 10000u : p;
+        const uint64_t man = (uint64_t)swar_val32(x0, t0) * p + swar_val32(x1, t1);
+        iv = neg ? -(int64_t)man : (int64_t)man;
+    }
+    return true;
+}
+
+template <class S>
+DGI bool fast_num_regs(const S &src, const FastTabs &tb, int64_t &iv, double &dv, bool &isint)
+{
+    const int32_t n = (int32_t)src.n;
+    if (n < 1 || n > 21) return false;
+    const uint64_t a0 = src.get8(0), a1 = src.get8(8), a2 = src.get8(16);
+    const uint32_t neg = (uint8_t)a0 == '-' ? 1u : 0u;
+    const uint32_t len = (uint32_t)n - neg;
+    const uint64_t d0 = neg ? (a0 >> 8) | (a1 << 56) : a0, d1 = neg ? (a1 >> 8) | (a2 << 56) : a1,
+                   d2 = neg ? a2 >> 8 : a2;
+    auto upto = [](uint32_t k) { return k >= 8 ? ~0ull : (1ull << (k << 3)) - 1; };
+    auto eqdot = [](uint64_t x) {
+        const uint64_t y = x ^ 0x2E2E2E2E2E2E2E2Eull;
+        return ~(((y & 0x7F7F7F7F7F7F7F7Full) + 0x7F7F7F7F7F7F7F7Full) | y | 0x7F7F7F7F7F7F7F7Full);
+    };
+    const uint32_t u0 = len < 8 ? len : 8u, u1 = len <= 8 ? 0u : len - 8 < 8 ? len - 8 : 8u,
+                   u2 = len <= 16 ? 0u : len - 16;
+    const uint64_t m0 = eqdot(d0) & upto(u0), m1 = eqdot(d1) & upto(u1), m2 = eqdot(d2) & upto(u2);
+    const uint32_t dots = (uint32_t)(__builtin_popcountll(m0) + __builtin_popcountll(m1) + __builtin_popcountll(m2));
+    if (dots > 1) return false;
+    const uint32_t pd = !dots ? len
+                        : m0  ? (uint32_t)__builtin_ctzll(m0) >> 3
+                        : m1  ? 8u + ((uint32_t)__builtin_ctzll(m1) >> 3)
+                              : 16u + ((uint32_t)__builtin_ctzll(m2) >> 3);
+    if (dots && (pd < 1 || pd + 2 > len)) return false;
+    const uint64_t s0 = (d0 >> 8) | (d1 << 56), s1 = (d1 >> 8) | (d2 << 56), s2 = d2 >> 8;
+    const uint64_t k0 = upto(pd), k1 = pd <= 8 ? 0ull : upto(pd - 8), k2 = pd <= 16 ? 0ull : upto(pd - 16);
+    const uint64_t r0 = (d0 & k0) | (s0 & ~k0), r1 = (d1 & k1) | (s1 & ~k1), r2 = (d2 & k2) | (s2 & ~k2);
+    const uint32_t nd = len - dots;
+    const uint64_t x0 = r0 ^ 0x3030303030303030ull, x1 = r1 ^ 0x3030303030303030ull, x2 = r2 ^ 0x3030303030303030ull;
+    auto nondig = [](uint64_t x) { return (((x & 0x7F7F7F7F7F7F7F7Full) + 0x7676767676767676ull) | x) & 0x8080808080808080ull; };
+    const uint32_t t0 = nd < 8 ? nd : 8u, t1 = nd <= 8 ? 0u : nd - 8 < 8 ? nd - 8 : 8u, t2 = nd <= 16 ? 0u : nd - 16;
+    const uint64_t bad = (nondig(x0) & upto(t0)) | (nondig(x1) & upto(t1)) | (nondig(x2) & upto(t2));
+    if (nd < 1 || nd > 19 || bad || ((x0 & 0xFF) == 0 && pd > 1)) return false;
+    auto p10 = [](uint32_t t) {
+        uint32_t p = (t & 1) ? 10u : 1u;
+        p = (t & 2) ? p * 100u : p;
+        p = (t & 4) ? p * 10000u : p;
+        return (t & 8) ? 100000000u : p;
+    };
+    uint64_t man = swar_val32(x0, t0);
+    man = man * (uint64_t)p10(t1) + swar_val32(x1, t1);
+    man = man * (uint64_t)p10(t2) + swar_val32(x2, t2);
+    const int sgn = neg ? -1 : 1;
+    if (!dots) {
+        if ((man >> 63) && !(neg && man == (1ull << 63))) return false;
+        iv = (int64_t)(man * (uint64_t)(int64_t)sgn);
+        dv = man ? with_sign((double)man, sgn) : 0.0;
+        isint = true;
+        return true;
+    }
+    const int exp10 = -(int)(nd - pd);
+    double val;
+    if (!atof_exact_l(man, exp10, sgn, val, tb) && !eisel_lemire_t(man, exp10, sgn, val, tb)) return false;
+    if ((__double_as_longlong(val) << 1) == 0xFFE0000000000000ull) return false;
+    isint = false;
+    dv = val;
     return true;
 }
 
diff --git a/dynamicgo_amd/csrc/j2t_flat.h b/dynamicgo_amd/csrc/j2t_flat.h
--- a/dynamicgo_amd/csrc/j2t_flat.h
+++ b/dynamicgo_amd/csrc/j2t_flat.h
@@ -34,6 +34,7 @@
 constexpr uint32_t FL_KEYS = 32;
 constexpr uint32_t FL_NESC = 8;
 static_assert(FLI_WLO == EL_WLO && FLI_WN == EL_WN, "the image's window is FastTabs' window");
+static_assert(FLP_SLOTS == FL_SLOTS && FLP_KEYS == FL_KEYS, "the plan's key table and order-check lengths are this kernel's");
 constexpr uint32_t FL_FMAPW = FL_SLOTS * FL_MPB / 8;
 static_assert(FL_MAXTASK >= FL_FMAPW + FL_MPB, "the task area holds the field map and, behind it, an unstaged block's offsets");
 #ifndef DG_FL_WPE
@@ -152,6 +153,30 @@
     {
         const uint32_t b = sh + (uint32_t)i, j = b >> 3, s8 = (b & 7) << 3;
         return (word(j) >> s8) | ((word(j + 1) << 1) << (63 - s8));
+    }
+};
+
+struct RSrcV {
+    typedef int32_t idx;
+    uint64_t w0 = 0, w1 = 0, w2 = 0, w3 = 0;
+    uint32_t sh = 0;
+    int32_t n = 0;
+    template <int NW>
+    DGI void load(const LSrc &src, int32_t p)
+    {
+        const uint32_t b = (uint32_t)(src.off0 + p);
+        const __attribute__((address_space(3))) uint64_t *q = src.w8 + (b >> 3);
+        sh = b & 7;
+        w0 = q[0];
+        w1 = q[1];
+        if (NW > 2) w2 = q[2];
+        if (NW > 3) w3 = q[3];
+    }
+    DGI uint64_t get8(int32_t i) const
+    {
+        const uint32_t s8 = sh << 3;
+        const uint64_t lo = i == 0 ? w0 : i == 8 ? w1 : w2, hi = i == 0 ? w1 : i == 8 ? w2 : w3;
+        return (lo >> s8) | ((hi << 1) << (63 - s8));
     }
 };
 
@@ -248,17 +273,58 @@
     return any;
 }
 
+typedef const __attribute__((address_space(3))) uint64_t lds_u64;
+struct FlPlan {
+    lds_u64 *base;
+    uint32_t nf, nk;
+    DGI lds_u64 *rec(uint32_t j) const { return base + 4 + 4 * j; }
+    DGI lds_u64 *kw() const { return base + 4 + 4 * nf; }
+    DGI const __attribute__((address_space(3))) uint32_t *km() const
+    {
+        return (const __attribute__((address_space(3))) uint32_t *)(kw() + 2 * nk);
+    }
+    DGI const __attribute__((address_space(3))) uint32_t *fkm() const { return km() + nk; }
+};
+DGI FlPlan fl_plan(const __attribute__((address_space(3))) uint8_t *p)
+{
+    FlPlan r;
+    r.base = (lds_u64 *)p;
+    r.nf = (uint32_t)(r.base[0] >> 32);
+    r.nk = (uint32_t)(r.base[2] >> 32);
+    return r;
+}
+
+#ifndef DG_FL_TYPED
+#define DG_FL_TYPED 1
+#endif
+#ifndef DG_FL_RSL
+#define DG_FL_RSL 0
+#endif
+
 template <bool KO = false, class S, class DV>
 DGI bool fl_field(const DV &D, const dg_struct &sd, S &src, uint32_t sk, uint32_t ck, uint32_t ek, uint32_t nq,
-                  bool hasbs, lds_esc *E, uint32_t ne, const __attribute__((address_space(3))) uint64_t *KW,
-                  const __attribute__((address_space(3))) uint32_t *KM, uint32_t nk, uint32_t k, uint64_t flag,
+                  bool hasbs, lds_esc *E, uint32_t ne, const FlPlan &PL, uint32_t pj, bool trust, uint64_t flag,
                   const FastTabs &tb, FField &F FLG_ARG)
 {
     typedef typename S::idx SI;
     const uint8_t d_s = src.raw((SI)sk), d_q = src.raw((SI)(ck - 1)), d_v = src.raw((SI)(ck + 1)),
                   d_e = src.raw((SI)(ek - 1));
-    const bool pred = k < sd.n_fields;
-    dg_field f = ldrec(&D.F[sd.field_begin + (pred ? k : 0u)]);
+    const bool pred = pj < sd.n_fields;
+    lds_u64 *R = PL.rec(pred ? pj : 0u);
+    const uint64_t rk0 = R[0], rk1 = R[1], rm0 = R[2];
+    const uint32_t rm1 = (uint32_t)R[3];
+    uint64_t a0 = src.get8((SI)(sk + 1)), a1 = src.get8((SI)(sk + 9));
+    const uint32_t utt = pred ? (uint32_t)__builtin_amdgcn_readfirstlane((int)(uint32_t)(rm0 >> 48)) & 0xFFu : 0u;
+    const bool t_b16 = DG_FL_TYPED && !KO && (utt == DG_T_BYTE || utt == DG_T_I16);
+    const bool t_i32 = DG_FL_TYPED && !KO && utt == DG_T_I32, t_dbl = DG_FL_TYPED && !KO && utt == DG_T_DOUBLE;
+    const bool t_i64 = DG_FL_TYPED && !KO && utt == DG_T_I64;
+    RSrcV vs;
+    auto vload = [&](uint32_t at) {
+        if (t_b16) vs.template load<2>(src, (int32_t)at);
+        else if (t_i32) vs.template load<3>(src, (int32_t)at);
+        else if (t_dbl | t_i64) vs.template load<4>(src, (int32_t)at);
+    };
+    vload(ck + 1);
     uint32_t p = sk, q = ck, v0 = ck + 1, ve = ek;
     uint8_t cs = d_s, cq = d_q, c = d_v, ce = d_e;
     if (isspace_(d_s) | isspace_(d_q) | isspace_(d_v) | isspace_(d_e) | (ck + 1 >= ek)) {
@@ -271,40 +337,54 @@
         cq = src.raw((SI)(q - 1));
         c = src.raw((SI)v0);
         ce = src.raw((SI)(ve - 1));
+        a0 = src.get8((SI)(p + 1));
+        a1 = src.get8((SI)(p + 9));
+        vload(v0);
     }
     if ((q < p + 2) | (cs != '"') | (cq != '"') | (nq != (c == '"' ? 4u : 2u))) return false;
     const uint32_t k0 = p + 1, kn = q - 1 - k0;
     FLG(1);
     uint32_t shrink = 0;
     if (hasbs && fl_esc_in(E, ne, k0, k0 + kn, shrink)) return false;
-    int32_t fi = -1;
-    uint64_t a0m = 0, a1m = 0;
-    {
-        const __attribute__((address_space(3))) uint64_t *pk = (decltype(&D.R[0]))(&D.P[f.key_off]);
-        bool hit;
-        if (kn <= 16) {
-            const uint64_t a0 = src.get8((SI)k0), a1 = src.get8((SI)(k0 + 8)), b0 = pk[0], b1 = pk[1];
-            const uint64_t m0 = kn >= 8 ? ~0ull : (1ull << (kn << 3)) - 1;
-            const uint64_t m1 = kn >= 16 ? ~0ull : kn <= 8 ? 0ull : (1ull << ((kn - 8) << 3)) - 1;
-            a0m = a0 & m0;
-            a1m = a1 & m1;
-            hit = (a0m == b0) & ((kn <= 8) | (a1m == b1));
-        } else {
-            hit = key_eq(src, (SI)k0, kn, pk);
-        }
-        if (pred & ((f.flags & DG_FF_ALIAS_SELF) != 0) & (f.key_len == kn) & hit) fi = (int32_t)(sd.field_begin + k);
-    }
-    if (fi < 0) {
-        if (nk && kn <= 16) {
+    const uint32_t ukl = (uint32_t)__builtin_amdgcn_readfirstlane((int)(uint32_t)rm0) & 0xFFFFu;
+    auto mask0 = [](uint32_t n) { return n >= 8 ? ~0ull : (1ull << (n << 3)) - 1; };
+    auto mask1 = [](uint32_t n) { return n >= 16 ? ~0ull : n <= 8 ? 0ull : (1ull << ((n - 8) << 3)) - 1; };
+    const bool planned = trust | (pred & (((rm1 >> 8) & 0xFF) != 0) & (ukl == kn) & ((a0 & mask0(ukl)) == rk0) &
+                                  ((a1 & mask1(ukl)) == rk1));
+    int32_t fi = (int32_t)(sd.field_begin + pj);
+    uint32_t f_id = (uint32_t)(rm0 >> 16) & 0xFFFFu, f_vm = (uint32_t)(rm0 >> 32) & 0xFFFFu;
+    uint32_t f_tt = (uint32_t)(rm0 >> 48) & 0xFFu, f_bin = (uint32_t)(rm0 >> 56) & 0xFFu, f_flags = rm1 & 0xFFu;
+    if (!planned) {
+        fi = -1;
+        const uint64_t a0m = a0 & mask0(kn), a1m = a1 & mask1(kn);
+        dg_field f = ldrec(&D.F[sd.field_begin + (pred ? pj : 0u)]);
+        if (kn > 16) {
+            const __attribute__((address_space(3))) uint64_t *pk = (decltype(&D.R[0]))(&D.P[f.key_off]);
+            if (pred & ((f.flags & DG_FF_ALIAS_SELF) != 0) & (f.key_len == kn) && key_eq(src, (SI)k0, kn, pk))
+                fi = (int32_t)(sd.field_begin + pj);
+        }
+        if (fi < 0) {
+            if (PL.nk && kn <= 16) {
+                lds_u64 *KW = PL.kw();
+                const __attribute__((address_space(3))) uint32_t *KM = PL.km();
 #pragma unroll 4
-            for (uint32_t e = 0; e < nk; e++) {
-                const uint32_t mt = KM[e];
-                if (((mt >> 24) == kn) & (KW[2 * e] == a0m) & (KW[2 * e + 1] == a1m)) fi = (int32_t)(mt & 0xFFFFFFu);
-            }
-        } else {
-            fi = fl_lookup(D, sd, src, k0, kn);
-        }
-        if (fi >= 0) f = ldrec(&D.F[fi]);
+                for (uint32_t e = 0; e < PL.nk; e++) {
+                    const uint32_t mt = KM[e];
+                    if (((mt >> 24) == kn) & (KW[2 * e] == a0m) & (KW[2 * e + 1] == a1m)) fi = (int32_t)(mt & 0xFFFFFFu);
+                }
+            } else {
+                fi = fl_lookup(D, sd, src, k0, kn);
+            }
+            if (fi >= 0) f = ldrec(&D.F[fi]);
+        }
+        if (!KO && fi >= 0) {
+            const dg_type ft = ldrec(&D.T[f.type]);
+            f_tt = ft.ttype;
+            f_bin = (ft.flags & DG_TF_BINARY) ? 1u : 0u;
+        }
+        f_id = f.id;
+        f_vm = f.vm;
+        f_flags = f.flags;
     }
     if constexpr (KO) {
         F.fi = fi;
@@ -324,11 +404,22 @@
         vesc = hasbs && fl_esc_in(E, ne, vs0, vs0 + vnb, shrink);
         vk = FV_STR;
     } else if (c == '-' || (uint8_t)(c - '0') <= 9) {
-        const bool later = DG_FL_DEFER_NUM && fi >= 0 && !((flag & DG_F_ENABLE_VM) && f.vm != DG_VM_NONE);
-        if (!later) {
-            const int32_t nl = (int32_t)(ve - v0);
+        const bool later = DG_FL_DEFER_NUM && fi >= 0 && !((flag & DG_F_ENABLE_VM) && f_vm != DG_VM_NONE);
+        const int32_t nl = (int32_t)(ve - v0);
+        bool done = false;
+        if (!later && (t_b16 | t_i32 | t_i64 | t_dbl) && planned && !((flag & DG_F_ENABLE_VM) && f_vm != DG_VM_NONE)) {
+            vs.n = nl;
+            if (t_b16) done = fast_int_short<1>(vs, iv);
+            else if (t_i32) done = fast_int_short<2>(vs, iv);
+            else if (t_i64) {
+                int32_t e;
+                done = fast_int_regs(vs, iv, dv, e);
+            } else done = fast_num_regs(vs, tb, iv, dv, isint);
+            if (!t_dbl) isint = done;
+        }
+        if (!later && !done) {
             bool okn;
-            if (nl <= RSL_MAX) {
+            if (DG_FL_RSL && nl <= RSL_MAX) {
                 RSrcL rs;
                 rs.load(src, (int32_t)v0, nl);
                 int32_t qq = 0;
@@ -355,22 +446,21 @@
     }
     FLG(3);
     F.fi = fi;
-    if (fi < 0 || ((f.flags & DG_FF_REQUEST_BASE) && (flag & DG_F_NO_WRITE_BASE))) {
+    if (fi < 0 || ((f_flags & DG_FF_REQUEST_BASE) && (flag & DG_F_NO_WRITE_BASE))) {
         if (fi < 0 && !(flag & DG_F_ALLOW_UNKNOWN)) return false;
         if (fi >= 0) return false;
         F.kind = FV_NONE;
         F.size = 0;
         return true;
     }
-    const dg_type ft = ldrec(&D.T[f.type]);
-    const uint8_t tt = ft.ttype;
-    const bool bin = (ft.flags & DG_TF_BINARY) && !(flag & DG_F_NO_BASE64);
+    const uint8_t tt = (uint8_t)f_tt;
+    const bool bin = f_bin && !(flag & DG_F_NO_BASE64);
     F.tt = tt;
-    F.id = f.id;
+    F.id = (uint16_t)f_id;
     F.i16q = false;
     uint32_t vsize;
-    if ((flag & DG_F_ENABLE_VM) && f.vm != DG_VM_NONE) {
-        if (f.vm != DG_VM_JSCONV) return false;
+    if ((flag & DG_F_ENABLE_VM) && f_vm != DG_VM_NONE) {
+        if (f_vm != DG_VM_JSCONV) return false;
         if (vk == FV_STR && tt != DG_T_STRING) {
             if (vnb == 0 || vesc) return false;
             S sub = src.sub((SI)vs0, (SI)vnb);
@@ -523,6 +613,7 @@
     uint32_t wrap;
     uint32_t wrap_inner;
     uint64_t wrap_ok;
+    uint32_t plan_off, plan_len;
 };
 
 #ifdef DG_FLPROF
@@ -575,9 +666,6 @@
     uint32_t wid[FL_MPB];
     uint32_t nesc[FL_MPB];
     uint32_t esc[FL_MPB * FL_NESC];
-    uint64_t kw[2 * FL_KEYS];
-    uint32_t km[FL_KEYS];
-    uint32_t fkm[FL_SLOTS];
     uint32_t sep[FL_MAXF * FL_MPB];
     uint16_t col[FL_MAXF * FL_MPB];
     uint16_t size[2 * FL_SLOTS * FL_MPB];
@@ -606,9 +694,14 @@
     static_assert(FL_WAVES >= 4, "the prologue gives waves 0..3 a part each");
 
     const uint32_t blob16 = fli_blob16(S.hdr.total_len);
-    const uint32_t ni = (blob16 + FLI_TABS) >> 4;
+    const uint32_t ni0 = (blob16 + FLI_TABS) >> 4;
+    const uint32_t ni = ni0 + (S.plan_len >> 4), pskip = (S.plan_off >> 4) - ni0;
     const uint4 *gi = (const uint4 *)S.img;
-    const uint4 i0 = gi[min(tid, ni - 1)], i1 = gi[min(tid + NT, ni - 1)];
+    auto isrc = [&](uint32_t u) {
+        u = min(u, ni - 1);
+        return u < ni0 ? u : u + pskip;
+    };
+    const uint4 i0 = gi[isrc(tid)], i1 = gi[isrc(tid + NT)];
     const uint64_t *po = (wave & 1) ? P.out_off : P.in_off;
     const uint64_t ov = po[b0 + min(lane, nb)];
     const uint64_t lo = P.in_off[b0], hi = P.in_off[b1], oend = P.out_off[b1];
@@ -678,7 +771,7 @@
         uint4 *li = (uint4 *)s_fdesc;
         if (tid < ni) li[tid] = i0;
         if (tid + NT < ni) li[tid + NT] = i1;
-        for (uint32_t k = tid + 2 * NT; k < ni; k += NT) li[k] = gi[k];
+        for (uint32_t k = tid + 2 * NT; k < ni; k += NT) li[k] = gi[isrc(k)];
     }
     __syncthreads();
     const uint32_t g = tid & 3, m1 = tid >> 2;
@@ -712,32 +805,20 @@
         (const __attribute__((address_space(3))) uint8_t *)(void *)s_fdesc + blob16;
     const FastTabs tb{(const __attribute__((address_space(3))) uint64_t *)(tabs + FLI_P10U), (lds_f64 *)(tabs + FLI_P10D),
                       (const __attribute__((address_space(3))) uint64_t *)(tabs + FLI_PW)};
-    const dg_type rt = ldrec(&D.T[S.wrap ? S.wrap_inner : P.root]);
-    const dg_struct sd = ldrec(&D.S[rt.st]);
-    const uint32_t nk = sd.name_mask + 1 <= FL_KEYS ? sd.name_mask + 1 : 0u;
-    if (tid < nk) {
-        const dg_name nm = ldrec(&D.N[sd.name_begin + tid]);
-        uint32_t mt = 0xFF000000u;
-        uint64_t w0 = 0, w1 = 0;
-        if (nm.field != DG_NONE && nm.key_len <= 16) {
-            const __attribute__((address_space(3))) uint64_t *pk = (decltype(&D.R[0]))(&D.P[nm.key_off]);
-            w0 = nm.key_len ? pk[0] : 0ull;
-            w1 = nm.key_len > 8 ? pk[1] : 0ull;
-            mt = nm.field | (nm.key_len << 24);
-        }
-        L.km[tid] = mt;
-        L.kw[2 * tid] = w0;
-        L.kw[2 * tid + 1] = w1;
-    }
-    if (tid >= 64 && tid < 64 + FL_SLOTS) {
-        const uint32_t j = tid - 64;
-        uint32_t len = 0xFF;
-        if (j < sd.n_fields) {
-            const dg_field f = ldrec(&D.F[sd.field_begin + j]);
-            if (f.flags & DG_FF_ALIAS_SELF) len = f.key_len;
-        }
-        L.fkm[j] = len;
-    }
+    const FlPlan PL = fl_plan((const __attribute__((address_space(3))) uint8_t *)(void *)s_fdesc + blob16 + FLI_TABS);
+    dg_struct sd;
+    {
+        const uint64_t h0 = PL.base[0], h1 = PL.base[1], h2 = PL.base[2];
+        sd.field_begin = (uint32_t)h0;
+        sd.n_fields = (uint32_t)(h0 >> 32);
+        sd.req_begin = (uint32_t)h1;
+        sd.name_begin = (uint32_t)(h1 >> 32);
+        sd.name_mask = (uint32_t)h2;
+        sd.req_words = 1;
+        sd.flags = 0;
+        sd._pad = 0;
+    }
+    const uint32_t nk = PL.nk;
     if (S.wrap) {
         if (tid < FL_MPB) {
             uint32_t wid = 0;
@@ -926,7 +1007,11 @@
 #ifndef DG_FL_ROT
 #define DG_FL_ROT 1
 #endif
-        const uint32_t fwave = DG_FL_ROT ? (wave + blockIdx.x) % FL_WAVES : wave;
+#ifndef DG_FL_SFW
+#define DG_FL_SFW 1
+#endif
+        const uint32_t fw0 = DG_FL_SFW ? wv : wave;
+        const uint32_t fwave = DG_FL_ROT ? (fw0 + blockIdx.x) % FL_WAVES : fw0;
         const uint32_t ok0 = L.ok[mm], lwa = L.lw[mm], oc = L.oc[mm], nfq = L.nfq[mm];
         const uint32_t nf = nfq & 0xFF, qtot = (nfq >> 8) & 0x3FF;
         const bool hasbs = (nfq >> 31) != 0;
@@ -937,13 +1022,12 @@
         const uint32_t rounds = L.rounds;
         uint32_t nbytes = 0;
         lds_esc *E = (lds_esc *)(void *)&L.esc[mm * FL_NESC];
-        const __attribute__((address_space(3))) uint64_t *KW = (const __attribute__((address_space(3))) uint64_t *)(void *)L.kw;
-        const __attribute__((address_space(3))) uint32_t *KM = (const __attribute__((address_space(3))) uint32_t *)(void *)L.km;
         const uint32_t ne = min(L.nesc[mm], FL_NESC);
 #ifdef DG_FLPROF_G
         uint64_t flg[8] = {0, 0, 0, 0, 0, 0, 0, __builtin_amdgcn_s_memtime()};
 #endif
-        auto parse = [&](uint32_t k, FField &F) {
+        uint64_t present = 0;
+        auto parse = [&](uint32_t k, uint32_t pj, bool trust, FField &F) {
             F.size = 0;
             F.kind = FV_NONE;
             if (ok0 && k < nf) {
@@ -957,14 +1041,12 @@
                 }
                 const uint32_t ck = L.col[k * FL_MPB + mm];
                 FLG(0);
-                if (!(ck >= sk && ck < ek && fl_field(D, sd, src, sk, ck, ek, q1 - q0, hasbs, E, ne, KW, KM, nk, k, P.flag, tb, F FLG_PASS))) {
+                if (!(ck >= sk && ck < ek && fl_field(D, sd, src, sk, ck, ek, q1 - q0, hasbs, E, ne, PL, pj, trust, P.flag, tb, F FLG_PASS))) {
                     L.ok[mm] = 0;
                     F.size = 0;
                     F.kind = FV_NONE;
                 } else if (F.fi >= 0) {
-                    const uint32_t bit = (uint32_t)F.fi - sd.field_begin;
-                    atomicOr(&L.plo[mm], bit < 32 ? 1u << (bit & 31) : 0u);
-                    atomicOr(&L.phi[mm], bit >= 32 ? 1u << (bit & 31) : 0u);
+                    present |= 1ull << (((uint32_t)F.fi - sd.field_begin) & 63);
                 }
                 FLG(5);
             }
@@ -991,7 +1073,7 @@
                 if (ok0 && k < nf) {
                     const uint32_t sk = k ? (L.sep[(k - 1) * FL_MPB + mm] & 0xFFFF) + 1 : (oc & 0xFFFF) + 1;
                     const uint32_t ck = L.col[k * FL_MPB + mm];
-                    mis |= (k >= sd.n_fields || L.fkm[k] != ck - sk - 2) ? 1u : 0u;
+                    mis |= (k >= sd.n_fields || PL.fkm()[k] != ck - sk - 2) ? 1u : 0u;
                 }
             }
             if (ballot(mis != 0) && lane == 0) atomicOr(&L.noremap, 2u);
@@ -1016,7 +1098,7 @@
                     FField G;
                     G.fi = -1;
                     if (!(ck >= sk && ck < ek &&
-                          fl_field<true>(D, sd, src, sk, ck, ek, q1 - q0, hasbs, E, ne, KW, KM, nk, k, P.flag, tb, G FLG_PASS)) ||
+                          fl_field<true>(D, sd, src, sk, ck, ek, q1 - q0, hasbs, E, ne, PL, k, false, P.flag, tb, G FLG_PASS)) ||
                         G.fi < 0) {
                         fail = 1;
                     } else {
@@ -1034,18 +1116,22 @@
             FField F[FL_FPW];
             uint32_t kslot[FL_FPW];
             uint16_t *sz = &L.size[(r & 1) * FL_SLOTS * FL_MPB];
-#pragma unroll
-            for (uint32_t h = 0; h < FL_FPW; h++) {
+            auto convert = [&](uint32_t h) __attribute__((always_inline)) {
                 FLF_T0();
                 const uint32_t j = fl_slot(fwave, h);
                 const uint32_t k = remap ? (uint32_t)fmap[j * FL_MPB + mm] : r * FL_SLOTS + j;
                 const uint32_t si = remap ? k : j;
                 kslot[h] = si;
-                parse(k, F[h]);
+                parse(k, remap ? j : k, remap, F[h]);
                 if (si < FL_SLOTS) sz[si * FL_MPB + mm] = (uint16_t)F[h].size;
                 if (remap && j >= nf) sz[j * FL_MPB + mm] = 0;
                 FLF_ADD(r * FL_SLOTS + fl_slot(fwave, h));
-            }
+            };
+            static_assert(FL_FPW <= 4, "a call of convert() per slot");
+            convert(0);
+            if (FL_FPW > 1) convert(1);
+            if (FL_FPW > 2) convert(2);
+            if (FL_FPW > 3) convert(3);
             FLP(4);
             __syncthreads();
             FLP(5);
@@ -1109,6 +1195,8 @@
             if (!good) L.ok[mm] = 0;
             FLP(6);
         }
+        if ((uint32_t)present) atomicOr(&L.plo[mm], (uint32_t)present);
+        if ((uint32_t)(present >> 32)) atomicOr(&L.phi[mm], (uint32_t)(present >> 32));
         if (wave == 0) L.nbytes[mm] = nbytes;
 #ifdef DG_FLPROF_G
         if (lane == 0 && (blockIdx.x & 31) == 0)
@@ -1159,10 +1247,11 @@
                 while (bits) {
                     const uint32_t kk = (uint32_t)__builtin_ctzll(bits);
                     bits &= bits - 1;
-                    const dg_field f = ldrec(&D.F[sd.field_begin + kk]);
-                    if (f.flags & DG_FF_REQUEST_BASE) continue;
-                    if (f.required == DG_REQ_REQUIRED || ((flag & DG_F_WRITE_DEFAULT) && f.required == DG_REQ_DEFAULT) ||
-                        ((flag & DG_F_WRITE_OPTIONAL) && f.required == DG_REQ_OPTIONAL)) {
+                    const uint32_t rm1 = (uint32_t)PL.rec(kk)[3];
+                    const uint32_t required = (rm1 >> 16) & 0xFF;
+                    if (rm1 & DG_FF_REQUEST_BASE) continue;
+                    if (required == DG_REQ_REQUIRED || ((flag & DG_F_WRITE_DEFAULT) && required == DG_REQ_DEFAULT) ||
+                        ((flag & DG_F_WRITE_OPTIONAL) && required == DG_REQ_OPTIONAL)) {
                         good = false;
                         break;
                     }
diff --git a/dynamicgo_amd/csrc/j2t_host.hip b/dynamicgo_amd/csrc/j2t_host.hip
--- a/dynamicgo_amd/csrc/j2t_host.hip
+++ b/dynamicgo_amd/csrc/j2t_host.hip
@@ -181,9 +181,24 @@
     if (h.magic != DG_DESC_MAGIC || h.version < 1 || h.version > DG_DESC_VERSION || h.total_len > len)
         return set_err(DG_E_DESC, "bad descriptor blob header");
     DevArr<uint8_t> d_flat;
+    std::vector<uint32_t> plan_off, plan_len;
     if (h.version >= 2 && h.total_len <= FL_DESC) {
-        std::vector<uint8_t> img(fli_len(h.total_len));
-        flat_image_build((const uint8_t *)host_blob, h.total_len, img.data());
+        const uint8_t *hb = (const uint8_t *)host_blob;
+        const uint32_t il = fli_len(h.total_len);
+        std::vector<uint8_t> img((size_t)il + flp_total(hb, h.total_len));
+        flat_image_build(hb, h.total_len, img.data());
+        if (img.size() > il) {
+            plan_off.assign(h.n_structs, FLP_NOPLAN);
+            plan_len.assign(h.n_structs, 0u);
+            flp_build(hb, h.total_len, img.data() + il, plan_off.data());
+            for (uint32_t s = 0; s < h.n_structs; s++) {
+                if (plan_off[s] == FLP_NOPLAN) continue;
+                flp_hdr ph;
+                memcpy(&ph, img.data() + il + plan_off[s], sizeof ph);
+                plan_off[s] += il;
+                plan_len[s] = ph.len;
+            }
+        }
         if (int rc = d_flat.alloc(img.size())) return rc;
         HIPCHK(hipMemcpy(d_flat, img.data(), img.size(), hipMemcpyHostToDevice));
     }
@@ -191,6 +206,8 @@
     d->ctx = c;
     d->d_blob = std::move(d_blob);
     d->d_flat = std::move(d_flat);
+    d->plan_off = std::move(plan_off);
+    d->plan_len = std::move(plan_len);
     d->len = len;
     d->hdr = h;
     d->hblob.assign((const uint8_t *)host_blob, (const uint8_t *)host_blob + h.total_len);
@@ -206,6 +223,7 @@
     const dg_type *T = (const dg_type *)(b + h.off_types);
     if (T[root].ttype != DG_T_STRUCT) return false;
     const dg_struct &sd = ((const dg_struct *)(b + h.off_structs))[T[root].st];
+    if (T[root].st >= d->plan_off.size() || d->plan_off[T[root].st] == FLP_NOPLAN) return false;
     if (sd.req_words != 1 || ((flags & DG_F_ENABLE_HM) && (sd.flags & DG_SF_HTTP_MAPPING))) return false;
     const dg_field *F = (const dg_field *)(b + h.off_fields);
     for (uint32_t k = 0; k < sd.n_fields; k++) {
@@ -437,6 +455,12 @@
         FP.wrap = wrap_ok ? 1u : 0u;
         FP.wrap_inner = wrap_ok ? inner : 0u;
         FP.wrap_ok = wrap_ok;
+        {
+            const dg_type *T = (const dg_type *)(d->hblob.data() + d->hdr.off_types);
+            const uint32_t st = T[wrap_ok ? inner : root].st;
+            FP.plan_off = d->plan_off[st];
+            FP.plan_len = d->plan_len[st];
+        }
         launch_flat_kernel(dim3((uint32_t)((n + FL_MPB - 1) / FL_MPB)), s, P1, FP);
     } else {
         SmallParams S;
diff --git a/dynamicgo_amd/csrc/j2t_kern_flat.hip b/dynamicgo_amd/csrc/j2t_kern_flat.hip
--- a/dynamicgo_amd/csrc/j2t_kern_flat.hip
+++ b/dynamicgo_amd/csrc/j2t_kern_flat.hip
@@ -3,7 +3,7 @@
 namespace dg {
 void launch_flat_kernel(dim3 grid, hipStream_t s, const Params &P, const FlatParams &S)
 {
-    const uint32_t shmem = fli_len(S.hdr.total_len);
+    const uint32_t shmem = fli_len(S.hdr.total_len) + S.plan_len;
     hipLaunchKernelGGL(j2t_flat_kernel<0>, grid, dim3(64 * FL_WAVES), shmem, s, P, S);
 }
 }
```

New measurement: 463.4 GB/s, median of 6. Within noise of the previous version (+0.9%).
